# mandyxmq/NeuralBTF-tiny-cuda-nn

Measured on AMD Instinct MI355X. Metric: training steps/sec at batch=2^18, config_hash.json (HashGrid+64-wide MLP), higher is better.
Workload: dtype fp16 storage / fp32 MFMA accumulate; 1 GPU; HashGrid L16 F2 log2T15 s1.5 base16 + FullyFusedMLP W64 H2 ReLU, RelativeL2, Adam, B=2^18; global_batch=262144, per_gpu_batch=262144, parallelism=dp1

## Files before the change

### neuralbtf-tiny-cuda-nn_amd/csrc/capi.cpp

```cpp
#include "../../include/tcnn_mi355x.h"
#include "debug_api.h"

#include <algorithm>
#include <cstring>
#include <mutex>

#include "runtime.h"

using namespace tcnn_amd;

namespace {
thread_local std::string g_last_error;
thread_local std::string g_str;

std::mutex g_log_mutex;
tcnn_log_callback_t g_log_cb = nullptr;
void* g_log_user = nullptr;

template <typename F>
int guard(F&& f) {
	try {
		f();
		return 0;
	} catch (const std::exception& e) {
		g_last_error = e.what();
	} catch (...) {
		g_last_error = "unknown C++ exception";
	}
	return 1;
}

template <typename T, typename F>
T* guard_ptr(F&& f) {
	try {
		return f();
	} catch (const std::exception& e) {
		g_last_error = e.what();
	} catch (...) {
		g_last_error = "unknown C++ exception";
	}
	return nullptr;
}

json parse_json(const char* s) {
	if (!s || !*s) return json::object();
	return json::parse(std::string(s));
}

struct KeepPool {
	std::mutex mu;
	std::vector<std::unique_ptr<DevBuf>> free;
	std::unique_ptr<DevBuf> get() {
		std::lock_guard<std::mutex> lk(mu);
		if (free.empty()) return std::make_unique<DevBuf>();
// ... 643 lines not shown
}
const char* tcnn_trainer_engine(const tcnn_trainer* t) { return t->t->model->engine(); }
const char* tcnn_trainer_inference_engine(const tcnn_trainer* t) { return t->t->model->inference_engine(); }
const char* tcnn_module_engine(const tcnn_module* m) { return m->m->engine(); }
const char* tcnn_module_inference_engine(const tcnn_module* m) { return m->m->inference_engine(); }
int tcnn_trainer_set_max_level(tcnn_trainer* t, float max_level) {
	return guard([&] {
		TCNN_CHECK(t->t->model->grid != nullptr, "trainer model has no grid encoding");
		t->t->model->grid->max_level = max_level;
	});
}

int tcnn_trainer_profile_begin(tcnn_trainer* t) { return tcnn_trainer_profile_begin_sampled(t, 1); }
int tcnn_trainer_profile_begin_sampled(tcnn_trainer* t, uint32_t every) {
	return guard([&] {
		t->t->timer.reset();
		t->t->timer.every = every ? every : 1;
		t->t->timer.counter = 0;
		t->t->timer.enabled = true;
	});
}
int tcnn_trainer_profile_end(tcnn_trainer* t, double* ms, uint32_t n_phases, uint32_t* n_steps) {
	return guard([&] { t->t->profile_end(ms, n_phases, n_steps); });
}

int tcnn_debug_fused_phase_cycles(tcnn_trainer* t, void* stream, uint32_t n, const float* input, const float* target,
                                  uint64_t* host_cycles8) {
	return guard([&] {
		auto& tr = *t->t;
		auto& m = *tr.model;
		TCNN_CHECK(m.mlp.width == 64 && m.mlp.n_input == 32 && m.mlp.n_hidden_layers == 2 && m.grid->desc.n_pos_dims == 2,
		           "phase profile: config_hash shape only");
		hipStream_t st = (hipStream_t)stream;
		tr.training_step(st, n, input, target, false);
		const uint32_t nb = fused_train_n_blocks(64, 32, 2, 2, tr.n_output_dims, false, n);
		const size_t WV = fused_train_waves();
		DevBuf prof;
		prof.reserve((size_t)nb * WV * 16 * 8);
		TCNN_HIP_CHECK(hipMemsetAsync(prof.p, 0, (size_t)nb * WV * 16 * 8, st));
		launch_fused_train_profile(st, n, tr.n_output_dims, tr.w16.p, (const uint8_t*)tr.w16.p + tr.n_mlp * 2, input, target,
		                           tr.ws.dLdenc.p, tr.ws.wgrad_partial.as<float>(), tr.ws.loss_partial.as<float>(),
		                           m.grid->dev_levels(), nb, tr.ws.wimage.p, prof.as<unsigned long long>());
		std::vector<unsigned long long> h((size_t)nb * WV * 16);
		TCNN_HIP_CHECK(hipMemcpyAsync(h.data(), prof.p, h.size() * 8, hipMemcpyDeviceToHost, st));
		TCNN_HIP_CHECK(hipStreamSynchronize(st));
		for (int k = 0; k < 16; ++k) {
			unsigned long long sum = 0;
			for (size_t w = 0; w < (size_t)nb * WV; ++w) sum += h[w * 16 + k];
			host_cycles8[k] = sum;
		}
	});
}

int tcnn_debug_hfma(void* stream, const void* a, const void* b, const void* c, void* out, uint32_t n_pairs) {
	return guard([&] { launch_probe_hfma((hipStream_t)stream, a, b, c, out, n_pairs); });
}

int tcnn_debug_probe(void* stream, float* mfma_out, int16_t* tr_out) {
	return guard([&] { launch_probe((hipStream_t)stream, mfma_out, tr_out); });
}

}

namespace tcnn_amd {
void log_msg(LogSeverity s, const std::string& msg) {
	std::lock_guard<std::mutex> lk(g_log_mutex);
	if (g_log_cb) g_log_cb((int)s, msg.c_str(), g_log_user);
}
}
```

### neuralbtf-tiny-cuda-nn_amd/csrc/dp.cpp

```cpp
#include <dlfcn.h>

#include <rccl/rccl.h>

#include <cstring>
#include <mutex>

#include "runtime.h"

namespace tcnn_amd {

namespace {
struct RcclApi {
	decltype(&ncclGetUniqueId) get_unique_id = nullptr;
	decltype(&ncclCommInitRank) comm_init_rank = nullptr;
	decltype(&ncclCommDestroy) comm_destroy = nullptr;
	decltype(&ncclAllReduce) all_reduce = nullptr;
	decltype(&ncclReduceScatter) reduce_scatter = nullptr;
	decltype(&ncclAllGather) all_gather = nullptr;
	decltype(&ncclGetErrorString) error_string = nullptr;
};

const RcclApi& rccl() {
	static std::once_flag once;
	static RcclApi api;
// ... 56 lines not shown
	if (n) check(rccl().all_reduce(buf, buf, n, ncclFloat32, ncclSum, (ncclComm_t)comm, st), "ncclAllReduce");
}

void DpComm::reduce_scatter_f32(float* buf, size_t per, hipStream_t st) {
	check(rccl().reduce_scatter(buf, buf + (size_t)rank * per, per, ncclFloat32, ncclSum, (ncclComm_t)comm, st), "ncclReduceScatter");
}

void DpComm::all_gather(void* buf, size_t per_elems, int elem_bytes, hipStream_t st) {
	const ncclDataType_t t = elem_bytes == 2 ? ncclFloat16 : ncclUint32;
	check(rccl().all_gather((const uint8_t*)buf + (size_t)rank * per_elems * elem_bytes, buf, per_elems, t, (ncclComm_t)comm, st),
	      "ncclAllGather");
}

static void grow_preserve(DevBuf& b, size_t bytes, size_t valid) {
	if (b.bytes >= bytes) return;
	DevBuf n;
	n.reserve(bytes);
	TCNN_HIP_CHECK(hipMemset(n.p, 0, bytes));
	if (b.p && valid) TCNN_HIP_CHECK(hipMemcpy(n.p, b.p, valid, hipMemcpyDeviceToDevice));
	std::swap(b.p, n.p);
	std::swap(b.bytes, n.bytes);
}

void TrainerHost::set_dp(DpComm* c, bool sharded) {
	TCNN_CHECK(!peer_attached, "set_dp: the trainer is attached to a peer exchange (detach it first)");
	if (dp && dp_sharded && dp_state_partial) dp_gather_state(nullptr);
	TCNN_HIP_CHECK(hipDeviceSynchronize());
	dp = c;
	dp_sharded = c && sharded;
	dp_state_partial = false;
	grad_scale = grad_scale_user / (float)dp_nranks();
	if (graph) set_graph(use_graph);
	if (!dp_sharded) return;
	const uint64_t N = (uint64_t)c->nranks;
	dp_per = (n_params + N - 1) / N;
	const size_t pad = (size_t)(dp_per * N);
	grow_preserve(w32, pad * 4, n_params * 4);
	grow_preserve(w16, pad * 2, n_params * 2);
	grow_preserve(g16, pad * 2, n_params * 2);
	grow_preserve(g32, pad * 4, n_params * 4);
	grow_preserve(m1, pad * 4, n_params * 4);
	grow_preserve(m2, pad * 4, n_params * 4);
	grow_preserve(steps, pad * 4, n_params * 4);
	ws.wimage_valid = false;
}

void TrainerHost::training_step_dp(hipStream_t st, uint32_t B, const float* input, const float* target) {
	DpComm& c = *dp;
	NetworkHost& m = *model;
	const size_t nm = (size_t)n_mlp;
	float* g = g32.as<float>();
	mark(st, 0);
	if (overlapped_ok()) {
		m.fused_kernel(st, ws, B, input, target, n_output_dims, loss_scale, w16.p, false);
		launch_column_sums(st, ws.wgrad_partial.as<float>(), ws.n_fused_blocks, (uint32_t)n_mlp, g);
		launch_sum(st, ws.loss_partial.as<float>(), ws.n_loss_partials, d_loss.as<float>());
		if (!dp_sharded) {
			TCNN_HIP_CHECK(hipEventRecord(c.ev[0], st));
			TCNN_HIP_CHECK(hipStreamWaitEvent(c.cs, c.ev[0], 0));
			c.all_reduce_f32(g, nm, c.cs);
		}
		mark(st, 1);
		m.grid_backward(st, ws, B, input);
		m.grid->backward_acc(st, ws.gbw, B, ws.dLdenc.p, 0, 0, g + nm);
		m.grid->reduce_items(st, ws.gbw, g + nm);
	} else {
		m.fwd_bwd(st, ws, B, input, target, n_output_dims, loss_scale, w16.p, nullptr, nullptr, g);
		launch_sum(st, ws.loss_partial.as<float>(), ws.n_loss_partials, d_loss.as<float>());
		mark(st, 1);
	}
	mark(st, 2);
	TCNN_HIP_CHECK(hipEventRecord(c.ev[1], st));
	TCNN_HIP_CHECK(hipStreamWaitEvent(c.cs, c.ev[1], 0));
	if (dp_sharded) c.reduce_scatter_f32(g, (size_t)dp_per, c.cs);
	else if (overlapped_ok()) c.all_reduce_f32(g + nm, (size_t)(n_params - nm), c.cs);
	else c.all_reduce_f32(g, (size_t)n_params, c.cs);
	TCNN_HIP_CHECK(hipEventRecord(c.ev[2], c.cs));
	TCNN_HIP_CHECK(hipStreamWaitEvent(st, c.ev[2], 0));
	last_B = B;
	if (dp_sharded) {
		const uint64_t lo = std::min<uint64_t>(n_params, (uint64_t)c.rank * dp_per), hi = std::min<uint64_t>(n_params, lo + dp_per);
		optimizer_step_range(st, lo, hi);
		c.all_gather(w16.p, (size_t)dp_per, 2, st);
		dp_state_partial = true;
	} else {
		optimizer_step(st);
	}
	mark(st, 3);
}

void TrainerHost::dp_gather_state(hipStream_t st) {
	if (peer_attached) {
		if (dp_state_partial) dp_peer_gather_state(st);
		return;
	}
	if (!dp || !dp_sharded || !dp_state_partial) return;
	for (DevBuf* b : {&w32, &m1, &m2, &steps}) dp->all_gather(b->p, (size_t)dp_per, 4, st);
	TCNN_HIP_CHECK(hipStreamSynchronize(st));
	dp_state_partial = false;
}

}
```

### neuralbtf-tiny-cuda-nn_amd/csrc/fused.hip

```cpp
#include "kernels.h"

#include <cstdlib>

#include "grid_device.h"
#include "mlp_fused.h"

namespace tcnn_amd {

#define TCNN_FUSED_SHAPES(X) \
	X(64, 32, 2)             \
	X(64, 32, 1)             \
	X(32, 32, 2)             \
	X(32, 32, 1)

bool fused_train_supported(uint32_t W, uint32_t IN, uint32_t NH, uint32_t D, uint32_t F, uint32_t OUTP, int act, HashType h) {
	if (F != 2 || OUTP != 16 || (D != 2 && D != 3) || (act != 0 && act != 1)) return false;
#define X(w, in, nh) if (W == w && IN == in && NH == nh) return true;
	TCNN_FUSED_SHAPES(X)
#undef X
	return false;
}

size_t fused_weight_image_bytes(uint32_t W, uint32_t IN, uint32_t NH) {
#define X(w, in, nh) if (W == w && IN == in && NH == nh) return (size_t)FusedLayout<w, in, nh>::oStage * 2;
// ... 40 lines not shown
}

uint32_t fused_train_waves() { return FUSED_WAVES; }

uint32_t fused_train_n_blocks(uint32_t W, uint32_t IN, uint32_t NH, uint32_t D, uint32_t dims, bool ext_dout, uint32_t B) {
	const uint32_t n_cu = device_cu_count();
	const uint32_t nb = div_round_up(B, 32u * FUSED_WAVES);
	const uint32_t cap = (8u / FUSED_WAVES) * n_cu;
	return nb < cap ? nb : cap;
}

template <int W, int IN, int NH, uint32_t D, HashType H, Act A, bool EXT, bool ENC = false>
static void launch_fused_e(hipStream_t st, const FusedTrainArgs& args, uint32_t n_blocks) {
	constexpr size_t bytes = RegKernelLayout<W, IN, NH>::BYTES;
	static uint64_t done = 0;
	set_dyn_lds((const void*)k_fused_train_grid<W, IN, NH, D, H, A, EXT, ENC>, (int)bytes, done);
	hipLaunchKernelGGL((k_fused_train_grid<W, IN, NH, D, H, A, EXT, ENC>), dim3(n_blocks), dim3(64 * FUSED_WAVES), bytes, st, args);
	TCNN_HIP_CHECK(hipGetLastError());
}

template <int W, int IN, int NH, uint32_t D, HashType H, Act A>
static void launch_fused_t(hipStream_t st, const FusedTrainArgs& args, uint32_t n_blocks) {
	if (args.enc) {
		if (args.dout) launch_fused_e<W, IN, NH, 2, HashType::CoherentPrime, A, true, true>(st, args, n_blocks);
		else launch_fused_e<W, IN, NH, 2, HashType::CoherentPrime, A, false, true>(st, args, n_blocks);
	} else if (args.dout) {
		launch_fused_e<W, IN, NH, D, H, A, true>(st, args, n_blocks);
	} else {
		launch_fused_e<W, IN, NH, D, H, A, false>(st, args, n_blocks);
	}
}

template <int W, int IN, int NH>
static void launch_fused_shape(hipStream_t st, uint32_t D, HashType h, int act, const FusedTrainArgs& a, uint32_t nb) {
#define DISPATCH_H(DD, AA)                                                                                   \
	switch (h) {                                                                                          \
		case HashType::Prime: launch_fused_t<W, IN, NH, DD, HashType::Prime, AA>(st, a, nb); break;       \
		case HashType::ReversedPrime: launch_fused_t<W, IN, NH, DD, HashType::ReversedPrime, AA>(st, a, nb); break; \
		default: launch_fused_t<W, IN, NH, DD, HashType::CoherentPrime, AA>(st, a, nb); break;            \
	}
	if (D == 2) {
		if (act == 1) { DISPATCH_H(2, Act::ReLU) } else { DISPATCH_H(2, Act::None) }
	} else {
		if (act == 1) { DISPATCH_H(3, Act::ReLU) } else { DISPATCH_H(3, Act::None) }
	}
#undef DISPATCH_H
}

void launch_fused_train(hipStream_t st, uint32_t W, uint32_t IN, uint32_t NH, uint32_t D, HashType h, int act,
                        uint32_t B, uint32_t dims, float loss_scale, const void* params16, const void* table16,
                        const float* pos, const float* target, void* out16, void* dLdenc_pairs,
                        float* wgrad_partial, float* loss_partial, const LevelInfo* levels, bool hash_grid,
                        Interp interp, uint32_t n_blocks, const void* dout16, const void* wimage, uint32_t loss_l2,
                        bool inrange_index, const void* enc16, float dout_scale) {
	TCNN_CHECK(B % 32 == 0, "fused train: batch must be a multiple of 32");
	TCNN_CHECK(wimage || ((uintptr_t)params16 & 15) == 0, "fused train: parameters must be 16-byte aligned");
	FusedTrainArgs a;
	a.enc = (const _Float16*)enc16;
	a.loss_l2 = loss_l2;
	a.inrange_index = inrange_index ? 1u : 0u;
	a.wimage = (const _Float16*)wimage;
	a.dout = (const _Float16*)dout16;
	a.dout_scale = dout_scale;
	a.B = B;
	a.dims = dims;
	a.loss_scale = loss_scale;
	a.n_total = (float)(B * dims);
	a.params = (const _Float16*)params16;
	a.table = (const uint32_t*)table16;
	a.pos = pos;
	a.target = target;
	a.out = (_Float16*)out16;
	a.dLdenc = (uint32_t*)dLdenc_pairs;
	a.wgrad_partial = wgrad_partial;
	a.loss_partial = loss_partial;
	a.levels = levels;
	a.hash_grid = hash_grid ? 1u : 0u;
	a.interp = (uint32_t)interp;
	a.prof = nullptr;
#define X(w, in, nh) if (W == w && IN == in && NH == nh) { launch_fused_shape<w, in, nh>(st, D, h, act, a, n_blocks); return; }
	TCNN_FUSED_SHAPES(X)
#undef X
	throw std::runtime_error("fused train: unsupported shape");
}

template <int W, int IN, int NH, Act A, bool SOA>
static void launch_infer_t(hipStream_t st, uint32_t B, const void* wimage, const void* in, void* out) {
	constexpr size_t bytes = (size_t)FusedLayout<W, IN, NH>::oStage * 2;
	static uint64_t done = 0;
	set_dyn_lds((const void*)k_mlp_infer<W, IN, NH, A, SOA>, (int)bytes, done);
	uint32_t nb = div_round_up(B, 64);
	if (nb > 1024) nb = 1024;
	hipLaunchKernelGGL((k_mlp_infer<W, IN, NH, A, SOA>), dim3(nb), dim3(256), bytes, st, B, (const _Float16*)wimage,
	                   (const _Float16*)in, (_Float16*)out);
	TCNN_HIP_CHECK(hipGetLastError());
}

bool mlp_infer_supported(uint32_t W, uint32_t IN, uint32_t NH, uint32_t OUTP, int act) {
	if (OUTP != 16 || (act != 0 && act != 1)) return false;
#define X(w, in, nh) if (W == w && IN == in && NH == nh) return true;
	TCNN_FUSED_SHAPES(X)
#undef X
	return false;
}

void launch_mlp_infer(hipStream_t st, uint32_t W, uint32_t IN, uint32_t NH, int act, bool soa, uint32_t B,
                      const void* wimage, const void* in16, void* out16) {
	TCNN_CHECK(B % 16 == 0, "mlp inference: batch must be a multiple of 16");
	if (B == 0) return;
#define X(w, in, nh)                                                                                      \
	if (W == w && IN == in && NH == nh) {                                                                 \
		if (act == 1) { if (soa) launch_infer_t<w, in, nh, Act::ReLU, true>(st, B, wimage, in16, out16);   \
		                else launch_infer_t<w, in, nh, Act::ReLU, false>(st, B, wimage, in16, out16); }    \
		else { if (soa) launch_infer_t<w, in, nh, Act::None, true>(st, B, wimage, in16, out16);            \
		       else launch_infer_t<w, in, nh, Act::None, false>(st, B, wimage, in16, out16); }             \
		return;                                                                                           \
	}
	TCNN_FUSED_SHAPES(X)
#undef X
	throw std::runtime_error("mlp inference: unsupported shape");
}

template <int W, int IN, int NH, uint32_t D, HashType H, Act A>
static void launch_fused_fwd_t(hipStream_t st, const FusedFwdArgs& a) {
	constexpr size_t bytes = FwdLayout<W, IN, NH>::BYTES;
	static uint64_t done = 0;
	set_dyn_lds((const void*)k_fused_fwd_grid<W, IN, NH, D, H, A>, (int)bytes, done);
	uint32_t nb = div_round_up(a.B, 16u * FWD_WAVES);
	const uint32_t cap = 3 * device_cu_count();
	if (nb > cap) nb = cap;
	hipLaunchKernelGGL((k_fused_fwd_grid<W, IN, NH, D, H, A>), dim3(nb), dim3(64 * FWD_WAVES), bytes, st, a);
	TCNN_HIP_CHECK(hipGetLastError());
// ... 77 lines not shown
```

### neuralbtf-tiny-cuda-nn_amd/csrc/grid.hip

```cpp
#include "kernels.h"

#include <algorithm>
#include <cstdio>
#include <cstdlib>
#include <vector>

#include "adam_device.h"
#include "grid_bwd_lds.h"
#include "grid_device.h"

namespace tcnn_amd {

template <uint32_t D, uint32_t F, HashType H>
__global__ __launch_bounds__(256) void k_grid_fwd(uint32_t B, const float* __restrict__ pos, uint32_t pstride,
                                                  const _Float16* __restrict__ table, _Float16* __restrict__ out,
                                                  uint32_t soa, uint32_t out_stride, const LevelInfo* __restrict__ levels,
                                                  uint32_t hash_grid, uint32_t interp_u, const GridOpts o, uint32_t L) {
	uint32_t i, level;
	if (soa) {
		i = blockIdx.x * blockDim.x + threadIdx.x;
		level = blockIdx.y;
	} else {
		const uint32_t t = blockIdx.x * blockDim.x + threadIdx.x;
		i = t / L;
// ... 515 lines not shown
template <uint32_t D, typename T>
static void grid_bwd_bwd_f(hipStream_t st, uint32_t F, HashType h, dim3 g, uint32_t B, uint32_t L, const float* pos, uint32_t ps,
                           const T* t, const float* gx, const T* dy, uint32_t dys, float* grad, T* ddy,
                           uint32_t ddys, float* dx, const LevelInfo* lv, uint32_t hg, uint32_t in, const GridOpts& go) {
	switch (F) {
		case 1: grid_bwd_bwd_h<D, 1, T>(st, h, g, B, L, pos, ps, t, gx, dy, dys, grad, ddy, ddys, dx, lv, hg, in, go); break;
		case 2: grid_bwd_bwd_h<D, 2, T>(st, h, g, B, L, pos, ps, t, gx, dy, dys, grad, ddy, ddys, dx, lv, hg, in, go); break;
		case 4: grid_bwd_bwd_h<D, 4, T>(st, h, g, B, L, pos, ps, t, gx, dy, dys, grad, ddy, ddys, dx, lv, hg, in, go); break;
		case 8: grid_bwd_bwd_h<D, 8, T>(st, h, g, B, L, pos, ps, t, gx, dy, dys, grad, ddy, ddys, dx, lv, hg, in, go); break;
		default: throw std::runtime_error("GridEncoding: n_features_per_level must be 1, 2, 4 or 8");
	}
}

template <typename T>
static void grid_bwd_bwd_t(hipStream_t st, uint32_t D, uint32_t F, HashType h, uint32_t B, uint32_t L, const float* pos, uint32_t pos_stride,
                           const T* t, const float* dL_ddLdx, const T* dy, uint32_t dy_stride, float* grad32, T* ddy, uint32_t ddy_stride,
                           float* dx, const LevelInfo* levels, bool hash_grid, Interp interp, const GridOpts& go) {
	if (B == 0) return;
	const dim3 g(div_round_up(B, 256));
	const uint32_t hg = hash_grid ? 1u : 0u, in = (uint32_t)interp;
	switch (D) {
		case 2: grid_bwd_bwd_f<2, T>(st, F, h, g, B, L, pos, pos_stride, t, dL_ddLdx, dy, dy_stride, grad32, ddy, ddy_stride, dx, levels, hg, in, go); break;
		case 3: grid_bwd_bwd_f<3, T>(st, F, h, g, B, L, pos, pos_stride, t, dL_ddLdx, dy, dy_stride, grad32, ddy, ddy_stride, dx, levels, hg, in, go); break;
		case 4: grid_bwd_bwd_f<4, T>(st, F, h, g, B, L, pos, pos_stride, t, dL_ddLdx, dy, dy_stride, grad32, ddy, ddy_stride, dx, levels, hg, in, go); break;
		default: throw std::runtime_error("GridEncoding: number of input dims must be 2, 3 or 4");
	}
	TCNN_HIP_CHECK(hipGetLastError());
}

void launch_grid_bwd_bwd(hipStream_t st, uint32_t D, uint32_t F, HashType h, uint32_t B, uint32_t L, const float* pos,
                         uint32_t pos_stride, const void* table16, const float* dL_ddLdx, const void* dLdy16, uint32_t dy_stride,
                         float* grad32, void* dLddLdy16, uint32_t ddy_stride, float* dx, const LevelInfo* levels, bool hash_grid,
                         Interp interp, const GridOpts& go) {
	grid_bwd_bwd_t<_Float16>(st, D, F, h, B, L, pos, pos_stride, (const _Float16*)table16, dL_ddLdx, (const _Float16*)dLdy16, dy_stride, grad32,
	                         (_Float16*)dLddLdy16, ddy_stride, dx, levels, hash_grid, interp, go);
}

void launch_grid_bwd_bwd_f32(hipStream_t st, uint32_t D, uint32_t F, HashType h, uint32_t B, uint32_t L, const float* pos,
                             uint32_t pos_stride, const float* table32, const float* dL_ddLdx, const float* dLdy32, uint32_t dy_stride,
                             float* grad32, float* dLddLdy32, uint32_t ddy_stride, float* dx, const LevelInfo* levels, bool hash_grid,
                             Interp interp, const GridOpts& go) {
	grid_bwd_bwd_t<float>(st, D, F, h, B, L, pos, pos_stride, table32, dL_ddLdx, dLdy32, dy_stride, grad32, dLddLdy32, ddy_stride, dx, levels,
	                      hash_grid, interp, go);
}

static DevBufLite g_dbg_times;
static bool dbg_grid_times() {
	static const bool on = std::getenv("TCNN_DEBUG_GRID_TIMES") != nullptr;
	return on;
}

uint32_t grid_bwd_slot_budget() { return GRID_BWD_SLOTS; }

extern template void grid_bwd_f<2>(hipStream_t, uint32_t, HashType, int, uint32_t, dim3, size_t, uint32_t, const float*, uint32_t,
                                   const _Float16*, const GridSlice*, float*, uint32_t, const LevelInfo*, uint32_t, uint32_t, uint32_t,
                                   const GridBwdLaunch&);
extern template void grid_bwd_f<3>(hipStream_t, uint32_t, HashType, int, uint32_t, dim3, size_t, uint32_t, const float*, uint32_t,
                                   const _Float16*, const GridSlice*, float*, uint32_t, const LevelInfo*, uint32_t, uint32_t, uint32_t,
                                   const GridBwdLaunch&);
extern template void grid_bwd_f<4>(hipStream_t, uint32_t, HashType, int, uint32_t, dim3, size_t, uint32_t, const float*, uint32_t,
                                   const _Float16*, const GridSlice*, float*, uint32_t, const LevelInfo*, uint32_t, uint32_t, uint32_t,
                                   const GridBwdLaunch&);

void launch_grid_bwd(hipStream_t st, uint32_t D, uint32_t F, HashType h, uint32_t B, const float* pos,
                     uint32_t pos_stride, const void* dLdy16, int dy_layout, uint32_t dy_stride, const GridSlice* slices,
                     uint32_t n_slices, uint32_t n_chunks, float* partial, uint32_t partial_stride,
                     const LevelInfo* levels, bool hash_grid, Interp interp, const GridBwdEpilogue* ep, const GridOpts& go,
                     const GridSlice* host_slices, const LevelInfo* host_levels, uint32_t n_levels) {
	const uint32_t n_tail = (ep && ep->enabled) ? ep->n_mlp_groups : 0u;
	if (n_tail == 0 && (n_slices == 0 || B == 0)) return;
	if (B == 0) n_slices = 0;
	const uint32_t ppc = div_round_up(std::max(B, 1u), n_chunks);
	GridBwdLaunch gl{};
	gl.n_items = n_slices;
	gl.n_chunks = n_chunks;
	if (ep) gl.ep = *ep;
	else gl.ep.enabled = 0;
	gl.dbg_times = nullptr;
	gl.opts = go;
	gl.tb.n_items = gl.tb.n_levels = 0;
	if (host_slices && host_levels && n_slices <= GRID_BWD_ARG_ITEMS && n_levels <= GRID_BWD_ARG_LEVELS) {
		gl.tb.n_items = n_slices;
		gl.tb.n_levels = n_levels;
		std::copy(host_slices, host_slices + n_slices, gl.tb.items);
		std::copy(host_levels, host_levels + n_levels, gl.tb.levels);
	}
	dim3 g(n_slices * n_chunks + n_tail);
	if (dbg_grid_times()) gl.dbg_times = (unsigned long long*)g_dbg_times.get((size_t)g.x * 64);
	const size_t lds = GRID_BWD_LDS_BYTES;
	const _Float16* dy = (const _Float16*)dLdy16;
	switch (D) {
		case 2: grid_bwd_f<2>(st, F, h, dy_layout, dy_stride, g, lds, B, pos, pos_stride, dy, slices, partial, partial_stride, levels, hash_grid, (uint32_t)interp, ppc, gl); break;
		case 3: grid_bwd_f<3>(st, F, h, dy_layout, dy_stride, g, lds, B, pos, pos_stride, dy, slices, partial, partial_stride, levels, hash_grid, (uint32_t)interp, ppc, gl); break;
		case 4: grid_bwd_f<4>(st, F, h, dy_layout, dy_stride, g, lds, B, pos, pos_stride, dy, slices, partial, partial_stride, levels, hash_grid, (uint32_t)interp, ppc, gl); break;
		default: throw std::runtime_error("GridEncoding: number of input dims must be 2, 3 or 4");
	}
	TCNN_HIP_CHECK(hipGetLastError());
	if (gl.dbg_times) {
		std::vector<unsigned long long> t((size_t)g.x * 8);
		TCNN_HIP_CHECK(hipStreamSynchronize(st));
		TCNN_HIP_CHECK(hipMemcpy(t.data(), gl.dbg_times, t.size() * 8, hipMemcpyDeviceToHost));
		unsigned long long t0 = ~0ull, t1 = 0;
		for (uint32_t b = 0; b < g.x; ++b) { t0 = std::min(t0, t[8 * b]); t1 = std::max(t1, t[8 * b + 4]); }
		fprintf(stderr, "grid_bwd: %u items x %u chunks + %u tail, span %.1f us\n", n_slices, n_chunks, n_tail, (t1 - t0) / 100.0);
		for (uint32_t it = 0; it < n_slices; ++it) {
			double sum = 0, mx = 0, st0 = 1e30, ph[4] = {0, 0, 0, 0}, ld = 0, zr = 0;
			for (uint32_t c = 0; c < n_chunks; ++c) {
				const uint32_t b = it * n_chunks + c;
				const double d = (t[8 * b + 4] - t[8 * b]) / 100.0;
				sum += d; mx = std::max(mx, d); st0 = std::min(st0, (t[8 * b] - t0) / 100.0);
				for (int k = 0; k < 4; ++k) ph[k] += (t[8 * b + k + 1] - t[8 * b + k]) / 100.0 / n_chunks;
					ld += ((double)t[8 * b + 5] - (double)t[8 * b]) / 100.0 / n_chunks;
					zr += ((double)t[8 * b + 6] - (double)t[8 * b]) / 100.0 / n_chunks;
			}
			fprintf(stderr, "  item %2u: mean %.1f max %.1f us, first start +%.1f | prepass %.1f (zero %.1f, +loads %.1f) accumulate %.1f merge %.1f write %.1f\n", it,
			        sum / n_chunks, mx, st0, ph[0], zr, ld, ph[1], ph[2], ph[3]);
		}
		for (uint32_t b = n_slices * n_chunks; b < g.x; ++b)
			fprintf(stderr, "  tail wg %u: %.1f us start +%.1f\n", b - n_slices * n_chunks, (t[8 * b + 4] - t[8 * b]) / 100.0, (t[8 * b] - t0) / 100.0);
	}
}

}
```

### neuralbtf-tiny-cuda-nn_amd/csrc/grid_bwd_lds.h

```cpp
#pragma once

#include "kernels.h"

#include <algorithm>
#include <cstdio>
#include <cstdlib>
#include <vector>

#include "adam_device.h"
#include "grid_device.h"

namespace tcnn_amd {

constexpr uint32_t GRID_BWD_THREADS = 1024;
constexpr uint32_t GRID_BWD_LDS_BYTES = 128 * 1024;
constexpr uint32_t GRID_BWD_SLOTS = GRID_BWD_LDS_BYTES / 4;



__device__ __forceinline__ void lds_add_i32(int* acc, float v) {
	__hip_atomic_fetch_add(acc, __float2int_rn(v), __ATOMIC_RELAXED, __HIP_MEMORY_SCOPE_WORKGROUP);
}

enum : int { IDX_HASH_POW2 = 0, IDX_DENSE = 1, IDX_GENERIC = 2, IDX_HASH_RANGE = 3 };

template <uint32_t D, HashType H, int KIND>
__device__ __forceinline__ uint32_t level_index(bool hash_grid, uint32_t size, uint32_t res, const uint32_t* g) {
	if constexpr (KIND == IDX_HASH_POW2 || KIND == IDX_HASH_RANGE) {
		uint32_t h = 0;
#pragma unroll
		for (uint32_t d = 0; d < D; ++d) h ^= g[d] * hash_prime<H>(d);
		return h & (size - 1);
	} else if constexpr (KIND == IDX_DENSE) {
		uint32_t idx = 0, stride = 1;
#pragma unroll
		for (uint32_t d = 0; d < D; ++d) {
			idx += g[d] * stride;
			stride *= res;
		}
		if (idx >= size) {
			idx -= size;
			if (idx >= size) idx %= size;
		}
		return idx;
	} else {
		return grid_index<D, H>(hash_grid, size, res, g);
	}
}

template <uint32_t D, uint32_t F, HashType H, int KIND, int MODE, bool OPTS>
__device__ __forceinline__ void accum_point(const float (&x)[D], const float (&dy)[F], uint32_t i, uint32_t level, uint32_t B,
                                            const LevelInfo& li, bool hash_grid, Interp interp, uint32_t begin, uint32_t len,
                                            uint32_t f0, uint32_t nf, int* acc, const GridOpts& o) {
	float p[D];
	uint32_t pg[D];
#pragma unroll
	for (uint32_t d = 0; d < D; ++d) pos_fract(x[d], li.scale, interp, p[d], pg[d]);
	const bool nearest = interp == Interp::Nearest;
	const bool single = nearest || (OPTS && o.stochastic);
	uint32_t cbits = 0;
	if (single && !nearest) {
		const float smp = random_val_1337(i + level * B);
// ... 49 lines not shown
		t[1][1] = t[1][0] + hash_prime<H>(1);
	} else {
		t[0][0] = g[0];
		t[0][1] = g[0] + 1u;
		t[1][0] = g[1] * li.res;
		t[1][1] = t[1][0] + li.res;
	}
#pragma unroll
	for (uint32_t c = 0; c < 4; ++c) {
		const uint32_t bx = c & 1u, by = c >> 1;
		const float w = (bx ? p[0] : 1.0f - p[0]) * (by ? p[1] : 1.0f - p[1]);
		const float wh = (float)f16_rn(w);
		uint32_t rel;
		if constexpr (KIND == IDX_HASH_POW2) {
			rel = (t[0][bx] ^ t[1][by]) & (li.size - 1u);
		} else if constexpr (KIND == IDX_HASH_RANGE) {
			rel = ((t[0][bx] ^ t[1][by]) & (li.size - 1u)) - begin;
			if (rel >= len) continue;
		} else {
			const uint32_t d = t[0][bx] + t[1][by];
			rel = __builtin_elementwise_min(d, d - li.size);
		}
		if constexpr (MODE == 0) {
			const int a = __float2int_rn(wh * dy[0]);
			const int b = __float2int_rn(wh * dy[1]);
			const unsigned long long pk = (unsigned long long)(((long long)b << 32) + (long long)a);
			__hip_atomic_fetch_add((unsigned long long*)acc + rel, pk, __ATOMIC_RELAXED, __HIP_MEMORY_SCOPE_WORKGROUP);
		} else {
#pragma unroll
			for (uint32_t f = 0; f < F; ++f) {
				if constexpr (MODE == 1) {
					if (f - f0 < nf) lds_add_i32(&acc[rel * nf + (f - f0)], wh * dy[f]);
				} else {
					lds_add_i32(&acc[rel * F + f], wh * dy[f]);
				}
			}
		}
	}
}

constexpr uint32_t GRID_BWD_PR = 32, GRID_BWD_PU = 8;
static_assert(GRID_BWD_THREADS * GRID_BWD_PR == GRID_BWD_REG_POINTS, "kernels.h GRID_BWD_REG_POINTS");
template <uint32_t D>
__device__ __forceinline__ void load_pos_batch(const float* __restrict__ pos, uint32_t pstride, uint32_t i0, uint32_t i1, uint32_t k,
                                               float (&dst)[GRID_BWD_PU][D]) {
#pragma unroll
	for (uint32_t u = 0; u < GRID_BWD_PU; ++u) {
		const uint32_t i = i0 + threadIdx.x + (k * GRID_BWD_PU + u) * blockDim.x;
#pragma unroll
		for (uint32_t d = 0; d < D; ++d) dst[u][d] = i < i1 ? pos[(size_t)i * pstride + d] : 0.0f;
	}
}

template <uint32_t D, uint32_t F, HashType H, int KIND, int MODE>
__device__ __forceinline__ void grid_bwd_points_regs(const uint32_t (&dyb)[GRID_BWD_PR], const float (&xs0)[GRID_BWD_PU][D],
                                                     uint32_t B, const float* __restrict__ pos,
                                                     uint32_t pstride, uint32_t level, const LevelInfo& li, bool hash_grid,
                                                     Interp interp, uint32_t begin, uint32_t len, uint32_t f0, uint32_t nf,
                                                     uint32_t i0, uint32_t i1, float scale, int* acc, const GridOpts& o) {
	constexpr uint32_t U = GRID_BWD_PU, NB = GRID_BWD_PR / U;
	constexpr bool FAST_KIND = D == 2 && (KIND == IDX_HASH_POW2 || KIND == IDX_DENSE || KIND == IDX_HASH_RANGE);
	const bool fast = FAST_KIND && interp == Interp::Linear && (begin == 0 || KIND == IDX_HASH_RANGE);
	float xs[2][U][D];
#pragma unroll
	for (uint32_t u = 0; u < U; ++u)
#pragma unroll
		for (uint32_t d = 0; d < D; ++d) xs[0][u][d] = xs0[u][d];
#pragma unroll
	for (uint32_t k = 0; k < NB; ++k) {
		if (i0 + threadIdx.x + k * U * blockDim.x >= i1) break;
		if (k + 1 < NB) load_pos_batch<D>(pos, pstride, i0, i1, k + 1, xs[(k + 1) & 1]);
		bool fast_b = fast;
		if constexpr (FAST_KIND && KIND == IDX_DENSE) {
			bool inr = true;
#pragma unroll
			for (uint32_t u = 0; u < U; ++u)
#pragma unroll
				for (uint32_t d = 0; d < D; ++d) inr = inr && xs[k & 1][u][d] >= 0.0f && xs[k & 1][u][d] <= 1.0f;
			fast_b = fast_b && __builtin_amdgcn_ballot_w64(!inr) == 0;
		}
		if (fast_b) {
			if constexpr (FAST_KIND) {
				if (i0 + threadIdx.x + (k * U + U - 1) * blockDim.x < i1) {
#pragma unroll
					for (uint32_t u = 0; u < U; ++u) {
						const uint32_t p = k * U + u;
						float dy[F];
#pragma unroll
						for (uint32_t f = 0; f < F; ++f) dy[f] = dy_bits_feature(dyb[p], f) * scale;
						accum_point_2d_fast<F, H, KIND, MODE>(*(const float(*)[2]) & xs[k & 1][u][0], dy, li, f0, nf, acc, begin, len);
					}
				} else {
#pragma unroll
					for (uint32_t u = 0; u < U; ++u) {
						const uint32_t p = k * U + u;
						if (i0 + threadIdx.x + p * blockDim.x >= i1) break;
						float dy[F];
#pragma unroll
						for (uint32_t f = 0; f < F; ++f) dy[f] = dy_bits_feature(dyb[p], f) * scale;
						accum_point_2d_fast<F, H, KIND, MODE>(*(const float(*)[2]) & xs[k & 1][u][0], dy, li, f0, nf, acc, begin, len);
					}
				}
			}
			continue;
		}
#pragma unroll
		for (uint32_t u = 0; u < U; ++u) {
			const uint32_t p = k * U + u;
			const uint32_t i = i0 + threadIdx.x + p * blockDim.x;
			if (i >= i1) break;
			float dy[F];
#pragma unroll
			for (uint32_t f = 0; f < F; ++f) dy[f] = dy_bits_feature(dyb[p], f) * scale;
			accum_point<D, F, H, KIND, MODE, false>(xs[k & 1][u], dy, i, level, B, li, hash_grid, interp, begin, len, f0, nf, acc, o);
		}
	}
}

template <uint32_t D, uint32_t F, HashType H, int KIND, int MODE, bool OPTS>
__device__ __forceinline__ void grid_bwd_points(int layout, uint32_t B, const float* __restrict__ pos, uint32_t pstride,
                                                const _Float16* __restrict__ dLdy, uint32_t dy_stride, uint32_t level,
                                                const LevelInfo& li, bool hash_grid, Interp interp, uint32_t begin,
                                                uint32_t len, uint32_t f0, uint32_t nf, uint32_t i0, uint32_t i1, float scale,
                                                int* acc, const GridOpts& o) {
	constexpr uint32_t NF = F;
	constexpr uint32_t U = 8;
	constexpr bool FAST_KIND = D == 2 && !OPTS && (KIND == IDX_HASH_POW2 || KIND == IDX_DENSE || KIND == IDX_HASH_RANGE);
	const bool fast = FAST_KIND && interp == Interp::Linear && (begin == 0 || KIND == IDX_HASH_RANGE);
	for (uint32_t base = i0 + threadIdx.x; base < i1; base += U * blockDim.x) {
		float xs[U][D], dy[U][NF];
#pragma unroll
		for (uint32_t u = 0; u < U; ++u) {
			const uint32_t i = base + u * blockDim.x;
			float v[F];
			if (i < i1) {
#pragma unroll
				for (uint32_t d = 0; d < D; ++d) xs[u][d] = pos[(size_t)i * pstride + d];
				load_dy<F>(layout, dLdy, dy_stride, level, B, i, v);
			} else {
#pragma unroll
				for (uint32_t d = 0; d < D; ++d) xs[u][d] = 0.0f;
#pragma unroll
				for (uint32_t f = 0; f < F; ++f) v[f] = 0.0f;
			}
			if (OPTS && i < i1 && (float)level > grid_max_level(o, i, F) + 1e-3f) {
#pragma unroll
				for (uint32_t f = 0; f < F; ++f) v[f] = 0.0f;
			}
#pragma unroll
			for (uint32_t f = 0; f < F; ++f) dy[u][f] = v[f] * scale;
		}
		if constexpr (FAST_KIND) {
			bool fast_b = fast;
			if constexpr (KIND == IDX_DENSE) {
				bool inr = true;
#pragma unroll
				for (uint32_t u = 0; u < U; ++u)
#pragma unroll
					for (uint32_t d = 0; d < D; ++d) inr = inr && xs[u][d] >= 0.0f && xs[u][d] <= 1.0f;
				fast_b = fast_b && __builtin_amdgcn_ballot_w64(!inr) == 0;
			}
			if (fast_b && base + (U - 1) * blockDim.x < i1) {
#pragma unroll
				for (uint32_t u = 0; u < U; ++u)
					accum_point_2d_fast<F, H, KIND, MODE>(*(const float(*)[2]) & xs[u][0], dy[u], li, f0, nf, acc, begin, len);
				continue;
			}
		}
#pragma unroll
		for (uint32_t u = 0; u < U; ++u) {
			if (base + u * blockDim.x >= i1) break;
			accum_point<D, F, H, KIND, MODE, OPTS>(xs[u], dy[u], base + u * blockDim.x, level, B, li, hash_grid, interp, begin, len, f0,
			                                       nf, acc, o);
		}
	}
}

template <uint32_t D, uint32_t F, HashType H, int KIND, bool OPTS>
__device__ __forceinline__ void grid_bwd_mode(int mode, int layout, uint32_t B, const float* pos, uint32_t pstride,
                                              const _Float16* dLdy, uint32_t dy_stride, uint32_t level, const LevelInfo& li,
                                              bool hash_grid, Interp interp, uint32_t begin, uint32_t len, uint32_t f0,
                                              uint32_t nf, uint32_t i0, uint32_t i1, float scale, int* acc, const GridOpts& o) {
	if constexpr (F == 2) {
		if (mode == 0) { grid_bwd_points<D, F, H, KIND, 0, OPTS>(layout, B, pos, pstride, dLdy, dy_stride, level, li, hash_grid, interp, begin, len, f0, nf, i0, i1, scale, acc, o); return; }
	} else if constexpr (F > 2) {
		if (mode == 2) { grid_bwd_points<D, F, H, KIND, 2, OPTS>(layout, B, pos, pstride, dLdy, dy_stride, level, li, hash_grid, interp, begin, len, f0, nf, i0, i1, scale, acc, o); return; }
	}
	grid_bwd_points<D, F, H, KIND, 1, OPTS>(layout, B, pos, pstride, dLdy, dy_stride, level, li, hash_grid, interp, begin, len, f0, nf, i0, i1, scale, acc, o);
}

template <uint32_t D, uint32_t F, HashType H, int KIND>
__device__ __forceinline__ void grid_bwd_mode_regs(int mode, const uint32_t (&dyb)[GRID_BWD_PR], const float (&xs0)[GRID_BWD_PU][D],
                                                   uint32_t B, const float* pos,
                                                   uint32_t pstride, uint32_t level, const LevelInfo& li, bool hash_grid, Interp interp,
                                                   uint32_t begin, uint32_t len, uint32_t f0, uint32_t nf, uint32_t i0, uint32_t i1,
                                                   float scale, int* acc, const GridOpts& o) {
	if constexpr (F == 2) {
		if (mode == 0) { grid_bwd_points_regs<D, F, H, KIND, 0>(dyb, xs0, B, pos, pstride, level, li, hash_grid, interp, begin, len, f0, nf, i0, i1, scale, acc, o); return; }
	}
	grid_bwd_points_regs<D, F, H, KIND, 1>(dyb, xs0, B, pos, pstride, level, li, hash_grid, interp, begin, len, f0, nf, i0, i1, scale, acc, o);
}

__device__ __forceinline__ void grid_bwd_mlp_tail(const GridBwdEpilogue& ep, uint32_t g, float* lds) {
	const uint32_t N = ep.n_mlp;
	const uint32_t cb = column_block(N, ep.n_mlp_groups);
	const uint32_t c0 = g * cb;
	if (c0 < N) {
		const uint32_t ncol = min(cb, N - c0);
		float* out = lds;
		float* tmp = lds + cb;
		block_column_sums(ep.wpart, ep.n_wparts, N, c0, ncol, tmp, out);
		const uint32_t nW0 = ep.W * ep.IN, nWh = (ep.NH - 1) * ep.W * ep.W;
		for (uint32_t t = threadIdx.x; t < ncol; t += blockDim.x) {
			const uint32_t i = c0 + t;
			const float s = out[t];
			if (ep.fin.out) {
				grad_finalize_store(s, ep.fin.s, ep.fin.out, i, ep.fin.out_f32);
				continue;
			}
			ep.buf.g32[i] = s;
			if (!ep.apply_adam) continue;
			const _Float16 h = adam_update(ep.adam_mlp, ep.buf, i, s);
			uint32_t o;
			if (i < nW0) {
				o = (i / ep.IN) * ep.RSI + i % ep.IN;
			} else if (i < nW0 + nWh) {
				const uint32_t k = i - nW0;
				o = ep.oWh + (k / ep.W) * ep.RSW + k % ep.W;
			} else {
				const uint32_t k = i - nW0 - nWh;
				o = ep.oWo + (4 * ((k / ep.W) & 3) + (k / ep.W) / 4) * ep.RSW + k % ep.W;
			}
			ep.wimage[o] = h;
		}
	}
	if (g == 0) {
		__syncthreads();
		const float l = block_sum_fixed(ep.lpart, ep.n_wparts, lds);
		if (threadIdx.x == 0) *ep.d_loss = l;
	}
}

constexpr uint32_t GRID_BWD_ARG_ITEMS = 32, GRID_BWD_ARG_LEVELS = 24;
struct GridBwdTables {
	uint32_t n_items, n_levels;
	GridSlice items[GRID_BWD_ARG_ITEMS];
	LevelInfo levels[GRID_BWD_ARG_LEVELS];
};

template <uint32_t D, uint32_t F, HashType H, bool OPTS>
__global__ __launch_bounds__(GRID_BWD_THREADS) void k_grid_bwd_lds(
	int layout, uint32_t B, const float* __restrict__ pos, uint32_t pstride, const _Float16* __restrict__ dLdy, uint32_t dy_stride,
	const GridSlice* __restrict__ items, float* __restrict__ partial, uint32_t partial_stride,
	const LevelInfo* __restrict__ levels, uint32_t hash_grid, uint32_t interp_u, uint32_t pts_per_chunk, uint32_t n_items,
	uint32_t n_chunks, const GridBwdEpilogue ep, unsigned long long* dbg_times, const GridOpts o, const GridBwdTables tb) {
	extern __shared__ __attribute__((aligned(16))) int acc[];
	const unsigned long long t_start = dbg_times ? wall_clock64() : 0ull;
	__shared__ float red[GRID_BWD_THREADS / 64];
	if (blockIdx.x >= n_items * n_chunks) {
		grid_bwd_mlp_tail(ep, blockIdx.x - n_items * n_chunks, (float*)acc);
		if (dbg_times && threadIdx.x == 0) {
			dbg_times[8 * blockIdx.x] = t_start;
			for (int k = 1; k < 5; ++k) dbg_times[8 * blockIdx.x + k] = wall_clock64();
		}
		return;
	}
	const uint32_t item = blockIdx.x / n_chunks, chunk = blockIdx.x % n_chunks;
	GridSlice it;
	if (item < tb.n_items) {
		it.level = tb.items[item].level;
		it.begin = tb.items[item].begin;
		it.end = tb.items[item].end;
		it.f0 = tb.items[item].f0;
		it.nf = tb.items[item].nf;
	} else {
		it = items[item];
	}
	const uint32_t len = it.end - it.begin;
	const uint32_t nf = it.nf, f0 = it.f0;
	const Interp interp = (Interp)interp_u;
	const uint32_t i0 = chunk * pts_per_chunk;
	const uint32_t i1 = min(B, i0 + pts_per_chunk);

	float m = 0.0f;
	constexpr bool REGS_OK = D == 2 && F <= 2 && !OPTS;
	const uint32_t n_pts = i1 > i0 ? i1 - i0 : 0u;
	const bool use_regs = REGS_OK && n_pts <= GRID_BWD_THREADS * GRID_BWD_PR;
	uint32_t dyb[GRID_BWD_PR];
	float xs0[GRID_BWD_PU][D];
	if constexpr (REGS_OK) {
		if (use_regs) {
#pragma unroll
			for (uint32_t p = 0; p < GRID_BWD_PR; ++p) {
				const uint32_t i = i0 + threadIdx.x + p * blockDim.x;
				dyb[p] = i < i1 ? load_dy_bits<F>(layout, dLdy, dy_stride, it.level, B, i) : 0u;
			}
			load_pos_batch<D>(pos, pstride, i0, i1, 0, xs0);
		}
	}
	LevelInfo li;
	if (it.level < tb.n_levels) {
		li.scale = tb.levels[it.level].scale;
		li.res = tb.levels[it.level].res;
		li.offset = tb.levels[it.level].offset;
		li.size = tb.levels[it.level].size;
	} else {
		li = levels[it.level];
	}
	const uint32_t slots = len * nf;
	const uint32_t R = max(1u, min(16u, GRID_BWD_SLOTS / max(slots, 1u)));
	const uint32_t nz = R * slots;
	for (uint32_t j = 4 * threadIdx.x; j + 4 <= nz; j += 4 * blockDim.x) *(int4*)(acc + j) = int4{0, 0, 0, 0};
	for (uint32_t j = nz / 4 * 4 + threadIdx.x; j < nz; j += blockDim.x) acc[j] = 0;
	if (dbg_times && threadIdx.x == 0) dbg_times[8 * blockIdx.x + 6] = wall_clock64();
	int* acc_w = acc + ((threadIdx.x >> 6) % R) * slots;
	if constexpr (REGS_OK) {
		if (use_regs) {
#pragma unroll
			for (uint32_t p = 0; p < GRID_BWD_PR; ++p) {
				float s = 0.0f;
#pragma unroll
				for (uint32_t f = 0; f < F; ++f) {
					const float v = dy_bits_feature(dyb[p], f);
					if (f - f0 < nf) s = __builtin_isfinite(v) ? fmaxf(s, fabsf(v)) : __builtin_inff();
				}
				m += s;
			}
		}
	}
	if (!use_regs) {
		for (uint32_t ib = i0 + threadIdx.x; ib < i1; ib += 8 * blockDim.x) {
			float dy[8][F];
#pragma unroll
			for (uint32_t u = 0; u < 8; ++u) {
				const uint32_t i = ib + u * blockDim.x;
				if (i < i1) load_dy<F>(layout, dLdy, dy_stride, it.level, B, i, dy[u]);
				else {
#pragma unroll
					for (uint32_t f = 0; f < F; ++f) dy[u][f] = 0.0f;
				}
			}
#pragma unroll
			for (uint32_t u = 0; u < 8; ++u) {
				float s = 0.0f;
#pragma unroll
				for (uint32_t f = 0; f < F; ++f)
					if (f - f0 < nf) s = __builtin_isfinite(dy[u][f]) ? fmaxf(s, fabsf(dy[u][f])) : __builtin_inff();
				m += s;
			}
		}
	}
	if (dbg_times && threadIdx.x == 0) dbg_times[8 * blockIdx.x + 5] = wall_clock64() + (m != m ? 1 : 0);
#pragma unroll
	for (int o = 32; o > 0; o >>= 1) m += __shfl_xor(m, o);
	if ((threadIdx.x & 63) == 0) red[threadIdx.x >> 6] = m;
	__syncthreads();
	m = red[0];
#pragma unroll
	for (uint32_t w = 1; w < GRID_BWD_THREADS / 64; ++w) m += red[w];
	const float P = (float)(i1 > i0 ? i1 - i0 : 1u);
	const bool finite = __builtin_isfinite(m);
	int e = 0;
	if (m > 0.0f && finite) {
		const float lim = (2147483647.0f - (float)(1u << D) * P) / (m * 1.01f);
		e = ilogbf(lim);
		e = max(-126, min(e, 100));
	}
	const float scale = ldexpf(1.0f, e);
	if (dbg_times && threadIdx.x == 0) dbg_times[8 * blockIdx.x + 1] = wall_clock64();

	uint64_t full = 1;
	for (uint32_t d = 0; d < D; ++d) full = full * li.res > 0xffffffffull ? 0x100000000ull : full * li.res;
	const bool whole = it.begin == 0 && len == li.size;
	int kind = IDX_GENERIC;
	if (whole && full <= li.size) kind = IDX_DENSE;
	else if (whole && hash_grid && (li.size & (li.size - 1)) == 0) kind = IDX_HASH_POW2;
	else if (!whole && hash_grid && (li.size & (li.size - 1)) == 0 && full > li.size) kind = IDX_HASH_RANGE;
	const int mode = nf < F ? 1 : (F == 2 ? 0 : 2);
	if constexpr (REGS_OK) {
		if (use_regs) {
			if (kind == IDX_HASH_POW2)
				grid_bwd_mode_regs<D, F, H, IDX_HASH_POW2>(mode, dyb, xs0, B, pos, pstride, it.level, li, hash_grid != 0, interp, it.begin, len, f0, nf, i0, i1, scale, acc_w, o);
			else if (kind == IDX_HASH_RANGE)
				grid_bwd_mode_regs<D, F, H, IDX_HASH_RANGE>(mode, dyb, xs0, B, pos, pstride, it.level, li, hash_grid != 0, interp, it.begin, len, f0, nf, i0, i1, scale, acc_w, o);
			else if (kind == IDX_DENSE)
				grid_bwd_mode_regs<D, F, H, IDX_DENSE>(mode, dyb, xs0, B, pos, pstride, it.level, li, hash_grid != 0, interp, it.begin, len, f0, nf, i0, i1, scale, acc_w, o);
			else
				grid_bwd_mode_regs<D, F, H, IDX_GENERIC>(mode, dyb, xs0, B, pos, pstride, it.level, li, hash_grid != 0, interp, it.begin, len, f0, nf, i0, i1, scale, acc_w, o);
		}
	}
	if (!use_regs) {
	if (kind == IDX_HASH_POW2)
		grid_bwd_mode<D, F, H, IDX_HASH_POW2, OPTS>(mode, layout, B, pos, pstride, dLdy, dy_stride, it.level, li, hash_grid != 0, interp, it.begin, len, f0, nf, i0, i1, scale, acc_w, o);
	else if (kind == IDX_HASH_RANGE)
		grid_bwd_mode<D, F, H, IDX_HASH_RANGE, OPTS>(mode, layout, B, pos, pstride, dLdy, dy_stride, it.level, li, hash_grid != 0, interp, it.begin, len, f0, nf, i0, i1, scale, acc_w, o);
	else if (kind == IDX_DENSE)
		grid_bwd_mode<D, F, H, IDX_DENSE, OPTS>(mode, layout, B, pos, pstride, dLdy, dy_stride, it.level, li, hash_grid != 0, interp, it.begin, len, f0, nf, i0, i1, scale, acc_w, o);
	else
		grid_bwd_mode<D, F, H, IDX_GENERIC, OPTS>(mode, layout, B, pos, pstride, dLdy, dy_stride, it.level, li, hash_grid != 0, interp, it.begin, len, f0, nf, i0, i1, scale, acc_w, o);
	}
	__syncthreads();
	if (dbg_times && threadIdx.x == 0) dbg_times[8 * blockIdx.x + 2] = wall_clock64();
	if (R > 1) {
		if (mode == 0) {
			long long* a64 = (long long*)acc;
			for (uint32_t j = threadIdx.x; j < len; j += blockDim.x) {
				long long t = a64[j];
				for (uint32_t r = 1; r < R; ++r) t += a64[(size_t)r * len + j];
				a64[j] = t;
			}
		} else {
			for (uint32_t j = threadIdx.x; j < slots; j += blockDim.x) {
				int t = acc[j];
				for (uint32_t r = 1; r < R; ++r) t += acc[(size_t)r * slots + j];
				acc[j] = t;
			}
		}
		__syncthreads();
	}
	if (dbg_times && threadIdx.x == 0) dbg_times[8 * blockIdx.x + 3] = wall_clock64();
	const float inv = finite ? ldexpf(1.0f, -e) : __builtin_nanf("");
	float* dst = partial + (size_t)chunk * partial_stride + (size_t)li.offset * F + (size_t)f0 * li.size + (size_t)it.begin * nf;
	if (mode == 0) {
		const long long* a64 = (const long long*)acc;
		auto dec = [&](long long t) {
			const int lo = (int)(uint32_t)(unsigned long long)t;
			const int hi = (int)((t - (long long)lo) >> 32);
			return make_float2((float)lo * inv, (float)hi * inv);
		};
		const bool al = (((uintptr_t)dst) & 15) == 0;
		for (uint32_t j = 2 * threadIdx.x; j < len; j += 2 * blockDim.x) {
			const float2 a = dec(a64[j]);
			if (al && j + 1 < len) {
				const float2 b = dec(a64[j + 1]);
				*(f4*)(dst + 2 * j) = f4{a.x, a.y, b.x, b.y};
			} else {
				*(float2*)(dst + 2 * j) = a;
				if (j + 1 < len) *(float2*)(dst + 2 * j + 2) = dec(a64[j + 1]);
			}
		}
	} else {
		const uint32_t n = len * nf;
		const bool al = (((uintptr_t)dst) & 15) == 0;
		for (uint32_t j = 4 * threadIdx.x; j < n; j += 4 * blockDim.x) {
			if (al && j + 4 <= n) {
				const int4 v = *(const int4*)(acc + j);
				*(f4*)(dst + j) = f4{(float)v.x * inv, (float)v.y * inv, (float)v.z * inv, (float)v.w * inv};
			} else {
				for (uint32_t k = j; k < n && k < j + 4; ++k) dst[k] = (float)acc[k] * inv;
			}
		}
	}
	if (dbg_times && threadIdx.x == 0) {
		dbg_times[8 * blockIdx.x] = t_start;
		dbg_times[8 * blockIdx.x + 4] = wall_clock64();
	}
}

struct GridBwdLaunch {
	uint32_t n_items, n_chunks;
	GridBwdEpilogue ep;
	unsigned long long* dbg_times;
	GridOpts opts;
	GridBwdTables tb;
};

template <uint32_t D, uint32_t F, HashType H>
static void grid_bwd_t(hipStream_t st, int layout, uint32_t dys, dim3 g, size_t lds, uint32_t B, const float* pos, uint32_t ps,
                       const _Float16* dy, const GridSlice* sl, float* part, uint32_t pstr, const LevelInfo* lv,
                       uint32_t hg, uint32_t in, uint32_t ppc, const GridBwdLaunch& gl) {
	static uint64_t done0 = 0, done1 = 0;
	set_dyn_lds((const void*)k_grid_bwd_lds<D, F, H, false>, (int)GRID_BWD_LDS_BYTES, done0);
	set_dyn_lds((const void*)k_grid_bwd_lds<D, F, H, true>, (int)GRID_BWD_LDS_BYTES, done1);
	if (gl.opts.active)
		hipLaunchKernelGGL((k_grid_bwd_lds<D, F, H, true>), g, dim3(GRID_BWD_THREADS), lds, st, layout, B, pos, ps, dy, dys, sl, part, pstr, lv, hg, in,
		                   ppc, gl.n_items, gl.n_chunks, gl.ep, gl.dbg_times, gl.opts, gl.tb);
	else
		hipLaunchKernelGGL((k_grid_bwd_lds<D, F, H, false>), g, dim3(GRID_BWD_THREADS), lds, st, layout, B, pos, ps, dy, dys, sl, part, pstr, lv, hg, in,
		                   ppc, gl.n_items, gl.n_chunks, gl.ep, gl.dbg_times, gl.opts, gl.tb);
}

template <uint32_t D, uint32_t F>
static void grid_bwd_h(hipStream_t st, HashType h, int pairs, uint32_t dys, dim3 g, size_t lds, uint32_t B, const float* pos, uint32_t ps,
                       const _Float16* dy, const GridSlice* sl, float* part, uint32_t pstr, const LevelInfo* lv,
                       uint32_t hg, uint32_t in, uint32_t ppc, const GridBwdLaunch& gl) {
	switch (h) {
		case HashType::Prime: grid_bwd_t<D, F, HashType::Prime>(st, pairs, dys, g, lds, B, pos, ps, dy, sl, part, pstr, lv, hg, in, ppc, gl); break;
		case HashType::ReversedPrime: grid_bwd_t<D, F, HashType::ReversedPrime>(st, pairs, dys, g, lds, B, pos, ps, dy, sl, part, pstr, lv, hg, in, ppc, gl); break;
		default: grid_bwd_t<D, F, HashType::CoherentPrime>(st, pairs, dys, g, lds, B, pos, ps, dy, sl, part, pstr, lv, hg, in, ppc, gl); break;
	}
}

template <uint32_t D>
void grid_bwd_f(hipStream_t st, uint32_t F, HashType h, int pairs, uint32_t dys, dim3 g, size_t lds, uint32_t B, const float* pos,
                       uint32_t ps, const _Float16* dy, const GridSlice* sl, float* part, uint32_t pstr, const LevelInfo* lv,
                       uint32_t hg, uint32_t in, uint32_t ppc, const GridBwdLaunch& gl) {
	switch (F) {
		case 1: grid_bwd_h<D, 1>(st, h, pairs, dys, g, lds, B, pos, ps, dy, sl, part, pstr, lv, hg, in, ppc, gl); break;
		case 2: grid_bwd_h<D, 2>(st, h, pairs, dys, g, lds, B, pos, ps, dy, sl, part, pstr, lv, hg, in, ppc, gl); break;
		case 4: grid_bwd_h<D, 4>(st, h, pairs, dys, g, lds, B, pos, ps, dy, sl, part, pstr, lv, hg, in, ppc, gl); break;
		case 8: grid_bwd_h<D, 8>(st, h, pairs, dys, g, lds, B, pos, ps, dy, sl, part, pstr, lv, hg, in, ppc, gl); break;
		default: throw std::runtime_error("GridEncoding: n_features_per_level must be 1, 2, 4 or 8");
	}
}

}
```

### neuralbtf-tiny-cuda-nn_amd/csrc/kernels.h

```cpp
#pragma once

#include "common.h"

namespace tcnn_amd {

struct LevelInfo;

struct GridSlice {
	uint32_t level;
	uint32_t begin;
	uint32_t end;
	uint32_t f0;
	uint32_t nf;
};

struct GridBinLevel {
	uint32_t level;
	uint32_t slice_log2;
	uint32_t n_slices;
	uint32_t bucket_base;
};

struct GridBinArgs {
	const GridBinLevel* lv;
// ... 37 lines not shown
	float loss_scale, grad_scale;
	float lr, beta1, beta2, eps, l2_reg, rel_decay, abs_decay, clip, nonmat_lr_factor;
	float lower_lr_bound, upper_lr_bound;
	int opt_matrix, opt_nonmatrix;
	float inv_loss_scale;
	uint32_t begin;
	const float* part;
	uint32_t n_parts, part_stride;
	const float* factor_table;
	uint32_t factor_n;
	const GridSlabMap* part_map;
};

struct AdamBuffers {
	float* w32;
	_Float16* w16;
	float* g32;
	_Float16* g16;
	float* m1;
	float* m2;
	uint32_t* steps;
};

struct GradFinalize {
	void* out = nullptr;
	float s = 1.0f;
	int out_f32 = 0;
};

struct GridBwdEpilogue {
	int enabled;
	int apply_adam;
	AdamArgs adam_mlp;
	AdamBuffers buf;
	uint32_t n_mlp_groups;
	const float* wpart;
	uint32_t n_wparts, n_mlp;
	const float* lpart;
	float* d_loss;
	_Float16* wimage;
	uint32_t W, IN, NH, RSI, RSW, oWh, oWo;
	GradFinalize fin;
};

bool fused_train_supported(uint32_t W, uint32_t IN, uint32_t NH, uint32_t D, uint32_t F, uint32_t OUTP, int act, HashType h);
uint32_t fused_train_waves();
uint32_t fused_train_n_blocks(uint32_t W, uint32_t IN, uint32_t NH, uint32_t D, uint32_t dims, bool ext_dout, uint32_t B);
void launch_fused_train(hipStream_t st, uint32_t W, uint32_t IN, uint32_t NH, uint32_t D, HashType h, int act,
                        uint32_t B, uint32_t dims, float loss_scale, const void* params16, const void* table16,
                        const float* pos, const float* target, void* out16, void* dLdenc_pairs,
                        float* wgrad_partial, float* loss_partial, const LevelInfo* levels, bool hash_grid,
                        Interp interp, uint32_t n_blocks, const void* dout16, const void* wimage, uint32_t loss_l2 = 0, bool inrange_index = false,
                        const void* enc16 = nullptr,
                        float dout_scale = 1.0f);
size_t fused_weight_image_bytes(uint32_t W, uint32_t IN, uint32_t NH);
void launch_pack_weights(hipStream_t st, uint32_t W, uint32_t IN, uint32_t NH, const void* params16, void* image);

bool mlp_infer_supported(uint32_t W, uint32_t IN, uint32_t NH, uint32_t OUTP, int act);
void launch_fused_fwd(hipStream_t st, uint32_t W, uint32_t IN, uint32_t NH, uint32_t D, HashType h, int act, uint32_t B,
                      const void* wimage, const void* params16, const void* table16, const float* pos, const LevelInfo* levels, bool hash_grid,
                      Interp interp, bool inrange_index, void* enc16, void* out16);
void launch_mlp_infer(hipStream_t st, uint32_t W, uint32_t IN, uint32_t NH, int act, bool soa, uint32_t B,
                      const void* wimage, const void* in16, void* out16);
void launch_trim_cast(hipStream_t st, uint32_t B, uint32_t in_stride, uint32_t n_out, const void* in16, float* out);

void launch_grid_fwd(hipStream_t st, uint32_t D, uint32_t F, HashType h, uint32_t B, uint32_t L,
                     const float* pos, uint32_t pos_stride, const void* table16, void* out16, bool soa,
                     uint32_t out_stride, const LevelInfo* levels, bool hash_grid, Interp interp, const GridOpts& opts = GridOpts{},
                     uint32_t aos_row_cols = 0);

uint32_t grid_bwd_slot_budget();
void launch_grid_bwd(hipStream_t st, uint32_t D, uint32_t F, HashType h, uint32_t B, const float* pos,
                     uint32_t pos_stride, const void* dLdy16, int dy_layout, uint32_t dy_stride, const GridSlice* slices,
                     uint32_t n_slices, uint32_t n_chunks, float* partial, uint32_t partial_stride,
                     const LevelInfo* levels, bool hash_grid, Interp interp, const GridBwdEpilogue* ep = nullptr,
                     const GridOpts& opts = GridOpts{}, const GridSlice* host_slices = nullptr, const LevelInfo* host_levels = nullptr,
                     uint32_t n_levels = 0);
void launch_grid_bin(hipStream_t st, uint32_t D, uint32_t F, HashType h, uint32_t B, const float* pos, uint32_t pos_stride,
                     const void* dLdy16, int dy_layout, uint32_t dy_stride, const LevelInfo* levels, bool hash_grid, Interp interp,
                     const GridBinArgs& a, const GridOpts& opts = GridOpts{});
struct GridAccAdam {
	AdamArgs a;
	AdamBuffers buf;
	uint32_t param_base;
	int write_grad32;
};
void launch_grid_acc(hipStream_t st, uint32_t D, uint32_t F, uint32_t B, const void* dLdy16, int dy_layout, uint32_t dy_stride,
                     const LevelInfo* levels, const GridBinArgs& a, float* grad32, const GridAccAdam* adam);

void launch_grid_bwd_input(hipStream_t st, uint32_t D, uint32_t F, HashType h, uint32_t B, uint32_t L, const float* pos,
                           uint32_t pos_stride, const void* table16, const void* dLdy16, int dy_layout, uint32_t dy_stride, float* dx,
                           uint32_t dx_stride, const LevelInfo* levels, bool hash_grid, Interp interp, const GridOpts& opts = GridOpts{});
void launch_grid_bwd_bwd(hipStream_t st, uint32_t D, uint32_t F, HashType h, uint32_t B, uint32_t L, const float* pos,
                         uint32_t pos_stride, const void* table16, const float* dL_ddLdx, const void* dLdy16, uint32_t dy_stride,
                         float* grad32, void* dLddLdy16, uint32_t ddy_stride, float* dx, const LevelInfo* levels, bool hash_grid,
                         Interp interp, const GridOpts& opts = GridOpts{});
void fused_image_layout(uint32_t W, uint32_t IN, uint32_t NH, uint32_t* RSI, uint32_t* RSW, uint32_t* oWh, uint32_t* oWo);

void launch_column_sums(hipStream_t st, const float* in, uint32_t n_parts, uint32_t N, float* out);
uint32_t mlp_tail_groups();
void launch_grid_slab_reduce(hipStream_t st, const float* in, uint32_t n_parts, uint32_t stride, uint32_t n, float* out,
                             const GridSlabMap* map, GradFinalize fin = {});
size_t reduce_partials_tmp_floats(uint32_t n_parts, uint32_t n);
void launch_reduce_partials(hipStream_t st, const float* in, uint32_t n_parts, uint32_t stride, uint32_t n,
                            float* out, float* tmp);

uint32_t tile_train_lds_bytes(uint32_t W, uint32_t IN, uint32_t NH);
bool tile_train_supported(uint32_t W, uint32_t IN, uint32_t NH, uint32_t outp, int act);
uint32_t tile_train_blocks(uint32_t B, uint32_t W, uint32_t IN, uint32_t NH);
uint32_t tile_train_n_streamed(uint32_t W, uint32_t IN, uint32_t NH);
uint32_t tile_train_wT_bytes(uint32_t W, uint32_t IN, uint32_t NH);
struct TileGridEnc {
	const float* pos;
	const void* table16;
	const LevelInfo* levels;
	HashType hash;
	uint32_t hash_grid, inrange;
};
bool tile_train_genc_ok(uint32_t W, uint32_t IN, uint32_t NH, int act, uint32_t B, HashType h);
void launch_mlp_tile_train(hipStream_t st, uint32_t W, uint32_t IN, uint32_t NH, int act, int out_act, uint32_t B, uint32_t dims,
                           float loss_scale, uint32_t loss_l2, const void* params16, const void* enc16, const float* target,
                           const void* dout16, void* out16, void* dldenc, int dldenc_pairs, float* wgrad_partial, float* loss_partial,
                           void* wT, const TileGridEnc* genc = nullptr);
bool tile_infer_supported(uint32_t W, uint32_t IN, uint32_t NH, uint32_t outp, int act);
uint32_t tile_infer_blocks(uint32_t B, uint32_t W, uint32_t IN, uint32_t NH);
void launch_mlp_tile_infer(hipStream_t st, uint32_t W, uint32_t IN, uint32_t NH, int act, int out_act, uint32_t B, const void* params16,
                           const void* enc16, void* out16);

void launch_generate_uniform(hipStream_t st, uint64_t n, uint64_t state, uint64_t inc, float* out, float lo, float hi);
void launch_generate_logistic(hipStream_t st, uint64_t n, uint64_t state, uint64_t inc, float* out, float mean, float stddev);
// ... 96 lines not shown
```

### neuralbtf-tiny-cuda-nn_amd/csrc/mlp_fused.h

```cpp
#pragma once

#include "common.h"
#include "grid_device.h"
#include "lds_dma.h"
#include "kernels.h"

namespace tcnn_amd {

enum class Act : int { None = 0, ReLU = 1 };

__device__ __forceinline__ f4 mfma16(h8 a, h8 b, f4 c) { return __builtin_amdgcn_mfma_f32_16x16x32_f16(a, b, c, 0, 0, 0); }

__device__ __forceinline__ h8 cat8(h4 lo, h4 hi) { return __builtin_shufflevector(lo, hi, 0, 1, 2, 3, 4, 5, 6, 7); }

typedef uint32_t u32x2 __attribute__((ext_vector_type(2)));

__device__ __forceinline__ h4 zero4() { return h4{(_Float16)0.0f, (_Float16)0.0f, (_Float16)0.0f, (_Float16)0.0f}; }

__device__ __forceinline__ uint32_t relu_pk_f16(uint32_t x) {
	const h2 m = __builtin_elementwise_max(__builtin_bit_cast(h2, x), (h2){(_Float16)0.0f, (_Float16)0.0f});
	return __builtin_bit_cast(uint32_t, m) & 0x7fff7fffu;
}
template <Act A>
__device__ __forceinline__ h4 act_fwd(f4 v) {
// ... 183 lines not shown
	constexpr int N0 = W * IN, NHW = L::NHM * W * W;
	const uint4* p = (const uint4*)params;
	for (int v = tid; v < L::N_MLP / 8; v += nthreads) {
		const int idx = 8 * v;
		int o;
		if (idx < N0) {
			o = L::oW0 + (idx / IN) * L::RSI + idx % IN;
		} else if (idx < N0 + NHW) {
			const int k = idx - N0;
			o = L::oWh + (k / W) * L::RSW + k % W;
		} else {
			const int k = idx - N0 - NHW;
			o = L::oWo + out_row(k / W) * L::RSW + k % W;
		}
		*(uint4*)(smem + o) = p[v];
	}
}

template <int W, int IN, int NH>
__global__ void k_pack_weights(const _Float16* __restrict__ params, _Float16* __restrict__ image) {
	load_weights_lds<W, IN, NH>(image, params, blockIdx.x * blockDim.x + threadIdx.x, gridDim.x * blockDim.x);
}

__device__ __forceinline__ void copy_image_to_lds(_Float16* smem, const _Float16* __restrict__ image, int n_halves, int tid, int nthreads) {
	const uint4* src = (const uint4*)image;
	uint4* dst = (uint4*)smem;
	const int n16 = n_halves / 8;
	for (int k = tid; k < n16; k += nthreads) dst[k] = src[k];
}

struct FusedTrainArgs {
	const _Float16* wimage;
	uint32_t B;
	uint32_t dims;
	float loss_scale;
	float n_total;
	uint32_t loss_l2;
	uint32_t inrange_index;
	const _Float16* params;
	const uint32_t* table;
	const float* pos;
	const float* target;
	_Float16* out;
	uint32_t* dLdenc;
	float* wgrad_partial;
	float* loss_partial;
	const LevelInfo* levels;
	uint32_t hash_grid;
	uint32_t interp;
	const _Float16* dout;
	float dout_scale;
	const _Float16* enc;
	unsigned long long* prof;
};

__device__ __forceinline__ unsigned long long stamp() {
	unsigned long long t;
	__builtin_amdgcn_sched_barrier(0);
	asm volatile("s_memtime %0\n\ts_waitcnt lgkmcnt(0)" : "=s"(t)::"memory");
	__builtin_amdgcn_sched_barrier(0);
	return t;
}

template <int W, int IN, int NH>
struct WgradAcc {
	using L = FusedLayout<W, IN, NH>;
	f4 Wo[L::NT];
	f4 H[L::NHM > 0 ? L::NHM : 1][L::NT][L::NT];
	f4 W0[L::NT][L::NTI];
	float loss;
	__device__ __forceinline__ void zero() {
		const f4 fz = {0.0f, 0.0f, 0.0f, 0.0f};
#pragma unroll
		for (int t = 0; t < L::NT; ++t) {
			Wo[t] = fz;
#pragma unroll
			for (int u = 0; u < L::NTI; ++u) W0[t][u] = fz;
#pragma unroll
			for (int j = 0; j < (L::NHM > 0 ? L::NHM : 1); ++j)
#pragma unroll
				for (int u = 0; u < L::NT; ++u) H[j][t][u] = fz;
		}
		loss = 0.0f;
	}
};

template <int W, int IN, int NH, Act ACT, bool EXT_DOUT, bool PROF, class TargetFn>
__device__ __forceinline__ void slice_fwd_loss(const FusedTrainArgs& a, uint32_t base, int c, int q, const h4 (&xt)[2][IN / 16],
                                               TargetFn target, const h4 (&Gext)[2], const _Float16* sW0, const _Float16* sWh,
                                               const _Float16* sWo, h4 (&act)[NH][2][W / 16], h4 (&G)[2], float& loss,
                                               unsigned long long (&ph)[8], unsigned long long& t0) {
	using L = FusedLayout<W, IN, NH>;
	constexpr int NT = L::NT, KW = L::KW, KI = L::KI;
	const f4 fz = {0.0f, 0.0f, 0.0f, 0.0f};
	unsigned long long t1;
	{
		f4 ac[2][NT];
#pragma unroll
		for (int t = 0; t < NT; ++t) {
			ac[0][t] = fz; ac[1][t] = fz;
#pragma unroll
			for (int s = 0; s < KI; ++s) {
				const h8 af = lds_afrag(sW0, L::RSI, 16 * t + c, 32 * s + 4 * q);
				ac[0][t] = mfma16(af, cat8(xt[0][2 * s], xt[0][2 * s + 1]), ac[0][t]);
				ac[1][t] = mfma16(af, cat8(xt[1][2 * s], xt[1][2 * s + 1]), ac[1][t]);
			}
		}
// ... 10 lines not shown
#pragma unroll
			for (int s = 0; s < KW; ++s) {
				const h8 af = lds_afrag(Wm, L::RSW, 16 * t + c, 32 * s + 4 * q);
				ac[0][t] = mfma16(af, cat8(act[j - 1][0][2 * s], act[j - 1][0][2 * s + 1]), ac[0][t]);
				ac[1][t] = mfma16(af, cat8(act[j - 1][1][2 * s], act[j - 1][1][2 * s + 1]), ac[1][t]);
			}
		}
#pragma unroll
		for (int t = 0; t < NT; ++t) { act[j][0][t] = act_fwd<ACT>(ac[0][t]); act[j][1][t] = act_fwd<ACT>(ac[1][t]); }
	}
	if constexpr (PROF) { t1 = stamp(); ph[1] += t1 - t0; t0 = t1; }
	{
		f4 yacc[2] = {fz, fz};
#pragma unroll
		for (int s = 0; s < KW; ++s) {
			const h8 af = lds_afrag(sWo, L::RSW, c, 32 * s + 4 * q);
			yacc[0] = mfma16(af, cat8(act[NH - 1][0][2 * s], act[NH - 1][0][2 * s + 1]), yacc[0]);
			yacc[1] = mfma16(af, cat8(act[NH - 1][1][2 * s], act[NH - 1][1][2 * s + 1]), yacc[1]);
		}
#pragma unroll
		for (int tau = 0; tau < 2; ++tau) {
			const uint32_t i = base + 16 * tau + c;
			if constexpr (EXT_DOUT) {
				(void)Gext;
				const _Float16* dp = a.dout + (size_t)i * 16 + q;
				const float ds = a.dout_scale;
				G[tau] = h4{f16_rn((float)dp[0] * ds), f16_rn((float)dp[4] * ds), f16_rn((float)dp[8] * ds), f16_rn((float)dp[12] * ds)};
				continue;
			}
			const h4 y = __builtin_convertvector(yacc[tau], h4);
			if (a.out) {
#pragma unroll
				for (int r = 0; r < 4; ++r) a.out[(size_t)i * 16 + 4 * r + q] = y[r];
			}
			h4 g = zero4();
#pragma unroll
			for (int r = 0; r < 4; ++r) {
				if (4u * r >= a.dims) break;
				const uint32_t o = 4 * r + q;
				if (o < a.dims) {
					const float p = (float)y[r];
					const float pse = a.loss_l2 ? 1.0f : __builtin_fmaf(p, p, 0.01f);
					const float d = p - target(tau, r, o);
					loss += d * d / pse / a.n_total;
					const float gr = 2.0f * d / pse;
					g[r] = f16_rn(a.loss_scale * gr / a.n_total);
				}
			}
			G[tau] = g;
		}
	}
}

template <int W, int IN, int NH, Act ACT, bool EXT_DOUT, bool PROF, class TargetFn, class AfterLossFn>
__device__ __forceinline__ void fused_slice(const FusedTrainArgs& a, uint32_t base, int c, int q, const h4 (&xt)[2][IN / 16],
                                            TargetFn target, AfterLossFn after_loss, const h4 (&Gext)[2], const _Float16* sW0,
                                            const _Float16* sWh, const _Float16* sWo, _Float16* bufA, _Float16* bufD,
                                            WgradAcc<W, IN, NH>& acc, unsigned long long (&ph)[8], unsigned long long& t0) {
	using L = FusedLayout<W, IN, NH>;
	constexpr int NT = L::NT, KW = L::KW, NTI = L::NTI;
	const f4 fz = {0.0f, 0.0f, 0.0f, 0.0f};
	unsigned long long t1;
	h4 act[NH][2][NT];
	h4 G[2];
	slice_fwd_loss<W, IN, NH, ACT, EXT_DOUT, PROF>(a, base, c, q, xt, target, Gext, sW0, sWh, sWo, act, G, acc.loss, ph, t0);
	after_loss();
	if constexpr (PROF) { t1 = stamp(); ph[2] += t1 - t0; t0 = t1; }
#pragma unroll
	for (int tau = 0; tau < 2; ++tau) {
		stg_put(bufD, 16 * tau + c, 4 * q, G[tau]);
#pragma unroll
		for (int t = 0; t < NT; ++t) stg_put(bufA, 16 * tau + c, 16 * t + 4 * q, act[NH - 1][tau][t]);
	}
	lds_fence();
	{
		const h8 ga = stg_trfrag(bufD, q, c, 0);
#pragma unroll
		for (int nt = 0; nt < NT; ++nt) acc.Wo[nt] = mfma16(ga, stg_trfrag(bufA, q, c, nt), acc.Wo[nt]);
	}
	h4 dl[2][NT];
#pragma unroll
	for (int t = 0; t < NT; ++t) {
		const h8 af = lds_wtfrag16(sWo, L::RSW, 16 * t, q, c);
		dl[0][t] = act_bwd<ACT>(act[NH - 1][0][t], mfma16(af, cat8(G[0], zero4()), fz));
		dl[1][t] = act_bwd<ACT>(act[NH - 1][1][t], mfma16(af, cat8(G[1], zero4()), fz));
	}
#pragma unroll
	for (int j = NH - 1; j >= 1; --j) {
		lds_fence();
#pragma unroll
		for (int tau = 0; tau < 2; ++tau) {
#pragma unroll
			for (int t = 0; t < NT; ++t) {
				stg_put(bufD, 16 * tau + c, 16 * t + 4 * q, dl[tau][t]);
				stg_put(bufA, 16 * tau + c, 16 * t + 4 * q, act[j - 1][tau][t]);
			}
		}
		lds_fence();
		{
			h8 bf[NT];
#pragma unroll
			for (int nt = 0; nt < NT; ++nt) bf[nt] = stg_trfrag(bufA, q, c, nt);
#pragma unroll
			for (int mt = 0; mt < NT; ++mt) {
				const h8 ad = stg_trfrag(bufD, q, c, mt);
#pragma unroll
				for (int nt = 0; nt < NT; ++nt) acc.H[j - 1][mt][nt] = mfma16(ad, bf[nt], acc.H[j - 1][mt][nt]);
			}
		}
		const _Float16* Wm = sWh + (j - 1) * W * L::RSW;
#pragma unroll
		for (int t = 0; t < NT; ++t) {
			f4 acc0 = fz, acc1 = fz;
#pragma unroll
			for (int s = 0; s < KW; ++s) {
				const h8 af = lds_wtfrag(Wm, L::RSW, 32 * s, 16 * t, q, c);
				acc0 = mfma16(af, stg_afrag(bufD, c, 32 * s + 4 * q), acc0);
				acc1 = mfma16(af, stg_afrag(bufD, 16 + c, 32 * s + 4 * q), acc1);
			}
			dl[0][t] = act_bwd<ACT>(act[j - 1][0][t], acc0);
			dl[1][t] = act_bwd<ACT>(act[j - 1][1][t], acc1);
		}
	}
	if constexpr (PROF) { t1 = stamp(); ph[3] += t1 - t0; t0 = t1; }
	lds_fence();
#pragma unroll
	for (int tau = 0; tau < 2; ++tau) {
#pragma unroll
		for (int t = 0; t < NT; ++t) stg_put(bufD, 16 * tau + c, 16 * t + 4 * q, dl[tau][t]);
#pragma unroll
		for (int u = 0; u < NTI; ++u) stg_put(bufA, 16 * tau + c, 16 * u + 4 * q, xt[tau][u]);
	}
	lds_fence();
	{
		h8 bf[NTI];
#pragma unroll
		for (int u = 0; u < NTI; ++u) bf[u] = stg_trfrag(bufA, q, c, u);
#pragma unroll
		for (int mt = 0; mt < NT; ++mt) {
			const h8 ad = stg_trfrag(bufD, q, c, mt);
#pragma unroll
			for (int u = 0; u < NTI; ++u) acc.W0[mt][u] = mfma16(ad, bf[u], acc.W0[mt][u]);
		}
	}
	if constexpr (PROF) { t1 = stamp(); ph[4] += t1 - t0; t0 = t1; }
#pragma unroll
	for (int u = 0; u < NTI; ++u) {
		f4 acc0 = fz, acc1 = fz;
#pragma unroll
		for (int s = 0; s < KW; ++s) {
			const h8 af = lds_wtfrag(sW0, L::RSI, 32 * s, 16 * u, q, c);
			acc0 = mfma16(af, stg_afrag(bufD, c, 32 * s + 4 * q), acc0);
			acc1 = mfma16(af, stg_afrag(bufD, 16 + c, 32 * s + 4 * q), acc1);
		}
		const h4 d0 = __builtin_convertvector(acc0, h4);
		const h4 d1 = __builtin_convertvector(acc1, h4);
		const uint32_t lv = 8 * u + 2 * q;
		const uint32_t i0 = base + c, i1 = base + 16 + c;
		a.dLdenc[(size_t)lv * a.B + i0] = __builtin_bit_cast(uint32_t, h2{d0[0], d0[1]});
		a.dLdenc[(size_t)(lv + 1) * a.B + i0] = __builtin_bit_cast(uint32_t, h2{d0[2], d0[3]});
		a.dLdenc[(size_t)lv * a.B + i1] = __builtin_bit_cast(uint32_t, h2{d1[0], d1[1]});
		a.dLdenc[(size_t)(lv + 1) * a.B + i1] = __builtin_bit_cast(uint32_t, h2{d1[2], d1[3]});
	}
	if constexpr (PROF) { t1 = stamp(); ph[5] += t1 - t0; t0 = t1; }
}

template <int W, int IN, int NH>
__device__ __forceinline__ uint32_t wgrad_frag_to_param(uint32_t f) {
	using L = FusedLayout<W, IN, NH>;
	constexpr uint32_t NT = L::NT, NTI = L::NTI, NHM = L::NHM;
	constexpr uint32_t oH = W * IN, oO = W * IN + NHM * W * W;
	const uint32_t j = f / 256, rem = f % 256, lane = rem / 4, r = rem % 4, q = lane >> 4, c = lane & 15;
	if (j < NT * NTI) {
		const uint32_t mt = j / NTI, u = j % NTI, n = 16 * mt + 4 * q + r;
		return n * IN + 16 * u + c;
	}
	if (j < NT * NTI + NHM * NT * NT) {
		const uint32_t k = j - NT * NTI, jj = k / (NT * NT), mt = (k / NT) % NT, nt = k % NT, n = 16 * mt + 4 * q + r;
		return oH + jj * W * W + n * W + 16 * nt + c;
	}
	const uint32_t nt = j - NT * NTI - NHM * NT * NT;
	return oO + (4 * r + q) * W + 16 * nt + c;
}

template <int W, int IN, int NH, int WAVES, bool PROF = false>
__device__ __forceinline__ void block_reduce_wgrad(WgradAcc<W, IN, NH>& acc, float* slab, const FusedTrainArgs& a,
                                                   int tid, int wave, int lane, unsigned long long* pst = nullptr) {
	int np = 0;
	auto pstamp = [&] {
		if constexpr (PROF) {
			const unsigned long long t = stamp();
			if (lane == 0 && np < 6) pst[np] = t;
			++np;
		}
	};
	using L = FusedLayout<W, IN, NH>;
	constexpr int NT = L::NT, NTI = L::NTI, NHM = L::NHM, N = L::N_MLP;
	static_assert(N % 256 == 0, "whole f4 per lane");
#pragma unroll
	for (int off = 32; off > 0; off >>= 1) acc.loss += __shfl_xor(acc.loss, off);
	float* lsum = slab + 2 * N;
	if (lane == 0) lsum[wave] = acc.loss;
	auto visit = [&](float* S, bool add) {
		int j = 0;
		auto io = [&](f4& v) {
			f4* p = (f4*)(S + 256 * j + 4 * lane);
			if (add) v += *p; else *p = v;
			++j;
		};
#pragma unroll
		for (int mt = 0; mt < NT; ++mt)
#pragma unroll
			for (int u = 0; u < NTI; ++u) io(acc.W0[mt][u]);
#pragma unroll
		for (int jj = 0; jj < NHM; ++jj)
// ... 166 lines not shown
				for (int s = 0; s < KI; ++s)
#pragma unroll
					for (int pp = 0; pp < 4; ++pp) {
						const float sc = sLvl[16 * s + 8 * (pp >> 1) + 2 * q + (pp & 1)].scale;
#pragma unroll
						for (int tau = 0; tau < 2; ++tau) {
							const h2 e = encode_level_f2_pair_combine<D>(g[s][pp][tau], sc, xA[tau], xB[tau], par);
							xt[tau][2 * s + (pp >> 1)][2 * (pp & 1) + 0] = e[0];
							xt[tau][2 * s + (pp >> 1)][2 * (pp & 1) + 1] = e[1];
						}
					}
			} else
#endif
			{
#pragma unroll
			for (int s = 0; s < KI; ++s)
#pragma unroll
				for (int pp = 0; pp < 4; ++pp) {
					const int level = 16 * s + 8 * (pp >> 1) + 2 * q + (pp & 1);
					const LevelConsts<D> lc = level_consts<D>(sLvl[level], hash_grid);
#pragma unroll
					for (int tau = 0; tau < 2; ++tau) {
#if TCNN_PAIR_GATHER
						const h2 e = encode_level_f2_pair<D, H>(a.table, lc, xA[tau], xB[tau], par);
#else
						const h2 e = encode_level_f2_inrange<D, H>(a.table, lc, xs[tau]);
#endif
						xt[tau][2 * s + (pp >> 1)][2 * (pp & 1) + 0] = e[0];
						xt[tau][2 * s + (pp >> 1)][2 * (pp & 1) + 1] = e[1];
					}
				}
			}
		} else {
#pragma unroll
			for (int tau = 0; tau < 2; ++tau)
#pragma unroll
				for (int s = 0; s < KI; ++s)
#pragma unroll
					for (int pp = 0; pp < 4; ++pp) {
						const int level = 16 * s + 8 * (pp >> 1) + 2 * q + (pp & 1);
						const h2 e = encode_level_f2<D, H>(a.table, sLvl[level], hash_grid, interp, xs[tau]);
						xt[tau][2 * s + (pp >> 1)][2 * (pp & 1) + 0] = e[0];
						xt[tau][2 * s + (pp >> 1)][2 * (pp & 1) + 1] = e[1];
					}
		}
		if (image_pending) {
			asm volatile("s_waitcnt vmcnt(0)" ::: "memory");
			__syncthreads();
			image_pending = false;
		}
		if constexpr (PROF) { t1 = stamp(); ph[0] += t1 - t0; t0 = t1; }
		auto target = [&](int tau, int r, uint32_t o) { return r == 0 ? tg[tau] : a.target[(size_t)(base + 16 * tau + c) * a.dims + o]; };
		auto after_loss = [] {};
		fused_slice<W, IN, NH, ACT, EXT_DOUT, PROF>(a, base, c, q, xt, target, after_loss, Gext, smem + L::oW0,
		                                            smem + L::oWh, smem + L::oWo, bufA, bufD, acc, ph, t0);
	}
	if (image_pending) {
		asm volatile("s_waitcnt vmcnt(0)" ::: "memory");
		__syncthreads();
	}
	if constexpr (PROF) {
		if (lane == 0) {
			unsigned long long* o = a.prof + (size_t)(blockIdx.x * FUSED_WAVES + wave) * 16;
			for (int k = 0; k < 7; ++k) o[k] = ph[k];
		}
		t0 = stamp();
	}
	__syncthreads();
	unsigned long long ts = 0;
	unsigned long long pst[6] = {0, 0, 0, 0, 0, 0};
	if constexpr (PROF) ts = stamp();
	block_reduce_wgrad<W, IN, NH, FUSED_WAVES, PROF>(acc, (float*)smem, a, tid, wave, lane, pst);
	if constexpr (PROF) {
		t1 = stamp();
		if (lane == 0) {
			unsigned long long* o = a.prof + (size_t)(blockIdx.x * FUSED_WAVES + wave) * 16;
			o[7] = t1 - ts;
			o[8] = ts - t0;
			unsigned long long prev = ts;
			for (int k = 0; k < 6; ++k) {
				if (pst[k] == 0) break;
				o[9 + k] = pst[k] - prev;
				prev = pst[k];
			}
		}
	}
}


template <int W, int IN, int NH, Act ACT, bool SOA>
__global__ __launch_bounds__(256, 2) void k_mlp_infer(uint32_t B, const _Float16* __restrict__ wimage,
                                                      const _Float16* __restrict__ in, _Float16* __restrict__ out) {
	using L = FusedLayout<W, IN, NH>;
	constexpr int NT = L::NT, KW = L::KW, NTI = L::NTI, KI = L::KI;
	extern __shared__ __attribute__((aligned(16))) _Float16 smem[];
	const int tid = threadIdx.x, lane = tid & 63, wave = tid >> 6;
	const int c = lane & 15, q = lane >> 4;
	copy_image_to_lds(smem, wimage, L::oStage, tid, 256);
	__syncthreads();
	const _Float16* sW0 = smem + L::oW0;
	const _Float16* sWh = smem + L::oWh;
	const _Float16* sWo = smem + L::oWo;
	const f4 fz = {0.0f, 0.0f, 0.0f, 0.0f};
	const uint32_t n_chunks = B / 16;
	for (uint32_t chunk = blockIdx.x * 4 + wave; chunk < n_chunks; chunk += gridDim.x * 4) {
		const uint32_t i = chunk * 16 + c;
		h4 xt[NTI];
// ... 180 lines not shown
```

### neuralbtf-tiny-cuda-nn_amd/csrc/runtime.cpp

```cpp
#include "runtime.h"

#include <algorithm>
#include <cctype>
#include <cmath>
#include <cstring>
#include <limits>
#include <random>

namespace tcnn_amd {

static constexpr uint64_t PCG32_MULT = 0x5851f42d4c957f2dULL;

void Pcg32::seed(uint64_t initstate, uint64_t initseq) {
	state = 0u;
	inc = (initseq << 1u) | 1u;
	next_uint();
	state += initstate;
	next_uint();
}

uint32_t Pcg32::next_uint() {
	uint64_t old = state;
	state = old * PCG32_MULT + inc;
	uint32_t xorshifted = (uint32_t)(((old >> 18u) ^ old) >> 27u);
// ... 23 lines not shown
	state = acc_mult * state + acc_plus;
}

static void strided_uniform(Pcg32& rng, size_t n, float* out, float lo, float hi) {
	const size_t n_gen = 4;
	const size_t n_thr = (n + n_gen - 1) / n_gen;
	const size_t n_threads = (n_thr + 127) / 128 * 128;
	const float range = hi - lo;
	for (size_t i = 0; i < n_threads; ++i) {
		Pcg32 r = rng;
		r.advance((int64_t)(i * n_gen));
		for (size_t j = 0; j < n_gen; ++j) {
			size_t idx = i + n_threads * j;
			if (idx >= n) break;
			out[idx] = std::fma(r.next_float(), range, lo);
		}
	}
	rng.advance((int64_t)n);
}

DevBuf::~DevBuf() { release(); }

void DevBuf::release() {
	if (p) (void)hipFree(p);
	p = nullptr;
	bytes = 0;
}

void DevBuf::reserve(size_t n) {
	if (n <= bytes && p) return;
	release();
	if (n == 0) n = 16;
	TCNN_HIP_CHECK(hipMalloc(&p, n));
	bytes = n;
	static const bool poison = std::getenv("TCNN_DEBUG_POISON") != nullptr;
	if (poison) TCNN_HIP_CHECK(hipMemset(p, 0xff, n));
}

EngineSwitches EngineSwitches::from_env() {
	EngineSwitches s;
	auto on = [](const char* n) { return std::getenv(n) != nullptr; };
	s.no_fused_grid = on("TCNN_NO_FUSED_GRID");
	s.no_tile_engine = on("TCNN_NO_TILE_ENGINE");
	s.no_inrange_index = on("TCNN_NO_INRANGE_INDEX");
	s.split_encode = on("TCNN_SPLIT_ENCODE");
	s.no_forward_keep = on("TCNN_NO_FORWARD_KEEP");
	s.split_forward = on("TCNN_SPLIT_FORWARD");
	const char* bin = std::getenv("TCNN_GRID_BIN");
	s.grid_bin_all = bin && std::string(bin) == "all";
	if (const char* e = std::getenv("TCNN_GRID_BWD_CHUNKS"))
		if (std::atoi(e) > 0) s.grid_bwd_chunks = (uint32_t)std::atoi(e);
	if (const char* e = std::getenv("TCNN_GRID_BWD_RANGES"))
		if (std::atoi(e) > 0) s.grid_bwd_ranges = (uint32_t)std::atoi(e);
	if (const char* e = std::getenv("TCNN_GRID_BWD_PLAN")) s.grid_bwd_plan = std::string(e) == "feature" ? 1 : (std::string(e) == "range" ? 0 : -1);
	return s;
}

bool ieq(const std::string& a, const std::string& b) {
	if (a.size() != b.size()) return false;
	for (size_t i = 0; i < a.size(); ++i)
		if (std::tolower((unsigned char)a[i]) != std::tolower((unsigned char)b[i])) return false;
	return true;
}

template <typename T>
static T jval(const json& j, const char* key, T dflt) {
	auto it = j.find(key);
	if (it == j.end() || it->is_null()) return dflt;
	return it->get<T>();
}

static bool jhas(const json& j, const char* key) { return j.is_object() && j.find(key) != j.end(); }

static uint32_t powi_u32(uint32_t base, uint32_t exp) {
	uint32_t r = 1;
	for (uint32_t i = 0; i < exp; ++i) r *= base;
	return r;
}

GridEncodingHost::GridEncodingHost(uint32_t n_dims, const json& enc) {
	const std::string otype = jval<std::string>(enc, "otype", "Grid");
	const std::string default_type = ieq(otype, "TiledGrid") ? "Tiled" : (ieq(otype, "DenseGrid") ? "Dense" : "Hash");
	const uint32_t F = jval<uint32_t>(enc, "n_features_per_level", 2u);
	TCNN_CHECK(F == 1 || F == 2 || F == 4 || F == 8, "GridEncoding: n_features_per_level must be 1, 2, 4, or 8.");
	uint32_t n_feat;
	if (jhas(enc, "n_features") || jhas(enc, "n_grid_features")) {
		n_feat = jhas(enc, "n_features") ? enc["n_features"].get<uint32_t>() : enc["n_grid_features"].get<uint32_t>();
		TCNN_CHECK(!jhas(enc, "n_levels"), "GridEncoding: may not specify n_features and n_levels simultaneously (one determines the other)");
	} else {
		n_feat = F * jval<uint32_t>(enc, "n_levels", 16u);
	}
	TCNN_CHECK(n_feat % F == 0, "GridEncoding: n_features must be a multiple of n_features_per_level");
	const uint32_t L = n_feat / F;
	TCNN_CHECK(L >= 1 && L <= MAX_LEVELS, "GridEncoding: too many levels");
	const std::string type = jval<std::string>(enc, "type", default_type);
	GridType gt;
	if (ieq(type, "Hash")) gt = GridType::Hash;
	else if (ieq(type, "Dense")) gt = GridType::Dense;
	else if (ieq(type, "Tiled")) gt = GridType::Tiled;
	else throw std::runtime_error("GridEncoding: invalid grid type " + type);
	const uint32_t base = jval<uint32_t>(enc, "base_resolution", 16u);
	const float default_scale = gt == GridType::Dense ? std::exp(std::log(256.0f / (float)base) / (float)(L - 1)) : 2.0f;
	const std::string interp = jval<std::string>(enc, "interpolation", "Linear");
	const std::string hash = jval<std::string>(enc, "hash", "CoherentPrime");
	TCNN_CHECK(n_dims >= 2 && n_dims <= 4, "GridEncoding: number of input dims must be 2, 3 or 4.");

// ... 95 lines not shown
		GridBinLevel b{l, s, div_round_up(size, 1u << s), n_buckets};
		n_buckets += b.n_slices;
		acc_lds_bytes = std::max(acc_lds_bytes, (1u << s) * F * 4);
		bin_levels.push_back(b);
	}
	if (!bin_levels.empty()) {
		d_bin_levels.reserve(bin_levels.size() * sizeof(GridBinLevel));
		TCNN_HIP_CHECK(hipMemcpy(d_bin_levels.p, bin_levels.data(), bin_levels.size() * sizeof(GridBinLevel), hipMemcpyHostToDevice));
	}

	inrange_index_ok = true;
	for (const LevelInfo& li : levels) {
		uint32_t stride = 1;
		for (uint32_t d = 0; d < desc.n_pos_dims; ++d)
			if (stride <= li.size) stride *= li.res;
		uint64_t full = 1;
		for (uint32_t d = 0; d < desc.n_pos_dims; ++d) full = std::min<uint64_t>(full * li.res, 1ull << 40);
		const bool hashed = hash_grid() && li.size < stride;
		if (hashed ? (li.size & (li.size - 1)) != 0 : full > li.size) inrange_index_ok = false;
		if (li.res < 2) inrange_index_ok = false;
	}
	d_levels.reserve(levels.size() * sizeof(LevelInfo));
	TCNN_HIP_CHECK(hipMemcpy(d_levels.p, levels.data(), levels.size() * sizeof(LevelInfo), hipMemcpyHostToDevice));
	for (GridPlan& pl : plans) {
		pl.d_slices.reserve(pl.slices.size() * sizeof(GridSlice));
		TCNN_HIP_CHECK(hipMemcpy(pl.d_slices.p, pl.slices.data(), pl.slices.size() * sizeof(GridSlice), hipMemcpyHostToDevice));
	}
}

void GridEncodingHost::initialize_params(Pcg32& rng, float* out, float scale) const {
	strided_uniform(rng, n_params, out, -1e-4f * scale, 1e-4f * scale);
}

GridBinArgs GridEncodingHost::bin_args(GridBwdBufs& w, uint32_t B) const {
	GridBinArgs a{};
	a.lv = d_bin_levels.as<GridBinLevel>();
	a.n_slots = (uint32_t)bin_levels.size();
	a.n_buckets = n_buckets;
	a.pts_per_chunk = GRID_BIN_RECS >> desc.n_pos_dims;
	a.n_chunks = div_round_up(std::max(B, 1u), a.pts_per_chunk);
	a.acc_lds_bytes = acc_lds_bytes;
	if (a.n_slots) {
		w.recs.reserve((size_t)a.n_slots * a.n_chunks * GRID_BIN_RECS * sizeof(uint2));
		w.dir.reserve((size_t)a.n_buckets * a.n_chunks * sizeof(uint2));
		w.dysum.reserve((size_t)a.n_slots * a.n_chunks * desc.n_features_per_level * sizeof(float));
	}
	a.recs = w.recs.as<uint2>();
	a.dir = w.dir.as<uint2>();
	a.dysum = w.dysum.as<float>();
	return a;
}

void GridEncodingHost::backward_items(hipStream_t st, GridBwdBufs& w, uint32_t B, const float* pos, uint32_t pstride, const void* dy,
                                      int layout, uint32_t dy_stride, const GridBwdEpilogue* ep, uint32_t reserved) const {
	const uint32_t n_chunks = bwd_chunks(B, reserved);
	w.n_chunks = n_chunks;
	w.plan = plan_for(B, reserved);
	const GridPlan& pl = plans[w.plan];
	if (!pl.slices.empty()) w.partial.reserve((size_t)n_chunks * n_lds_params * 4);
	launch_grid_bwd(st, desc.n_pos_dims, desc.n_features_per_level, desc.hash_type, B, pos, pstride, dy, layout, dy_stride,
	                pl.d_slices.as<GridSlice>(), (uint32_t)pl.slices.size(), n_chunks, w.partial.as<float>(), n_lds_params, dev_levels(),
	                hash_grid(), desc.interp, ep, opts(), pl.slices.data(), levels.data(), (uint32_t)levels.size());
}

void GridEncodingHost::backward_bin(hipStream_t st, GridBwdBufs& w, uint32_t B, const float* pos, uint32_t pstride, const void* dy,
                                    int layout, uint32_t dy_stride) const {
	if (bin_levels.empty() || B == 0) return;
	const GridBinArgs a = bin_args(w, B);
	launch_grid_bin(st, desc.n_pos_dims, desc.n_features_per_level, desc.hash_type, B, pos, pstride, dy, layout, dy_stride, dev_levels(),
	                hash_grid(), desc.interp, a, opts());
}

void GridEncodingHost::backward_acc(hipStream_t st, GridBwdBufs& w, uint32_t B, const void* dy, int layout, uint32_t dy_stride,
                                    float* grad32, const GridAccAdam* adam) const {
	if (bin_levels.empty()) return;
	if (B == 0) {
		if (!adam) TCNN_HIP_CHECK(hipMemsetAsync(grad32 + n_lds_params, 0, (size_t)(n_params - n_lds_params) * 4, st));
		return;
	}
	const GridBinArgs a = bin_args(w, B);
	launch_grid_acc(st, desc.n_pos_dims, desc.n_features_per_level, B, dy, layout, dy_stride, dev_levels(), a, grad32, adam);
}

void GridEncodingHost::reduce_items(hipStream_t st, GridBwdBufs& w, float* grad32, GradFinalize fin) const {
	if (plans[0].slices.empty()) return;
	launch_grid_slab_reduce(st, w.partial.as<float>(), w.n_chunks, n_lds_params, n_lds_params, grad32, slab_map(w.plan), fin);
}

void GridEncodingHost::backward(hipStream_t st, GridBwdBufs& w, uint32_t B, const float* pos, uint32_t pstride, const void* dy,
                                int layout, uint32_t dy_stride, float* grad32) const {
	backward_items(st, w, B, pos, pstride, dy, layout, dy_stride);
	backward_bin(st, w, B, pos, pstride, dy, layout, dy_stride);
	backward_acc(st, w, B, dy, layout, dy_stride, grad32);
	reduce_items(st, w, grad32);
}

void GridEncodingHost::forward(hipStream_t st, uint32_t B, const float* pos, uint32_t pos_stride, const void* table16, void* out16,
                               bool soa, uint32_t out_stride, uint32_t aos_row_cols) const {
	launch_grid_fwd(st, desc.n_pos_dims, desc.n_features_per_level, desc.hash_type, B, desc.n_levels, pos, pos_stride, table16, out16, soa,
	                out_stride, dev_levels(), hash_grid(), desc.interp, opts(), aos_row_cols);
}

void GridEncodingHost::backward_input(hipStream_t st, uint32_t B, const float* pos, uint32_t pos_stride, const void* table16,
                                      const void* dy16, int dy_layout, uint32_t dy_stride, float* dx, uint32_t dx_stride) const {
	launch_grid_bwd_input(st, desc.n_pos_dims, desc.n_features_per_level, desc.hash_type, B, desc.n_levels, pos, pos_stride, table16, dy16,
	                      dy_layout, dy_stride, dx, dx_stride, dev_levels(), hash_grid(), desc.interp, opts());
}

void GridEncodingHost::backward_backward_input(hipStream_t st, uint32_t B, const float* pos, uint32_t pos_stride, const void* table16,
                                               const float* dL_ddLdx, const void* dy16, uint32_t dy_stride, float* grad32,
                                               void* dLddLdy16, uint32_t ddy_stride, float* dx) const {
	launch_grid_bwd_bwd(st, desc.n_pos_dims, desc.n_features_per_level, desc.hash_type, B, desc.n_levels, pos, pos_stride, table16,
	                    dL_ddLdx, dy16, dy_stride, grad32, dLddLdy16, ddy_stride, dx, dev_levels(), hash_grid(), desc.interp, opts());
}

// ... 529 lines not shown
		ws.wimage_valid = false;
		use_image = true;
	}
	launch_fused_fwd(st, mlp.width, IN, mlp.n_hidden_layers, grid->desc.n_pos_dims, grid->desc.hash_type, mlp.activation, B,
	                 use_image ? ws.wimage.p : nullptr, params16, eparams, pos, grid->dev_levels(), grid->hash_grid(), grid->desc.interp,
	                 grid->inrange_index_ok && grid->desc.interp == Interp::Linear && !sw.no_inrange_index, enc_soa, out16);
}

int NetworkHost::backward_engine_keep(bool with_dinput) const {
	if (fused_ok() && !with_dinput) return KEEP_FUSED_SOA;
	if (tile_shape_ok()) return KEEP_TILE_AOS;
	return KEEP_NONE;
}

int NetworkHost::forward_keep(hipStream_t st, StepWorkspace& ws, uint32_t B, const float* pos, const void* params16, void* out16,
                              bool with_dinput, DevBuf& keep) {
	const int layout = backward_engine_keep(with_dinput);
	const uint32_t IN = mlp.n_input;
	const void* eparams = enc_params(params16);
	if (layout == KEEP_FUSED_SOA && mlp_infer_supported(mlp.width, IN, mlp.n_hidden_layers, mlp.padded_output, mlp.activation)) {
		keep.reserve((size_t)IN * B * 2);
		fused_forward(st, ws, B, pos, params16, false, keep.p, out16);
		return KEEP_FUSED_SOA;
	}
	if (layout == KEEP_TILE_AOS && tile_infer_ok()) {
		keep.reserve((size_t)IN * B * 2);
		enc->forward_aos(st, B, pos, eparams, keep.p);
		launch_mlp_tile_infer(st, mlp.width, IN, mlp.n_hidden_layers, mlp.activation, mlp.output_activation, B, params16, keep.p, out16);
		return KEEP_TILE_AOS;
	}
	inference(st, ws, B, pos, params16, out16);
	return KEEP_NONE;
}

void NetworkHost::fwd_bwd(hipStream_t st, StepWorkspace& ws, uint32_t B, const float* pos, const float* target, uint32_t dims,
                          float loss_scale, const void* params16, const void* dout16, void* out16, float* grad32,
                          const std::function<void(int)>& mark, float* dL_dinput, const void* kept, int kept_layout) {
	if (fused_ok() && !dL_dinput)
		fwd_bwd_fused(st, ws, B, pos, target, dims, loss_scale, params16, dout16, out16, grad32, mark,
		              kept_layout == KEEP_FUSED_SOA ? kept : nullptr);
	else if (tile_shape_ok())
		fwd_bwd_tile(st, ws, B, pos, target, dims, loss_scale, params16, dout16, out16, grad32, mark, dL_dinput,
		             kept_layout == KEEP_TILE_AOS ? kept : nullptr);
	else fwd_bwd_layered(st, ws, B, pos, target, dims, loss_scale, params16, dout16, out16, grad32, mark, dL_dinput);
}

void NetworkHost::pack_weights(hipStream_t st, StepWorkspace& ws, const void* params16) {
	ws.wimage.reserve(fused_weight_image_bytes(mlp.width, mlp.n_input, mlp.n_hidden_layers));
	launch_pack_weights(st, mlp.width, mlp.n_input, mlp.n_hidden_layers, params16, ws.wimage.p);
	ws.wimage_valid = true;
}

void NetworkHost::fused_kernel(hipStream_t st, StepWorkspace& ws, uint32_t B, const float* pos, const float* target, uint32_t dims,
                               float loss_scale, const void* params16, bool pack, const void* dout16, void* out16, const void* enc_soa) {
	TCNN_CHECK(B % 32 == 0, "training: batch must be a multiple of 32");
	const uint32_t n_mlp = mlp.n_params();
	const uint32_t L = grid->desc.n_levels, F = grid->desc.n_features_per_level;
	const uint32_t nb = fused_train_n_blocks(mlp.width, mlp.n_input, mlp.n_hidden_layers, grid->desc.n_pos_dims, dims,
	                                         dout16 != nullptr, B);
	ws.n_fused_blocks = nb;
	ws.n_loss_partials = nb;
	ws.dLdenc.reserve((size_t)L * F * B * 2);
	ws.wgrad_partial.reserve((size_t)nb * n_mlp * 4);
	ws.loss_partial.reserve((size_t)nb * 4);
	ws.wimage.reserve(fused_weight_image_bytes(mlp.width, mlp.n_input, mlp.n_hidden_layers));
	bool use_image = !pack && ws.wimage_valid;
	if (!use_image && ((uintptr_t)params16 & 15)) {
		launch_pack_weights(st, mlp.width, mlp.n_input, mlp.n_hidden_layers, params16, ws.wimage.p);
		ws.wimage_valid = false;
		use_image = true;
	}
	launch_fused_train(st, mlp.width, mlp.n_input, mlp.n_hidden_layers, grid->desc.n_pos_dims, grid->desc.hash_type,
	                   mlp.activation, B, dims, loss_scale, params16, enc_params(params16), pos, target, out16, ws.dLdenc.p,
	                   ws.wgrad_partial.as<float>(), ws.loss_partial.as<float>(), grid->dev_levels(), grid->hash_grid(),
	                   grid->desc.interp, nb, dout16, use_image ? ws.wimage.p : nullptr, loss_l2,
	                   grid->inrange_index_ok && grid->desc.interp == Interp::Linear && !sw.no_inrange_index, enc_soa,
	                   dout16 ? ext_dout_scale : 1.0f);
}

void NetworkHost::grid_backward(hipStream_t st, StepWorkspace& ws, uint32_t B, const float* pos, GridBwdEpilogue* ep) {
	if (ep) {
		ep->wimage = ws.wimage.as<_Float16>();
		ep->W = mlp.width;
		ep->IN = mlp.n_input;
		ep->NH = mlp.n_hidden_layers;
		fused_image_layout(mlp.width, mlp.n_input, mlp.n_hidden_layers, &ep->RSI, &ep->RSW, &ep->oWh, &ep->oWo);
		ep->wpart = ws.wgrad_partial.as<float>();
		ep->n_wparts = ws.n_fused_blocks;
		ep->lpart = ws.loss_partial.as<float>();
	}
	grid->backward_items(st, ws.gbw, B, pos, grid->desc.n_pos_dims, ws.dLdenc.p, 0, 0, ep, ep ? ep->n_mlp_groups : 0u);
	grid->backward_bin(st, ws.gbw, B, pos, grid->desc.n_pos_dims, ws.dLdenc.p, 0, 0);
	if (ep && ep->apply_adam) ws.wimage_valid = true;
}

void NetworkHost::fwd_bwd_fused(hipStream_t st, StepWorkspace& ws, uint32_t B, const float* pos, const float* target,
                                uint32_t dims, float loss_scale, const void* params16, const void* dout16, void* out16, float* grad32,
                                const std::function<void(int)>& mark, const void* enc_soa) {
	const uint32_t n_mlp = mlp.n_params();
	fused_kernel(st, ws, B, pos, target, dims, loss_scale, params16, true, dout16, out16, enc_soa);
	if (mark) mark(1);
	GridBwdEpilogue ep{};
	ep.enabled = 1;
	ep.apply_adam = 0;
	ep.buf.g32 = grad32;
	ep.n_mlp_groups = mlp_tail_groups();
	ep.n_mlp = n_mlp;
	ws.loss_sum.reserve(16);
	ep.d_loss = ws.loss_sum.as<float>();
	TCNN_CHECK(n_mlp % 4 == 0, "network parameter count must be a multiple of 4");
	const bool fin = grad_fin.out && grid->bin_levels.empty();
	GradFinalize fin_grid{};
	if (fin) {
		ep.fin = grad_fin;
		fin_grid = grad_fin;
		fin_grid.out = (char*)grad_fin.out + (size_t)n_mlp * (grad_fin.out_f32 ? 4 : 2);
	}
	grad_fin_done = fin;
	grid_backward(st, ws, B, pos, &ep);
	grid->backward_acc(st, ws.gbw, B, ws.dLdenc.p, 0, 0, grad32 + n_mlp);
	if (mark) mark(2);
	grid->reduce_items(st, ws.gbw, grad32 + n_mlp, fin_grid);
	if (mark) mark(3);
}

void NetworkHost::fwd_bwd_tile(hipStream_t st, StepWorkspace& ws, uint32_t B, const float* pos, const float* target, uint32_t dims,
                               float loss_scale, const void* params16, const void* dout16, void* out16, float* grad32,
                               const std::function<void(int)>& mark, float* dL_dinput, const void* enc_aos) {
	TCNN_CHECK(B % 32 == 0, "training: batch must be a multiple of 32");
	const uint32_t W = mlp.width, IN = mlp.n_input, NH = mlp.n_hidden_layers;
	const uint32_t n_mlp = mlp.n_params();
	const void* eparams = enc_params(params16);
	TileGridEnc genc{};
	const bool in_kernel = !enc_aos && grid && grid->desc.n_pos_dims == 2 && grid->desc.n_features_per_level == 2 &&
	                       grid->n_to_pad == 0 && grid->desc.interp == Interp::Linear && !grid->opts().active &&
	                       tile_train_genc_ok(W, IN, NH, mlp.activation, B, grid->desc.hash_type);
	if (in_kernel) {
		genc.pos = pos;
		genc.table16 = eparams;
		genc.levels = grid->dev_levels();
		genc.hash = grid->desc.hash_type;
		genc.hash_grid = grid->hash_grid() ? 1u : 0u;
		genc.inrange = grid->opts().inrange_index;
	} else if (!enc_aos) {
// ... 154 lines not shown
	launch_cast_f32_f16(nullptr, w32.as<float>(), w16.p, n_params);
	ws.wimage_valid = false;
	TCNN_HIP_CHECK(hipDeviceSynchronize());
}

void TrainerHost::training_step(hipStream_t st, uint32_t B, const float* input, const float* target, bool run_optimizer) {
	TCNN_CHECK(B % BATCH_GRANULARITY == 0, "training_step: batch size must be a multiple of 256");
	if (timer.enabled) {
		timer.sampling = (timer.counter++ % timer.every) == 0;
		if (timer.sampling) timer.marks.push_back({-1, -1, -1, -1, -1});
	}
	if (run_optimizer && use_graph && !(timer.enabled && timer.sampling) && !adam.adabound && training_step_graph(st, B, input, target))
		return;
	if (run_optimizer) {
		step_eager(st, B, input, target);
		return;
	}
	if (overlapped_ok()) {
		training_step_overlapped(st, B, input, target, false);
		return;
	}
	training_step_sequential(st, B, input, target, false);
}

void TrainerHost::step_eager(hipStream_t st, uint32_t B, const float* input, const float* target) {
	if (dp) training_step_dp(st, B, input, target);
	else if (peer_attached) training_step_peer(st, B, input, target);
	else if (overlapped_ok()) training_step_overlapped(st, B, input, target, true);
	else training_step_sequential(st, B, input, target, true);
}

void TrainerHost::training_step_sequential(hipStream_t st, uint32_t B, const float* input, const float* target, bool run_optimizer) {
	mark(st, 0);
	model->fwd_bwd(st, ws, B, input, target, n_output_dims, loss_scale, w16.p, nullptr, nullptr, g32.as<float>(),
	               [&](int ph) { mark(st, ph); });
	launch_sum(st, ws.loss_partial.as<float>(), ws.n_loss_partials, d_loss.as<float>());
	mark(st, 4);
	last_B = B;
	if (run_optimizer) optimizer_step(st);
}


void TrainerHost::training_step_overlapped(hipStream_t st, uint32_t B, const float* input, const float* target, bool run_optimizer,
                                           float* grad_out, bool skip_reduce) {
	NetworkHost& m = *model;
	float* const gsum = (grad_out && !run_optimizer) ? grad_out : g32.as<float>();
	mark(st, 0);
	const void* enc_soa = nullptr;
	if (m.sw.split_encode) {
		ws.enc16.reserve((size_t)m.mlp.n_input * B * 2);
		m.grid->forward(st, B, input, m.grid->desc.n_pos_dims, m.enc_params(w16.p), ws.enc16.p, true, 0);
		enc_soa = ws.enc16.p;
	}
	m.fused_kernel(st, ws, B, input, target, n_output_dims, loss_scale, w16.p, false, nullptr, nullptr, enc_soa);
	mark(st, 1);
	if (run_optimizer) ++adam_step;
	GridBwdEpilogue ep{};
	ep.enabled = 1;
	ep.apply_adam = run_optimizer ? 1 : 0;
	ep.adam_mlp = run_optimizer ? adam_args_table(st, adam_step) : adam_args();
	ep.adam_mlp.n = (uint32_t)n_mlp;
	ep.buf = AdamBuffers{w32.as<float>(), w16.as<_Float16>(), gsum, g16.as<_Float16>(), m1.as<float>(), m2.as<float>(),
	                     steps.as<uint32_t>()};
	ep.n_mlp_groups = mlp_tail_groups();
	ep.n_mlp = (uint32_t)n_mlp;
	ep.d_loss = d_loss.as<float>();
	TCNN_CHECK(n_mlp % 4 == 0, "network parameter count must be a multiple of 4");
	m.grid_backward(st, ws, B, input, &ep);
	GridEncodingHost& g = *m.grid;
	if (run_optimizer) {
		GridAccAdam ga{};
		ga.a = adam_args_table(st, adam_step);
		ga.buf = ep.buf;
		ga.param_base = (uint32_t)n_mlp;
		ga.write_grad32 = 0;
		g.backward_acc(st, ws.gbw, B, ws.dLdenc.p, 0, 0, g32.as<float>() + n_mlp, &ga);
		mark(st, 2);
		AdamArgs ag = adam_args_table(st, adam_step);
		ag.n = (uint32_t)n_mlp + g.n_lds_params;
		ag.begin = (uint32_t)n_mlp;
		ag.part = ws.gbw.partial.as<float>();
		ag.n_parts = ws.gbw.n_chunks;
		ag.part_stride = g.n_lds_params;
		ag.part_map = g.slab_map(ws.gbw.plan);
		if (!g.plans[0].slices.empty())
			launch_adam(st, ag, w32.as<float>(), w16.p, g32.as<float>(), g16.p, m1.as<float>(), m2.as<float>(), steps.as<uint32_t>());
	} else {
		g.backward_acc(st, ws.gbw, B, ws.dLdenc.p, 0, 0, gsum + n_mlp);
		mark(st, 2);
		if (!skip_reduce) g.reduce_items(st, ws.gbw, gsum + n_mlp);
	}
	mark(st, 3);
	last_B = B;
}

struct TrainerHost::StepGraph {
	static constexpr size_t MAX_GRAPHS = 8;
	hipStream_t cs = nullptr;
	hipEvent_t e0 = nullptr, e1 = nullptr;
	std::vector<std::pair<std::vector<uint64_t>, hipGraphExec_t>> execs;
	StepGraph() {
		TCNN_HIP_CHECK(hipStreamCreateWithFlags(&cs, hipStreamNonBlocking));
		TCNN_HIP_CHECK(hipEventCreateWithFlags(&e0, hipEventDisableTiming));
		TCNN_HIP_CHECK(hipEventCreateWithFlags(&e1, hipEventDisableTiming));
	}
	~StepGraph() {
		for (auto& e : execs) (void)hipGraphExecDestroy(e.second);
		(void)hipEventDestroy(e0);
		(void)hipEventDestroy(e1);
		(void)hipStreamDestroy(cs);
	}
	hipGraphExec_t find(const std::vector<uint64_t>& key) {
		for (size_t i = 0; i < execs.size(); ++i)
			if (execs[i].first == key) {
				auto e = execs[i];
				execs.erase(execs.begin() + i);
				execs.push_back(e);
				return e.second;
			}
		return nullptr;
	}
};

TrainerHost::~TrainerHost() {
	if (graph) (void)hipDeviceSynchronize();
}

void TrainerHost::set_graph(bool on) {
	if (!on && graph) {
		TCNN_HIP_CHECK(hipDeviceSynchronize());
		graph.reset();
	}
	use_graph = on;
}

std::vector<uint64_t> TrainerHost::graph_key(uint32_t B, const float* input, const float* target) const {
	std::vector<uint64_t> k = {B, (uint64_t)(uintptr_t)input, (uint64_t)(uintptr_t)target, (uint64_t)ftable_valid,
	                           (uint64_t)(uintptr_t)w32.p, (uint64_t)(uintptr_t)w16.p, (uint64_t)(uintptr_t)g16.p,
	                           (uint64_t)(uintptr_t)g32.p, (uint64_t)(uintptr_t)m1.p, (uint64_t)(uintptr_t)m2.p,
	                           (uint64_t)(uintptr_t)steps.p, (uint64_t)(uintptr_t)d_loss.p, (uint64_t)(uintptr_t)d_ftable.p,
	                           (uint64_t)(uintptr_t)ws.dLdenc.p, (uint64_t)(uintptr_t)ws.wgrad_partial.p,
	                           (uint64_t)(uintptr_t)ws.loss_partial.p, (uint64_t)(uintptr_t)ws.wimage.p,
	                           (uint64_t)(uintptr_t)ws.gbw.partial.p, (uint64_t)(uintptr_t)ws.gbw.recs.p,
	                           (uint64_t)(uintptr_t)ws.gbw.dir.p, (uint64_t)(uintptr_t)ws.gbw.dysum.p, ws.n_fused_blocks,
	                           ws.gbw.n_chunks, (uint64_t)overlapped_ok(), (uint64_t)(uintptr_t)dp, (uint64_t)dp_sharded, dp_per,
	                           (uint64_t)(uintptr_t)ws.enc16.p, (uint64_t)(uintptr_t)ws.acts.p, (uint64_t)(uintptr_t)ws.delta0.p,
	                           (uint64_t)(uintptr_t)ws.delta1.p, (uint64_t)(uintptr_t)ws.dout16.p, (uint64_t)(uintptr_t)ws.out16.p,
	                           (uint64_t)(uintptr_t)ws.red_tmp.p, (uint64_t)(uintptr_t)ws.tile_wT.p, (uint64_t)(uintptr_t)ws.loss_sum.p,
	                           ws.n_loss_partials, (uint64_t)(uintptr_t)peer.get(), (uint64_t)peer_attached};
	const AdamArgs a = adam_args();
	const size_t n = sizeof(AdamArgs) / 8 + 1;
	std::vector<uint64_t> ab(n, 0);
	std::memcpy(ab.data(), &a, sizeof(AdamArgs));
	k.insert(k.end(), ab.begin(), ab.end());
	const GridOpts o = model->grid ? model->grid->opts() : GridOpts{};
	uint32_t ml = 0;
	std::memcpy(&ml, &o.max_level, 4);
	k.insert(k.end(), {(uint64_t)ml, (uint64_t)(uintptr_t)o.max_level_gpu, o.stochastic, o.n_features, o.active, o.inrange_index});
	uint32_t ls = 0, gs = 0;
	std::memcpy(&ls, &loss_scale, 4);
	std::memcpy(&gs, &grad_scale, 4);
	k.insert(k.end(), {(uint64_t)ls, (uint64_t)gs});
	return k;
}

bool TrainerHost::training_step_graph(hipStream_t st, uint32_t B, const float* input, const float* target) {
	const bool image_step = overlapped_ok() && !dp && !peer_attached;
	if (adam_step + 1 >= GRAPH_STEPS || (image_step && !ws.wimage_valid)) return false;
	if (peer_attached) peer_check();
	if (ftable_valid < GRAPH_STEPS || ftable_b1 != adam.beta1 || ftable_b2 != adam.beta2)
		(void)adam_args_table(st, GRAPH_STEPS, GRAPH_STEPS);
	if (!graph) graph = std::make_unique<StepGraph>();
	std::vector<uint64_t> key = graph_key(B, input, target);
	hipGraphExec_t exec = graph->find(key);
	if (!exec) {
		step_eager(st, B, input, target);
		key = graph_key(B, input, target);
		TCNN_HIP_CHECK(hipStreamSynchronize(st));
		TCNN_HIP_CHECK(hipStreamSynchronize(graph->cs));
		if (graph->execs.size() >= StepGraph::MAX_GRAPHS) {
			(void)hipGraphExecDestroy(graph->execs.front().second);
			graph->execs.erase(graph->execs.begin());
		}
		const uint32_t step0 = adam_step, ftv0 = ftable_valid, lb0 = last_B;
		const bool wv0 = ws.wimage_valid, dps0 = dp_state_partial;
		hipGraph_t g = nullptr;
		const bool tim = timer.enabled;
		timer.enabled = false;
		TCNN_HIP_CHECK(hipStreamBeginCapture(graph->cs, hipStreamCaptureModeThreadLocal));
		step_eager(graph->cs, B, input, target);
		TCNN_HIP_CHECK(hipStreamEndCapture(graph->cs, &g));
		timer.enabled = tim;
		adam_step = step0;
		ftable_valid = ftv0;
// ... 45 lines not shown
	for (auto& m : timer.marks) {
		for (uint32_t p = 0; p < P; ++p) {
			if (m[p] < 0 || m[p + 1] < 0) continue;
			float t = 0.0f;
			TCNN_HIP_CHECK(hipEventElapsedTime(&t, timer.pool[m[p]], timer.pool[m[p + 1]]));
			ms[p] += t;
			++cnt[p];
		}
	}
	for (uint32_t p = 0; p < P; ++p)
		if (cnt[p]) ms[p] /= cnt[p];
	if (n_steps) *n_steps = P ? cnt[0] : 0;
	timer.enabled = false;
	timer.reset();
}

AdamArgs TrainerHost::adam_args() const {
	AdamArgs a{};
	a.n = (uint32_t)n_params;
	a.n_matrix = (uint32_t)n_mlp;
	a.loss_scale = loss_scale;
	a.grad_scale = grad_scale;
	a.lr = adam.learning_rate;
	a.beta1 = adam.beta1;
	a.beta2 = adam.beta2;
	a.eps = adam.epsilon;
	a.l2_reg = adam.l2_reg;
	a.rel_decay = adam.relative_decay;
	a.abs_decay = adam.absolute_decay;
	a.clip = adam.clipping_magnitude;
	a.nonmat_lr_factor = adam.non_matrix_learning_rate_factor;
	a.lower_lr_bound = 0.0f;
	a.upper_lr_bound = std::numeric_limits<float>::max();
	if (adam.adabound) {
		a.lower_lr_bound = 0.1f - 0.1f / ((1 - adam.beta2) * (float)adam_step + 1);
		a.upper_lr_bound = 0.1f + 0.1f / ((1 - adam.beta2) * (float)adam_step);
	}
	a.opt_matrix = adam.optimize_matrix_params;
	a.opt_nonmatrix = adam.optimize_non_matrix_params;
	int e = 0;
	a.inv_loss_scale = (std::frexp(loss_scale, &e) == 0.5f) ? 1.0f / loss_scale : 0.0f;
	return a;
}

void TrainerHost::training_step_part(hipStream_t st, uint32_t B, const float* input, const float* target, int part) {
	TCNN_CHECK(B % BATCH_GRANULARITY == 0, "training_step: batch size must be a multiple of 256");
	TCNN_CHECK(part == 0 || part == 1, "training_step_part: part must be 0 or 1");
	NetworkHost& m = *model;
	if (!overlapped_ok()) {
		if (part == 0) training_step(st, B, input, target, false);
		return;
	}
	if (part == 0) {
		m.fused_kernel(st, ws, B, input, target, n_output_dims, loss_scale, w16.p, false);
		launch_column_sums(st, ws.wgrad_partial.as<float>(), ws.n_fused_blocks, (uint32_t)n_mlp, g32.as<float>());
		launch_sum(st, ws.loss_partial.as<float>(), ws.n_loss_partials, d_loss.as<float>());
		last_B = B;
		return;
	}
	TCNN_CHECK(last_B == B, "training_step_part: part 1 must follow part 0 of the same batch");
	m.grid_backward(st, ws, B, input);
	m.grid->backward_acc(st, ws.gbw, B, ws.dLdenc.p, 0, 0, g32.as<float>() + n_mlp);
	m.grid->reduce_items(st, ws.gbw, g32.as<float>() + n_mlp);
}

AdamArgs TrainerHost::adam_args_table(hipStream_t st, uint32_t upto, uint32_t reserve) {
	AdamArgs a = adam_args();
	if (ftable_b1 != adam.beta1 || ftable_b2 != adam.beta2) {
		ftable_valid = 0;
		ftable_b1 = adam.beta1;
		ftable_b2 = adam.beta2;
	}
	if (std::max(upto, reserve) > ftable_cap) {
		ftable_cap = std::max((std::max(upto, reserve) + 1023u) / 1024u * 1024u, std::max(1024u, 2 * ftable_cap));
		TCNN_HIP_CHECK(hipStreamSynchronize(st));
		d_ftable.reserve((size_t)ftable_cap * 4);
		ftable_valid = 0;
	}
	if (std::max(upto, reserve) > ftable_valid) {
		const uint32_t ahead = std::min(ftable_cap, (std::max(upto, reserve) + 1023u) / 1024u * 1024u);
		h_ftable.resize(ahead);
		for (uint32_t t = ftable_valid + 1; t <= ahead; ++t)
			h_ftable[t - 1] = std::sqrt(1.0f - std::pow(adam.beta2, (float)t)) / (1.0f - std::pow(adam.beta1, (float)t));
		TCNN_HIP_CHECK(hipMemcpyAsync(d_ftable.as<float>() + ftable_valid, h_ftable.data() + ftable_valid, (size_t)(ahead - ftable_valid) * 4,
		                              hipMemcpyHostToDevice, st));
		TCNN_HIP_CHECK(hipStreamSynchronize(st));
		ftable_valid = ahead;
	}
	a.factor_table = d_ftable.as<float>();
	a.factor_n = ftable_valid;
	return a;
}

void TrainerHost::optimizer_step(hipStream_t st) {
	++adam_step;
	const AdamArgs a = adam_args_table(st, adam_step);
	launch_adam(st, a, w32.as<float>(), w16.p, g32.as<float>(), g16.p, m1.as<float>(), m2.as<float>(), steps.as<uint32_t>());
	ws.wimage_valid = false;
}

std::unique_ptr<TrainerFwdCtx> TrainerHost::forward(hipStream_t st, uint32_t B, const float* input, const float* target, const float* pdf,
                                                    const void* ext_dLdy16, bool prep_dinput, const float* perturbation) {
	TCNN_CHECK(B % BATCH_GRANULARITY == 0, "forward: batch size must be a multiple of 256");
	TCNN_CHECK(ext_dLdy16 || target, "forward: a target (or an external dL/dy) is required");
	NetworkHost& m = *model;
	const uint32_t OUTP = m.mlp.padded_output;
	auto c = std::make_unique<TrainerFwdCtx>();
// ... 68 lines not shown
```

### neuralbtf-tiny-cuda-nn_amd/csrc/runtime.h

```cpp
#pragma once

#include <json.hpp>

#include <array>
#include <cstdlib>
#include <functional>
#include <memory>
#include <string>
#include <vector>

#include "common.h"
#include "grid_device.h"
#include "kernels.h"

namespace tcnn_amd {

using json = nlohmann::json;

struct Pcg32 {
	uint64_t state = 0x853c49e6748fea9bULL, inc = 0xda3e39cb94b95bdbULL;
	Pcg32() = default;
	explicit Pcg32(uint64_t initstate, uint64_t initseq = 1u) { seed(initstate, initseq); }
	void seed(uint64_t initstate, uint64_t initseq = 1u);
	uint32_t next_uint();
	float next_float();
	void advance(int64_t delta);
};

struct DevBuf {
	void* p = nullptr;
	size_t bytes = 0;
	DevBuf() = default;
	DevBuf(const DevBuf&) = delete;
	DevBuf& operator=(const DevBuf&) = delete;
	~DevBuf();
	void reserve(size_t n);
	void release();
	template <typename T> T* as() const { return (T*)p; }
};

bool ieq(const std::string& a, const std::string& b);

struct GridBwdBufs {
	DevBuf partial, recs, dir, dysum;
	uint32_t n_chunks = 0;
	int plan = 0;
};
struct GridPlan {
	std::vector<GridSlice> slices;
	DevBuf d_slices;
	bool identity = true;
	GridPlan() = default;
	GridPlan& operator=(const GridPlan& o) {
		slices = o.slices;
		identity = o.identity;
		return *this;
	}
};
enum : int { PLAN_RANGE = 0, PLAN_FEATURE = 1 };

struct EngineSwitches {
	bool no_fused_grid = false;
	bool no_tile_engine = false;
	bool no_inrange_index = false;
	bool split_encode = false;
	bool no_forward_keep = false;
	bool split_forward = false;
	bool grid_bin_all = false;
	uint32_t grid_bwd_chunks = 0;
	uint32_t grid_bwd_ranges = 0;
	int grid_bwd_plan = -1;
	static EngineSwitches from_env();
};

struct GridEncodingHost {
	EngineSwitches sw = EngineSwitches::from_env();
	GridDesc desc{};
	uint32_t n_features = 0;
	uint32_t n_to_pad = 0;
	uint32_t n_params = 0;
	bool stochastic = false;
	float max_level = 1000.0f;
	const float* max_level_gpu = nullptr;
	std::vector<LevelInfo> levels;
	GridPlan plans[2];
	uint32_t first_binned = 0;
	bool inrange_index_ok = false;
	uint32_t n_lds_params = 0;
	std::vector<GridBinLevel> bin_levels;
	uint32_t n_buckets = 0, acc_lds_bytes = 0;
	DevBuf d_levels, d_slab_map, d_bin_levels;

	GridEncodingHost(uint32_t n_dims_to_encode, const json& enc);
	uint32_t padded_output_width() const { return n_features + n_to_pad; }
	void set_alignment(uint32_t a) { n_to_pad = (n_features + a - 1) / a * a - n_features; }
	bool hash_grid() const { return desc.grid_type == GridType::Hash; }
	void initialize_params(Pcg32& rng, float* host_out, float scale = 1.0f) const;
	json hyperparams() const;
	const LevelInfo* dev_levels() const { return d_levels.as<LevelInfo>(); }
	GridOpts opts() const {
		GridOpts o;
		o.max_level = max_level;
		o.max_level_gpu = max_level_gpu;
		o.stochastic = stochastic ? 1u : 0u;
		o.n_features = n_features;
		const float t = (max_level * (float)n_features) / (float)desc.n_features_per_level + 1e-3f;
		o.active = (stochastic || max_level_gpu || (float)(desc.n_levels - 1) >= t) ? 1u : 0u;
		o.inrange_index = (inrange_index_ok && desc.interp == Interp::Linear && !sw.no_inrange_index) ? 1u : 0u;
		return o;
	}
	const GridSlabMap* slab_map(int plan) const { return plans[plan].identity ? nullptr : d_slab_map.as<GridSlabMap>(); }
	int plan_for(uint32_t B, uint32_t reserved = 0) const {
		if (sw.grid_bwd_plan >= 0) return sw.grid_bwd_plan;
		const uint32_t n_items = (uint32_t)plans[PLAN_RANGE].slices.size();
		return (uint64_t)bwd_chunks(B, reserved) * n_items + reserved <= 256 ? PLAN_RANGE : PLAN_FEATURE;
	}
	uint32_t bwd_chunks(uint32_t B, uint32_t reserved = 0) const {
		const std::vector<GridSlice>& slices = plans[PLAN_RANGE].slices;
		if (slices.empty()) return 1;
		const uint32_t n_cu = 256;
		const uint32_t fit = (n_cu > reserved ? n_cu - reserved : 1u) / (uint32_t)slices.size();
		uint32_t c = std::max(1u, fit > 2 ? fit - 1 : fit);
		c = std::max(c, (B + GRID_BWD_REG_POINTS - 1) / GRID_BWD_REG_POINTS);
		if (sw.grid_bwd_chunks) return std::max(1u, std::min(std::min(sw.grid_bwd_chunks, 32u), B / 1024));
		return std::max(1u, std::min(std::min(c, 32u), B / 8192));
	}
	GridBinArgs bin_args(GridBwdBufs& w, uint32_t B) const;
	void backward_items(hipStream_t st, GridBwdBufs& w, uint32_t B, const float* pos, uint32_t pstride, const void* dy, int layout,
	                    uint32_t dy_stride, const GridBwdEpilogue* ep = nullptr, uint32_t reserved = 0) const;
	void backward_bin(hipStream_t st, GridBwdBufs& w, uint32_t B, const float* pos, uint32_t pstride, const void* dy, int layout,
	                  uint32_t dy_stride) const;
	void backward_acc(hipStream_t st, GridBwdBufs& w, uint32_t B, const void* dy, int layout, uint32_t dy_stride, float* grad32,
	                  const GridAccAdam* adam = nullptr) const;
	void reduce_items(hipStream_t st, GridBwdBufs& w, float* grad32, GradFinalize fin = {}) const;
	void backward(hipStream_t st, GridBwdBufs& w, uint32_t B, const float* pos, uint32_t pstride, const void* dy, int layout,
	              uint32_t dy_stride, float* grad32) const;
	void forward(hipStream_t st, uint32_t B, const float* pos, uint32_t pos_stride, const void* table16, void* out16, bool soa,
	             uint32_t out_stride, uint32_t aos_row_cols = 0) const;
	void backward_input(hipStream_t st, uint32_t B, const float* pos, uint32_t pos_stride, const void* table16, const void* dy16,
	                    int dy_layout, uint32_t dy_stride, float* dx, uint32_t dx_stride) const;
	void backward_backward_input(hipStream_t st, uint32_t B, const float* pos, uint32_t pos_stride, const void* table16,
	                             const float* dL_ddLdx, const void* dy16, uint32_t dy_stride, float* grad32, void* dLddLdy16,
	                             uint32_t ddy_stride, float* dx) const;

	GridPlan plan_f32;
	void build_plan_f32();
	uint32_t bwd_chunks_f32(uint32_t B) const {
		const uint32_t n_items = std::max<uint32_t>(1u, (uint32_t)plan_f32.slices.size());
		return std::max(1u, std::min(std::min(std::max(256u / n_items, 1u), 32u), B / 8192));
	}
	void forward_f32(hipStream_t st, uint32_t B, const float* pos, uint32_t pos_stride, const float* table32, float* out32,
	                 uint32_t out_stride) const;
	void backward_f32(hipStream_t st, GridBwdBufs& w, uint32_t B, const float* pos, uint32_t pstride, const float* dy32, uint32_t dy_stride,
	                  float* grad32) const;
	void backward_input_f32(hipStream_t st, uint32_t B, const float* pos, uint32_t pos_stride, const float* table32, const float* dy32,
	                        uint32_t dy_stride, float* dx, uint32_t dx_stride) const;
	void backward_backward_input_f32(hipStream_t st, uint32_t B, const float* pos, uint32_t pos_stride, const float* table32,
	                                 const float* dL_ddLdx, const float* dy32, uint32_t dy_stride, float* grad32, float* dLddLdy32,
	                                 uint32_t ddy_stride, float* dx) const;
};

struct MlpHost {
	uint32_t width = 64, n_input = 32, n_hidden_layers = 2, n_output = 16, padded_output = 16;
	int activation = 1, output_activation = 0;
	std::string otype = "FullyFusedMLP";
	MlpHost() = default;
	MlpHost(uint32_t n_input_dims, uint32_t n_output_dims, const json& net);
	uint32_t n_params() const {
		return n_hidden_layers == 0 ? padded_output * n_input
		                            : width * n_input + (n_hidden_layers - 1) * width * width + padded_output * width;
	}
	void initialize_params(Pcg32& rng, float* host_out, float scale = 1.0f) const;
	json hyperparams() const;
};

struct AdamHost {
	float learning_rate = 1e-3f, beta1 = 0.9f, beta2 = 0.999f, epsilon = 1e-8f, l2_reg = 1e-8f;
	float relative_decay = 0.0f, absolute_decay = 0.0f, clipping_magnitude = 0.0f, non_matrix_learning_rate_factor = 1.0f;
	bool adabound = false, optimize_matrix_params = true, optimize_non_matrix_params = true;
	void update(const json& p);
	json hyperparams() const;
};
// ... 3 lines not shown
	bool f32 = false;

	struct Part {
		uint32_t kind = 0;
		uint32_t in_col = 0, n_in = 0, out_col = 0, width = 0, n_values = 0;
		uint32_t p0 = 0;
		float f0 = 1.0f, f1 = 0.0f;
		uint32_t param_offset = 0;
		std::unique_ptr<GridEncodingHost> grid;
		std::unique_ptr<GridBwdBufs> bufs;
		bool f32 = false;
		uint32_t required_alignment() const { return grid ? grid->desc.n_features_per_level : 1u; }
		bool own_kernel() const { return kind == COMP_GRID || kind == COMP_ONEBLOB || kind == COMP_IDENTITY; }
		json hyperparams() const;
		void forward(hipStream_t st, uint32_t B, const float* x, uint32_t x_stride, const void* params16, void* out16, uint32_t stride,
		             bool alone) const;
		void backward_input(hipStream_t st, uint32_t B, const float* x, uint32_t x_stride, const void* params16, const void* dy16,
		                    int dy_layout, uint32_t stride, float* dx) const;
	};
	std::vector<Part> parts;
	std::string otype;
	CompTable table{};
	uint32_t n_grid_params = 0;

	EncodingHost(uint32_t n_dims_to_encode, const json& enc, bool fp32 = false);
	static bool known(const std::string& otype);
	static bool is_grid_otype(const std::string& otype);
	const Part* lone_part() const { return otype != "Composite" && parts[0].own_kernel() ? &parts[0] : nullptr; }
	GridEncodingHost* lone_grid() const { return lone_part() ? parts[0].grid.get() : nullptr; }
	uint32_t padded_output_width() const { return parts.empty() ? 0u : parts.back().out_col + parts.back().width; }
	void set_alignment(uint32_t a) { layout(a); }
	uint32_t n_params() const { return n_grid_params; }
	void initialize_params(Pcg32& rng, float* host_out, float scale = 1.0f) const;
	json hyperparams() const;
	std::string name() const { return otype + "Encoding"; }
	void forward_aos(hipStream_t st, uint32_t B, const float* x, const void* params16, void* out16) const;
	int dy_layout() const {
		const GridEncodingHost* g = lone_grid();
		return !f32 && g && g->desc.n_features_per_level == 2 && g->n_to_pad == 0 ? 0 : 2;
	}
	void backward_input(hipStream_t st, uint32_t B, const float* x, const void* dy16, float* dx, const void* params16 = nullptr,
	                    int dy_layout = 2) const;
	void backward_params(hipStream_t st, uint32_t B, const float* x, const void* dy16, int dy_layout, float* grad32) const;

private:
	void parse_composite(const json& enc);
	void add_part(uint32_t n_in, uint32_t in_col, const json& enc);
	void layout(uint32_t alignment);
	void build_table();
};

struct StepWorkspace {
	DevBuf dLdenc, wgrad_partial, loss_partial, grad32_tmp, out16, enc16, wimage;
	GridBwdBufs gbw;
	DevBuf acts, delta0, delta1, dout16, red_tmp;
	DevBuf tile_wT;
	DevBuf loss_sum;
	uint32_t n_fused_blocks = 0, n_loss_partials = 0;
	bool wimage_valid = false;
};

struct NetworkHost {
	EngineSwitches sw = EngineSwitches::from_env();
	float ext_dout_scale = 1.0f;
	GradFinalize grad_fin{};
	bool grad_fin_done = false;
	std::unique_ptr<EncodingHost> enc;
	GridEncodingHost* grid = nullptr;
	MlpHost mlp;
	uint32_t n_input_dims = 0, n_output_dims = 0;
	uint32_t loss_l2 = 0;
	NetworkHost(uint32_t n_in, uint32_t n_out, const json& enc, const json& net);
	uint64_t n_params() const { return (uint64_t)mlp.n_params() + enc->n_params(); }
	const void* enc_params(const void* params16) const { return (const uint8_t*)params16 + (size_t)mlp.n_params() * 2; }
	bool fused_ok() const;
	bool tile_shape_ok() const;
	bool tile_ok() const;
	bool tile_infer_ok() const;
	bool layered_ok() const;
	const char* engine() const { return (fused_ok() || tile_ok()) ? "fused" : layered_ok() ? "layered" : "unsupported"; }
	const char* inference_engine() const;
	void initialize_params(Pcg32& rng, float* host_out, float scale = 1.0f) const;

	void inference(hipStream_t st, StepWorkspace& ws, uint32_t B, const float* pos, const void* params16, void* out16,
	               bool trust_image = false);
	enum : int { KEEP_NONE = 0, KEEP_FUSED_SOA = 1, KEEP_TILE_AOS = 2 };
	int backward_engine_keep(bool with_dinput) const;
	void fused_forward(hipStream_t st, StepWorkspace& ws, uint32_t B, const float* pos, const void* params16, bool use_image, void* enc_soa,
	                   void* out16);
	int forward_keep(hipStream_t st, StepWorkspace& ws, uint32_t B, const float* pos, const void* params16, void* out16, bool with_dinput,
	                 DevBuf& keep);
	void fwd_bwd(hipStream_t st, StepWorkspace& ws, uint32_t B, const float* pos, const float* target, uint32_t dims,
	             float loss_scale, const void* params16, const void* dout16, void* out16, float* grad32,
	             const std::function<void(int)>& mark = nullptr, float* dL_dinput = nullptr, const void* kept = nullptr,
	             int kept_layout = KEEP_NONE);
	json hyperparams() const;

	void fused_kernel(hipStream_t st, StepWorkspace& ws, uint32_t B, const float* pos, const float* target, uint32_t dims,
	                  float loss_scale, const void* params16, bool pack, const void* dout16 = nullptr, void* out16 = nullptr,
	                  const void* enc_soa = nullptr);
	void grid_backward(hipStream_t st, StepWorkspace& ws, uint32_t B, const float* pos, GridBwdEpilogue* ep = nullptr);
	void pack_weights(hipStream_t st, StepWorkspace& ws, const void* params16);

private:
	void fwd_bwd_fused(hipStream_t st, StepWorkspace& ws, uint32_t B, const float* pos, const float* target, uint32_t dims,
	                   float loss_scale, const void* params16, const void* dout16, void* out16, float* grad32,
	                   const std::function<void(int)>& mark, const void* enc_soa);
	void fwd_bwd_tile(hipStream_t st, StepWorkspace& ws, uint32_t B, const float* pos, const float* target, uint32_t dims,
	                  float loss_scale, const void* params16, const void* dout16, void* out16, float* grad32,
	                  const std::function<void(int)>& mark, float* dL_dinput, const void* enc_aos);
	void fwd_bwd_layered(hipStream_t st, StepWorkspace& ws, uint32_t B, const float* pos, const float* target, uint32_t dims,
	                     float loss_scale, const void* params16, const void* dout16, void* out16, float* grad32,
	                     const std::function<void(int)>& mark, float* dL_dinput);
	void forward_layers(hipStream_t st, StepWorkspace& ws, uint32_t B, const void* params16, void* out16, bool keep);
};

struct PhaseTimer {
	static constexpr int N_PHASES = 4;
	bool enabled = false;
	uint32_t every = 1, counter = 0;
	bool sampling = false;
	std::vector<hipEvent_t> pool;
	std::vector<std::array<int, N_PHASES + 1>> marks;
	size_t next = 0;
	hipEvent_t get();
	void reset() { next = 0; marks.clear(); }
	~PhaseTimer();
};

struct DpComm {
	void* comm = nullptr;
	int nranks = 1, rank = 0;
	hipStream_t cs = nullptr;
	hipEvent_t ev[3] = {nullptr, nullptr, nullptr};
	DpComm(const void* unique_id, int nranks, int rank);
	~DpComm();
	DpComm(const DpComm&) = delete;
	DpComm& operator=(const DpComm&) = delete;
	void all_reduce_f32(float* buf, size_t n, hipStream_t st);
	void reduce_scatter_f32(float* buf, size_t per, hipStream_t st);
	void all_gather(void* buf, size_t per_elems, int elem_bytes, hipStream_t st);
};
void dp_unique_id(void* id128);

struct TrainerFwdCtx {
	uint32_t B = 0;
	DevBuf keep;
	int layout = 0;
	DevBuf out16, dLdy16, lpart;
	DevBuf pert16;
	const void* ext = nullptr;
	uint32_t n_lpart = 0;
	const void* dLdy() const { return ext ? ext : dLdy16.p; }
// ... 94 lines not shown
```

Before: 11700 training steps/s (2^18-sample batches, whole job).

## Emit per-slice dy bounds from fused kernel to stream grid backward dy loads

```diff
diff --git a/neuralbtf-tiny-cuda-nn_amd/csrc/capi.cpp b/neuralbtf-tiny-cuda-nn_amd/csrc/capi.cpp
--- a/neuralbtf-tiny-cuda-nn_amd/csrc/capi.cpp
+++ b/neuralbtf-tiny-cuda-nn_amd/csrc/capi.cpp
@@ -1,5 +1,6 @@
 #include "../../include/tcnn_mi355x.h"
 #include "debug_api.h"
+#include "debug_grid_bwd.h"
 
 #include <algorithm>
 #include <cstring>
@@ -749,6 +750,46 @@
 	});
 }
 
+int tcnn_debug_grid_bwd_count_fallbacks(int on) {
+	return guard([&] { grid_bwd_debug_count_fallbacks(on != 0); });
+}
+int tcnn_debug_grid_bwd_fallbacks(uint32_t* count) {
+	return guard([&] { *count = grid_bwd_debug_fallbacks(); });
+}
+int tcnn_debug_step_dldenc(tcnn_trainer* t, void* host_dldenc, size_t dldenc_bytes, float* host_bound, size_t bound_bytes,
+                           int* bound_live) {
+	return guard([&] {
+		auto& ws = t->t->ws;
+		TCNN_HIP_CHECK(hipDeviceSynchronize());
+		TCNN_CHECK(dldenc_bytes <= ws.dLdenc.bytes, "debug: dL/d(encoding) read past the workspace");
+		TCNN_HIP_CHECK(hipMemcpy(host_dldenc, ws.dLdenc.p, dldenc_bytes, hipMemcpyDeviceToHost));
+		*bound_live = ws.dy_bound_live ? 1 : 0;
+		if (ws.dy_bound_live) {
+			TCNN_CHECK(bound_bytes <= ws.dy_bound.bytes, "debug: slice sums read past the workspace");
+			TCNN_HIP_CHECK(hipMemcpy(host_bound, ws.dy_bound.p, bound_bytes, hipMemcpyDeviceToHost));
+		}
+	});
+}
+int tcnn_debug_grid_backward_items(tcnn_trainer* t, void* stream, uint32_t n, const float* input, const void* dldy_pairs,
+                                   const float* dy_bound, float* host_slabs, size_t slab_floats, uint32_t* n_chunks,
+                                   uint32_t* slab_stride) {
+	return guard([&] {
+		auto& tr = *t->t;
+		TCNN_CHECK(tr.model->grid != nullptr, "debug: trainer model has no grid encoding");
+		TCNN_CHECK(n % 32 == 0, "debug: batch must be a multiple of 32");
+		GridEncodingHost& g = *tr.model->grid;
+		hipStream_t st = (hipStream_t)stream;
+		GridBwdBufs w;
+		g.backward_items(st, w, n, input, g.desc.n_pos_dims, dldy_pairs, 0, 0, nullptr, 0, dy_bound);
+		TCNN_HIP_CHECK(hipStreamSynchronize(st));
+		*n_chunks = w.n_chunks;
+		*slab_stride = g.n_lds_params;
+		const size_t nfl = (size_t)w.n_chunks * g.n_lds_params;
+		TCNN_CHECK(nfl <= slab_floats, "debug: slab buffer too small");
+		TCNN_HIP_CHECK(hipMemcpy(host_slabs, w.partial.p, nfl * 4, hipMemcpyDeviceToHost));
+	});
+}
+
 int tcnn_debug_hfma(void* stream, const void* a, const void* b, const void* c, void* out, uint32_t n_pairs) {
 	return guard([&] { launch_probe_hfma((hipStream_t)stream, a, b, c, out, n_pairs); });
 }
diff --git a/neuralbtf-tiny-cuda-nn_amd/csrc/debug_grid_bwd.h b/neuralbtf-tiny-cuda-nn_amd/csrc/debug_grid_bwd.h
--- /dev/null
+++ b/neuralbtf-tiny-cuda-nn_amd/csrc/debug_grid_bwd.h
@@ -0,0 +1,19 @@
+#ifndef TCNN_DEBUG_GRID_BWD_H
+#define TCNN_DEBUG_GRID_BWD_H
+#include "../../include/tcnn_mi355x.h"
+#ifdef __cplusplus
+extern "C" {
+#endif
+
+int tcnn_debug_grid_bwd_count_fallbacks(int on);
+int tcnn_debug_grid_bwd_fallbacks(uint32_t* count);
+int tcnn_debug_step_dldenc(tcnn_trainer* t, void* host_dldenc, size_t dldenc_bytes, float* host_bound, size_t bound_bytes,
+                           int* bound_live);
+int tcnn_debug_grid_backward_items(tcnn_trainer* t, void* stream, uint32_t n, const float* input, const void* dldy_pairs,
+                                   const float* dy_bound, float* host_slabs, size_t slab_floats, uint32_t* n_chunks,
+                                   uint32_t* slab_stride);
+
+#ifdef __cplusplus
+}
+#endif
+#endif
diff --git a/neuralbtf-tiny-cuda-nn_amd/csrc/dp.cpp b/neuralbtf-tiny-cuda-nn_amd/csrc/dp.cpp
--- a/neuralbtf-tiny-cuda-nn_amd/csrc/dp.cpp
+++ b/neuralbtf-tiny-cuda-nn_amd/csrc/dp.cpp
@@ -132,7 +132,7 @@
 	float* g = g32.as<float>();
 	mark(st, 0);
 	if (overlapped_ok()) {
-		m.fused_kernel(st, ws, B, input, target, n_output_dims, loss_scale, w16.p, false);
+		m.fused_kernel(st, ws, B, input, target, n_output_dims, loss_scale, w16.p, false, nullptr, nullptr, nullptr, true);
 		launch_column_sums(st, ws.wgrad_partial.as<float>(), ws.n_fused_blocks, (uint32_t)n_mlp, g);
 		launch_sum(st, ws.loss_partial.as<float>(), ws.n_loss_partials, d_loss.as<float>());
 		if (!dp_sharded) {
diff --git a/neuralbtf-tiny-cuda-nn_amd/csrc/fused.hip b/neuralbtf-tiny-cuda-nn_amd/csrc/fused.hip
--- a/neuralbtf-tiny-cuda-nn_amd/csrc/fused.hip
+++ b/neuralbtf-tiny-cuda-nn_amd/csrc/fused.hip
@@ -116,7 +116,7 @@
                         const float* pos, const float* target, void* out16, void* dLdenc_pairs,
                         float* wgrad_partial, float* loss_partial, const LevelInfo* levels, bool hash_grid,
                         Interp interp, uint32_t n_blocks, const void* dout16, const void* wimage, uint32_t loss_l2,
-                        bool inrange_index, const void* enc16, float dout_scale) {
+                        bool inrange_index, const void* enc16, float dout_scale, float* dy_bound) {
 	TCNN_CHECK(B % 32 == 0, "fused train: batch must be a multiple of 32");
 	TCNN_CHECK(wimage || ((uintptr_t)params16 & 15) == 0, "fused train: parameters must be 16-byte aligned");
 	FusedTrainArgs a;
@@ -142,6 +142,8 @@
 	a.hash_grid = hash_grid ? 1u : 0u;
 	a.interp = (uint32_t)interp;
 	a.prof = nullptr;
+	TCNN_CHECK(!dy_bound || (!dout16 && !enc16), "fused train: slice sums only with the loss inside and the encoding gathered");
+	a.dy_bound = dy_bound;
 #define X(w, in, nh) if (W == w && IN == in && NH == nh) { launch_fused_shape<w, in, nh>(st, D, h, act, a, n_blocks); return; }
 	TCNN_FUSED_SHAPES(X)
 #undef X
diff --git a/neuralbtf-tiny-cuda-nn_amd/csrc/grid.hip b/neuralbtf-tiny-cuda-nn_amd/csrc/grid.hip
--- a/neuralbtf-tiny-cuda-nn_amd/csrc/grid.hip
+++ b/neuralbtf-tiny-cuda-nn_amd/csrc/grid.hip
@@ -591,6 +591,17 @@
 
 uint32_t grid_bwd_slot_budget() { return GRID_BWD_SLOTS; }
 
+static DevBufLite g_fallbacks;
+static bool g_count_fallbacks = false;
+void grid_bwd_debug_count_fallbacks(bool on) { g_count_fallbacks = on; }
+uint32_t grid_bwd_debug_fallbacks() {
+	uint32_t n = 0;
+	if (!g_fallbacks.p) return 0;
+	TCNN_HIP_CHECK(hipDeviceSynchronize());
+	TCNN_HIP_CHECK(hipMemcpy(&n, g_fallbacks.p, 4, hipMemcpyDeviceToHost));
+	return n;
+}
+
 extern template void grid_bwd_f<2>(hipStream_t, uint32_t, HashType, int, uint32_t, dim3, size_t, uint32_t, const float*, uint32_t,
                                    const _Float16*, const GridSlice*, float*, uint32_t, const LevelInfo*, uint32_t, uint32_t, uint32_t,
                                    const GridBwdLaunch&);
@@ -605,7 +616,7 @@
                      uint32_t pos_stride, const void* dLdy16, int dy_layout, uint32_t dy_stride, const GridSlice* slices,
                      uint32_t n_slices, uint32_t n_chunks, float* partial, uint32_t partial_stride,
                      const LevelInfo* levels, bool hash_grid, Interp interp, const GridBwdEpilogue* ep, const GridOpts& go,
-                     const GridSlice* host_slices, const LevelInfo* host_levels, uint32_t n_levels) {
+                     const GridSlice* host_slices, const LevelInfo* host_levels, uint32_t n_levels, const float* dy_bound) {
 	const uint32_t n_tail = (ep && ep->enabled) ? ep->n_mlp_groups : 0u;
 	if (n_tail == 0 && (n_slices == 0 || B == 0)) return;
 	if (B == 0) n_slices = 0;
@@ -617,6 +628,12 @@
 	else gl.ep.enabled = 0;
 	gl.dbg_times = nullptr;
 	gl.opts = go;
+	gl.dy_bound = dy_layout == 0 ? dy_bound : nullptr;
+	gl.fallback_count = nullptr;
+	if (g_count_fallbacks) {
+		gl.fallback_count = (uint32_t*)g_fallbacks.get(4);
+		TCNN_HIP_CHECK(hipMemsetAsync(gl.fallback_count, 0, 4, st));
+	}
 	gl.tb.n_items = gl.tb.n_levels = 0;
 	if (host_slices && host_levels && n_slices <= GRID_BWD_ARG_ITEMS && n_levels <= GRID_BWD_ARG_LEVELS) {
 		gl.tb.n_items = n_slices;
diff --git a/neuralbtf-tiny-cuda-nn_amd/csrc/grid_bwd_lds.h b/neuralbtf-tiny-cuda-nn_amd/csrc/grid_bwd_lds.h
--- a/neuralbtf-tiny-cuda-nn_amd/csrc/grid_bwd_lds.h
+++ b/neuralbtf-tiny-cuda-nn_amd/csrc/grid_bwd_lds.h
@@ -8,6 +8,7 @@
 #include <vector>
 
 #include "adam_device.h"
+#include "grid_bwd_scale.h"
 #include "grid_device.h"
 
 namespace tcnn_amd {
@@ -163,8 +164,18 @@
 	}
 }
 
-template <uint32_t D, uint32_t F, HashType H, int KIND, int MODE>
-__device__ __forceinline__ void grid_bwd_points_regs(const uint32_t (&dyb)[GRID_BWD_PR], const float (&xs0)[GRID_BWD_PU][D],
+__device__ __forceinline__ void load_dy_batch(const uint32_t* __restrict__ dy_lv, uint32_t i0, uint32_t i1, uint32_t k,
+                                              uint32_t (&dst)[GRID_BWD_PU]) {
+#pragma unroll
+	for (uint32_t u = 0; u < GRID_BWD_PU; ++u) {
+		const uint32_t i = i0 + threadIdx.x + (k * GRID_BWD_PU + u) * blockDim.x;
+		dst[u] = i < i1 ? dy_lv[i] : 0u;
+	}
+}
+
+template <uint32_t D, uint32_t F, HashType H, int KIND, int MODE, bool STREAM = false>
+__device__ __forceinline__ void grid_bwd_points_regs(const uint32_t (&dyb)[STREAM ? GRID_BWD_PU : GRID_BWD_PR],
+                                                     const float (&xs0)[GRID_BWD_PU][D], const uint32_t* __restrict__ dy_lv,
                                                      uint32_t B, const float* __restrict__ pos,
                                                      uint32_t pstride, uint32_t level, const LevelInfo& li, bool hash_grid,
                                                      Interp interp, uint32_t begin, uint32_t len, uint32_t f0, uint32_t nf,
@@ -173,14 +184,24 @@
 	constexpr bool FAST_KIND = D == 2 && (KIND == IDX_HASH_POW2 || KIND == IDX_DENSE || KIND == IDX_HASH_RANGE);
 	const bool fast = FAST_KIND && interp == Interp::Linear && (begin == 0 || KIND == IDX_HASH_RANGE);
 	float xs[2][U][D];
-#pragma unroll
-	for (uint32_t u = 0; u < U; ++u)
+	uint32_t ds[2][STREAM ? U : 1];
+#pragma unroll
+	for (uint32_t u = 0; u < U; ++u) {
 #pragma unroll
 		for (uint32_t d = 0; d < D; ++d) xs[0][u][d] = xs0[u][d];
+		if constexpr (STREAM) ds[0][u] = dyb[u];
+	}
+	auto dy_bits = [&](uint32_t k, uint32_t u) -> uint32_t {
+		if constexpr (STREAM) return ds[k & 1][u];
+		else return dyb[k * U + u];
+	};
 #pragma unroll
 	for (uint32_t k = 0; k < NB; ++k) {
 		if (i0 + threadIdx.x + k * U * blockDim.x >= i1) break;
-		if (k + 1 < NB) load_pos_batch<D>(pos, pstride, i0, i1, k + 1, xs[(k + 1) & 1]);
+		if (k + 1 < NB) {
+			load_pos_batch<D>(pos, pstride, i0, i1, k + 1, xs[(k + 1) & 1]);
+			if constexpr (STREAM) load_dy_batch(dy_lv, i0, i1, k + 1, ds[(k + 1) & 1]);
+		}
 		bool fast_b = fast;
 		if constexpr (FAST_KIND && KIND == IDX_DENSE) {
 			bool inr = true;
@@ -195,10 +216,9 @@
 				if (i0 + threadIdx.x + (k * U + U - 1) * blockDim.x < i1) {
 #pragma unroll
 					for (uint32_t u = 0; u < U; ++u) {
-						const uint32_t p = k * U + u;
 						float dy[F];
 #pragma unroll
-						for (uint32_t f = 0; f < F; ++f) dy[f] = dy_bits_feature(dyb[p], f) * scale;
+						for (uint32_t f = 0; f < F; ++f) dy[f] = dy_bits_feature(dy_bits(k, u), f) * scale;
 						accum_point_2d_fast<F, H, KIND, MODE>(*(const float(*)[2]) & xs[k & 1][u][0], dy, li, f0, nf, acc, begin, len);
 					}
 				} else {
@@ -208,7 +228,7 @@
 						if (i0 + threadIdx.x + p * blockDim.x >= i1) break;
 						float dy[F];
 #pragma unroll
-						for (uint32_t f = 0; f < F; ++f) dy[f] = dy_bits_feature(dyb[p], f) * scale;
+						for (uint32_t f = 0; f < F; ++f) dy[f] = dy_bits_feature(dy_bits(k, u), f) * scale;
 						accum_point_2d_fast<F, H, KIND, MODE>(*(const float(*)[2]) & xs[k & 1][u][0], dy, li, f0, nf, acc, begin, len);
 					}
 				}
@@ -222,7 +242,7 @@
 			if (i >= i1) break;
 			float dy[F];
 #pragma unroll
-			for (uint32_t f = 0; f < F; ++f) dy[f] = dy_bits_feature(dyb[p], f) * scale;
+			for (uint32_t f = 0; f < F; ++f) dy[f] = dy_bits_feature(dy_bits(k, u), f) * scale;
 			accum_point<D, F, H, KIND, MODE, false>(xs[k & 1][u], dy, i, level, B, li, hash_grid, interp, begin, len, f0, nf, acc, o);
 		}
 	}
@@ -307,9 +327,9 @@
                                                    uint32_t begin, uint32_t len, uint32_t f0, uint32_t nf, uint32_t i0, uint32_t i1,
                                                    float scale, int* acc, const GridOpts& o) {
 	if constexpr (F == 2) {
-		if (mode == 0) { grid_bwd_points_regs<D, F, H, KIND, 0>(dyb, xs0, B, pos, pstride, level, li, hash_grid, interp, begin, len, f0, nf, i0, i1, scale, acc, o); return; }
-	}
-	grid_bwd_points_regs<D, F, H, KIND, 1>(dyb, xs0, B, pos, pstride, level, li, hash_grid, interp, begin, len, f0, nf, i0, i1, scale, acc, o);
+		if (mode == 0) { grid_bwd_points_regs<D, F, H, KIND, 0>(dyb, xs0, nullptr, B, pos, pstride, level, li, hash_grid, interp, begin, len, f0, nf, i0, i1, scale, acc, o); return; }
+	}
+	grid_bwd_points_regs<D, F, H, KIND, 1>(dyb, xs0, nullptr, B, pos, pstride, level, li, hash_grid, interp, begin, len, f0, nf, i0, i1, scale, acc, o);
 }
 
 __device__ __forceinline__ void grid_bwd_mlp_tail(const GridBwdEpilogue& ep, uint32_t g, float* lds) {
@@ -364,7 +384,8 @@
 	int layout, uint32_t B, const float* __restrict__ pos, uint32_t pstride, const _Float16* __restrict__ dLdy, uint32_t dy_stride,
 	const GridSlice* __restrict__ items, float* __restrict__ partial, uint32_t partial_stride,
 	const LevelInfo* __restrict__ levels, uint32_t hash_grid, uint32_t interp_u, uint32_t pts_per_chunk, uint32_t n_items,
-	uint32_t n_chunks, const GridBwdEpilogue ep, unsigned long long* dbg_times, const GridOpts o, const GridBwdTables tb) {
+	uint32_t n_chunks, const GridBwdEpilogue ep, unsigned long long* dbg_times, const GridOpts o, const GridBwdTables tb,
+	const float* __restrict__ dy_bound, uint32_t* fallback_count) {
 	extern __shared__ __attribute__((aligned(16))) int acc[];
 	const unsigned long long t_start = dbg_times ? wall_clock64() : 0ull;
 	__shared__ float red[GRID_BWD_THREADS / 64];
@@ -393,22 +414,9 @@
 	const uint32_t i0 = chunk * pts_per_chunk;
 	const uint32_t i1 = min(B, i0 + pts_per_chunk);
 
-	float m = 0.0f;
 	constexpr bool REGS_OK = D == 2 && F <= 2 && !OPTS;
 	const uint32_t n_pts = i1 > i0 ? i1 - i0 : 0u;
 	const bool use_regs = REGS_OK && n_pts <= GRID_BWD_THREADS * GRID_BWD_PR;
-	uint32_t dyb[GRID_BWD_PR];
-	float xs0[GRID_BWD_PU][D];
-	if constexpr (REGS_OK) {
-		if (use_regs) {
-#pragma unroll
-			for (uint32_t p = 0; p < GRID_BWD_PR; ++p) {
-				const uint32_t i = i0 + threadIdx.x + p * blockDim.x;
-				dyb[p] = i < i1 ? load_dy_bits<F>(layout, dLdy, dy_stride, it.level, B, i) : 0u;
-			}
-			load_pos_batch<D>(pos, pstride, i0, i1, 0, xs0);
-		}
-	}
 	LevelInfo li;
 	if (it.level < tb.n_levels) {
 		li.scale = tb.levels[it.level].scale;
@@ -421,10 +429,81 @@
 	const uint32_t slots = len * nf;
 	const uint32_t R = max(1u, min(16u, GRID_BWD_SLOTS / max(slots, 1u)));
 	const uint32_t nz = R * slots;
-	for (uint32_t j = 4 * threadIdx.x; j + 4 <= nz; j += 4 * blockDim.x) *(int4*)(acc + j) = int4{0, 0, 0, 0};
-	for (uint32_t j = nz / 4 * 4 + threadIdx.x; j < nz; j += blockDim.x) acc[j] = 0;
-	if (dbg_times && threadIdx.x == 0) dbg_times[8 * blockIdx.x + 6] = wall_clock64();
 	int* acc_w = acc + ((threadIdx.x >> 6) % R) * slots;
+	auto zero_acc = [&] {
+		for (uint32_t j = 4 * threadIdx.x; j + 4 <= nz; j += 4 * blockDim.x) *(int4*)(acc + j) = int4{0, 0, 0, 0};
+		for (uint32_t j = nz / 4 * 4 + threadIdx.x; j < nz; j += blockDim.x) acc[j] = 0;
+		if (dbg_times && threadIdx.x == 0) dbg_times[8 * blockIdx.x + 6] = wall_clock64();
+	};
+	auto item_kind = [&] {
+		uint64_t full = 1;
+		for (uint32_t d = 0; d < D; ++d) full = full * li.res > 0xffffffffull ? 0x100000000ull : full * li.res;
+		const bool whole = it.begin == 0 && len == li.size;
+		int kind = IDX_GENERIC;
+		if (whole && full <= li.size) kind = IDX_DENSE;
+		else if (whole && hash_grid && (li.size & (li.size - 1)) == 0) kind = IDX_HASH_POW2;
+		else if (!whole && hash_grid && (li.size & (li.size - 1)) == 0 && full > li.size) kind = IDX_HASH_RANGE;
+		return kind;
+	};
+	const int mode = nf < F ? 1 : (F == 2 ? 0 : 2);
+	const float P = (float)(i1 > i0 ? i1 - i0 : 1u);
+	int e = 0;
+	bool finite = true;
+
+	constexpr bool STREAM_OK = D == 2 && F == 2 && !OPTS;
+	bool stream = false;
+	if constexpr (STREAM_OK) {
+		const uint32_t n_sl = n_pts / 32u;
+		if (dy_bound && layout == 0 && nf == F && use_regs && n_pts > 0 && ((i0 | i1) & 31u) == 0 && n_sl <= GRID_BWD_THREADS) {
+			float mh = threadIdx.x < n_sl ? dy_bound[(size_t)it.level * (B / 32u) + i0 / 32u + threadIdx.x] : 0.0f;
+			const uint32_t* dy_lv = (const uint32_t*)dLdy + (size_t)it.level * B;
+			uint32_t ds0[GRID_BWD_PU];
+			float xs0[GRID_BWD_PU][D];
+			load_dy_batch(dy_lv, i0, i1, 0, ds0);
+			load_pos_batch<D>(pos, pstride, i0, i1, 0, xs0);
+			zero_acc();
+#pragma unroll
+			for (int o2 = 32; o2 > 0; o2 >>= 1) mh += __shfl_xor(mh, o2);
+			if ((threadIdx.x & 63) == 0) red[threadIdx.x >> 6] = mh;
+			__syncthreads();
+			mh = red[0];
+#pragma unroll
+			for (uint32_t w = 1; w < GRID_BWD_THREADS / 64; ++w) mh += red[w];
+			stream = grid_bwd_scale_guard(mh, P, D);
+			if (stream) {
+				e = grid_bwd_scale_exp(mh, P, D);
+				const float scale = ldexpf(1.0f, e);
+				if (dbg_times && threadIdx.x == 0) dbg_times[8 * blockIdx.x + 5] = dbg_times[8 * blockIdx.x + 1] = wall_clock64();
+				const int kind = item_kind();
+				if (kind == IDX_HASH_POW2)
+					grid_bwd_points_regs<D, F, H, IDX_HASH_POW2, 0, true>(ds0, xs0, dy_lv, B, pos, pstride, it.level, li, hash_grid != 0, interp, it.begin, len, f0, nf, i0, i1, scale, acc_w, o);
+				else if (kind == IDX_HASH_RANGE)
+					grid_bwd_points_regs<D, F, H, IDX_HASH_RANGE, 0, true>(ds0, xs0, dy_lv, B, pos, pstride, it.level, li, hash_grid != 0, interp, it.begin, len, f0, nf, i0, i1, scale, acc_w, o);
+				else if (kind == IDX_DENSE)
+					grid_bwd_points_regs<D, F, H, IDX_DENSE, 0, true>(ds0, xs0, dy_lv, B, pos, pstride, it.level, li, hash_grid != 0, interp, it.begin, len, f0, nf, i0, i1, scale, acc_w, o);
+				else
+					grid_bwd_points_regs<D, F, H, IDX_GENERIC, 0, true>(ds0, xs0, dy_lv, B, pos, pstride, it.level, li, hash_grid != 0, interp, it.begin, len, f0, nf, i0, i1, scale, acc_w, o);
+			} else {
+				if (fallback_count && threadIdx.x == 0) atomicAdd(fallback_count, 1u);
+				__syncthreads();
+			}
+		}
+	}
+	if (!stream) {
+	float m = 0.0f;
+	uint32_t dyb[GRID_BWD_PR];
+	float xs0[GRID_BWD_PU][D];
+	if constexpr (REGS_OK) {
+		if (use_regs) {
+#pragma unroll
+			for (uint32_t p = 0; p < GRID_BWD_PR; ++p) {
+				const uint32_t i = i0 + threadIdx.x + p * blockDim.x;
+				dyb[p] = i < i1 ? load_dy_bits<F>(layout, dLdy, dy_stride, it.level, B, i) : 0u;
+			}
+			load_pos_batch<D>(pos, pstride, i0, i1, 0, xs0);
+		}
+	}
+	zero_acc();
 	if constexpr (REGS_OK) {
 		if (use_regs) {
 #pragma unroll
@@ -469,25 +548,11 @@
 	m = red[0];
 #pragma unroll
 	for (uint32_t w = 1; w < GRID_BWD_THREADS / 64; ++w) m += red[w];
-	const float P = (float)(i1 > i0 ? i1 - i0 : 1u);
-	const bool finite = __builtin_isfinite(m);
-	int e = 0;
-	if (m > 0.0f && finite) {
-		const float lim = (2147483647.0f - (float)(1u << D) * P) / (m * 1.01f);
-		e = ilogbf(lim);
-		e = max(-126, min(e, 100));
-	}
+	finite = __builtin_isfinite(m);
+	e = grid_bwd_scale_exp(m, P, D);
 	const float scale = ldexpf(1.0f, e);
 	if (dbg_times && threadIdx.x == 0) dbg_times[8 * blockIdx.x + 1] = wall_clock64();
-
-	uint64_t full = 1;
-	for (uint32_t d = 0; d < D; ++d) full = full * li.res > 0xffffffffull ? 0x100000000ull : full * li.res;
-	const bool whole = it.begin == 0 && len == li.size;
-	int kind = IDX_GENERIC;
-	if (whole && full <= li.size) kind = IDX_DENSE;
-	else if (whole && hash_grid && (li.size & (li.size - 1)) == 0) kind = IDX_HASH_POW2;
-	else if (!whole && hash_grid && (li.size & (li.size - 1)) == 0 && full > li.size) kind = IDX_HASH_RANGE;
-	const int mode = nf < F ? 1 : (F == 2 ? 0 : 2);
+	const int kind = item_kind();
 	if constexpr (REGS_OK) {
 		if (use_regs) {
 			if (kind == IDX_HASH_POW2)
@@ -509,6 +574,7 @@
 		grid_bwd_mode<D, F, H, IDX_DENSE, OPTS>(mode, layout, B, pos, pstride, dLdy, dy_stride, it.level, li, hash_grid != 0, interp, it.begin, len, f0, nf, i0, i1, scale, acc_w, o);
 	else
 		grid_bwd_mode<D, F, H, IDX_GENERIC, OPTS>(mode, layout, B, pos, pstride, dLdy, dy_stride, it.level, li, hash_grid != 0, interp, it.begin, len, f0, nf, i0, i1, scale, acc_w, o);
+	}
 	}
 	__syncthreads();
 	if (dbg_times && threadIdx.x == 0) dbg_times[8 * blockIdx.x + 2] = wall_clock64();
@@ -574,6 +640,8 @@
 	unsigned long long* dbg_times;
 	GridOpts opts;
 	GridBwdTables tb;
+	const float* dy_bound;
+	uint32_t* fallback_count;
 };
 
 template <uint32_t D, uint32_t F, HashType H>
@@ -585,10 +653,10 @@
 	set_dyn_lds((const void*)k_grid_bwd_lds<D, F, H, true>, (int)GRID_BWD_LDS_BYTES, done1);
 	if (gl.opts.active)
 		hipLaunchKernelGGL((k_grid_bwd_lds<D, F, H, true>), g, dim3(GRID_BWD_THREADS), lds, st, layout, B, pos, ps, dy, dys, sl, part, pstr, lv, hg, in,
-		                   ppc, gl.n_items, gl.n_chunks, gl.ep, gl.dbg_times, gl.opts, gl.tb);
+		                   ppc, gl.n_items, gl.n_chunks, gl.ep, gl.dbg_times, gl.opts, gl.tb, gl.dy_bound, gl.fallback_count);
 	else
 		hipLaunchKernelGGL((k_grid_bwd_lds<D, F, H, false>), g, dim3(GRID_BWD_THREADS), lds, st, layout, B, pos, ps, dy, dys, sl, part, pstr, lv, hg, in,
-		                   ppc, gl.n_items, gl.n_chunks, gl.ep, gl.dbg_times, gl.opts, gl.tb);
+		                   ppc, gl.n_items, gl.n_chunks, gl.ep, gl.dbg_times, gl.opts, gl.tb, gl.dy_bound, gl.fallback_count);
 }
 
 template <uint32_t D, uint32_t F>
diff --git a/neuralbtf-tiny-cuda-nn_amd/csrc/grid_bwd_scale.h b/neuralbtf-tiny-cuda-nn_amd/csrc/grid_bwd_scale.h
--- /dev/null
+++ b/neuralbtf-tiny-cuda-nn_amd/csrc/grid_bwd_scale.h
@@ -0,0 +1,41 @@
+#pragma once
+
+#include <cmath>
+#include <cstdint>
+#include <cstring>
+
+#if defined(__HIPCC__) || defined(__CUDACC__)
+#define TCNN_SCALE_HD __host__ __device__ __forceinline__
+#else
+#define TCNN_SCALE_HD inline
+#endif
+
+namespace tcnn_amd {
+
+TCNN_SCALE_HD float grid_bwd_scale_lim(float m, float P, uint32_t D) {
+	return (2147483647.0f - (float)(1u << D) * P) / (m * 1.01f);
+}
+
+TCNN_SCALE_HD int grid_bwd_scale_exp(float m, float P, uint32_t D) {
+	int e = 0;
+	if (m > 0.0f && std::isfinite(m)) {
+		e = ilogbf(grid_bwd_scale_lim(m, P, D));
+		e = e < 100 ? e : 100;
+		e = e > -126 ? e : -126;
+	}
+	return e;
+}
+
+constexpr uint32_t GRID_BWD_GUARD_BITS = 1u << 9;
+TCNN_SCALE_HD bool grid_bwd_scale_guard(float mh, float P, uint32_t D) {
+	if (!std::isfinite(mh)) return false;
+	if (!(mh > 0.0f)) return true;
+	const float lim = grid_bwd_scale_lim(mh, P, D);
+	uint32_t b;
+	memcpy(&b, &lim, 4);
+	const uint32_t ex = (b >> 23) & 0xffu, mant = b & 0x7fffffu;
+	if (ex == 0u || ex == 0xffu) return false;
+	return mant >= GRID_BWD_GUARD_BITS && mant <= 0x800000u - 2u * GRID_BWD_GUARD_BITS;
+}
+
+}
diff --git a/neuralbtf-tiny-cuda-nn_amd/csrc/kernels.h b/neuralbtf-tiny-cuda-nn_amd/csrc/kernels.h
--- a/neuralbtf-tiny-cuda-nn_amd/csrc/kernels.h
+++ b/neuralbtf-tiny-cuda-nn_amd/csrc/kernels.h
@@ -113,7 +113,8 @@
                         float* wgrad_partial, float* loss_partial, const LevelInfo* levels, bool hash_grid,
                         Interp interp, uint32_t n_blocks, const void* dout16, const void* wimage, uint32_t loss_l2 = 0, bool inrange_index = false,
                         const void* enc16 = nullptr,
-                        float dout_scale = 1.0f);
+                        float dout_scale = 1.0f,
+                        float* dy_bound = nullptr);
 size_t fused_weight_image_bytes(uint32_t W, uint32_t IN, uint32_t NH);
 void launch_pack_weights(hipStream_t st, uint32_t W, uint32_t IN, uint32_t NH, const void* params16, void* image);
 
@@ -136,7 +137,10 @@
                      uint32_t n_slices, uint32_t n_chunks, float* partial, uint32_t partial_stride,
                      const LevelInfo* levels, bool hash_grid, Interp interp, const GridBwdEpilogue* ep = nullptr,
                      const GridOpts& opts = GridOpts{}, const GridSlice* host_slices = nullptr, const LevelInfo* host_levels = nullptr,
-                     uint32_t n_levels = 0);
+                     uint32_t n_levels = 0,
+                     const float* dy_bound = nullptr);
+void grid_bwd_debug_count_fallbacks(bool on);
+uint32_t grid_bwd_debug_fallbacks();
 void launch_grid_bin(hipStream_t st, uint32_t D, uint32_t F, HashType h, uint32_t B, const float* pos, uint32_t pos_stride,
                      const void* dLdy16, int dy_layout, uint32_t dy_stride, const LevelInfo* levels, bool hash_grid, Interp interp,
                      const GridBinArgs& a, const GridOpts& opts = GridOpts{});
diff --git a/neuralbtf-tiny-cuda-nn_amd/csrc/mlp_fused.h b/neuralbtf-tiny-cuda-nn_amd/csrc/mlp_fused.h
--- a/neuralbtf-tiny-cuda-nn_amd/csrc/mlp_fused.h
+++ b/neuralbtf-tiny-cuda-nn_amd/csrc/mlp_fused.h
@@ -259,7 +259,26 @@
 	float dout_scale;
 	const _Float16* enc;
 	unsigned long long* prof;
+	float* dy_bound;
 };
+
+__device__ __forceinline__ float dy_pair_bound(uint32_t w) {
+	const uint32_t m = w & 0x7fff7fffu;
+	const uint32_t b = min(max(m >> 16, m & 0xffffu), 0x7c00u);
+	return (float)__builtin_bit_cast(_Float16, (uint16_t)b);
+}
+
+template <int CTRL>
+__device__ __forceinline__ float dpp_row_perm(float v) {
+	return __builtin_bit_cast(float, __builtin_amdgcn_update_dpp(0, __builtin_bit_cast(int, v), CTRL, 0xf, 0xf, true));
+}
+__device__ __forceinline__ float row_sum16(float v) {
+	v += dpp_row_perm<0xB1>(v);
+	v += dpp_row_perm<0x4E>(v);
+	v += dpp_row_perm<0x141>(v);
+	v += dpp_row_perm<0x140>(v);
+	return v;
+}
 
 __device__ __forceinline__ unsigned long long stamp() {
 	unsigned long long t;
@@ -376,7 +395,7 @@
 	}
 }
 
-template <int W, int IN, int NH, Act ACT, bool EXT_DOUT, bool PROF, class TargetFn, class AfterLossFn>
+template <int W, int IN, int NH, Act ACT, bool EXT_DOUT, bool PROF, bool EMIT_BOUND, class TargetFn, class AfterLossFn>
 __device__ __forceinline__ void fused_slice(const FusedTrainArgs& a, uint32_t base, int c, int q, const h4 (&xt)[2][IN / 16],
                                             TargetFn target, AfterLossFn after_loss, const h4 (&Gext)[2], const _Float16* sW0,
                                             const _Float16* sWh, const _Float16* sWo, _Float16* bufA, _Float16* bufD,
@@ -481,10 +500,21 @@
 		const h4 d1 = __builtin_convertvector(acc1, h4);
 		const uint32_t lv = 8 * u + 2 * q;
 		const uint32_t i0 = base + c, i1 = base + 16 + c;
-		a.dLdenc[(size_t)lv * a.B + i0] = __builtin_bit_cast(uint32_t, h2{d0[0], d0[1]});
-		a.dLdenc[(size_t)(lv + 1) * a.B + i0] = __builtin_bit_cast(uint32_t, h2{d0[2], d0[3]});
-		a.dLdenc[(size_t)lv * a.B + i1] = __builtin_bit_cast(uint32_t, h2{d1[0], d1[1]});
-		a.dLdenc[(size_t)(lv + 1) * a.B + i1] = __builtin_bit_cast(uint32_t, h2{d1[2], d1[3]});
+		const uint32_t w00 = __builtin_bit_cast(uint32_t, h2{d0[0], d0[1]}), w01 = __builtin_bit_cast(uint32_t, h2{d0[2], d0[3]});
+		const uint32_t w10 = __builtin_bit_cast(uint32_t, h2{d1[0], d1[1]}), w11 = __builtin_bit_cast(uint32_t, h2{d1[2], d1[3]});
+		a.dLdenc[(size_t)lv * a.B + i0] = w00;
+		a.dLdenc[(size_t)(lv + 1) * a.B + i0] = w01;
+		a.dLdenc[(size_t)lv * a.B + i1] = w10;
+		a.dLdenc[(size_t)(lv + 1) * a.B + i1] = w11;
+		if constexpr (EMIT_BOUND) if (a.dy_bound) {
+			const float b0 = row_sum16(dy_pair_bound(w00) + dy_pair_bound(w10));
+			const float b1 = row_sum16(dy_pair_bound(w01) + dy_pair_bound(w11));
+			if (c == 0) {
+				const uint32_t ns = a.B / 32u, sl = base / 32u;
+				a.dy_bound[(size_t)lv * ns + sl] = b0;
+				a.dy_bound[(size_t)(lv + 1) * ns + sl] = b1;
+			}
+		}
 	}
 	if constexpr (PROF) { t1 = stamp(); ph[5] += t1 - t0; t0 = t1; }
 }
@@ -757,7 +787,7 @@
 		if constexpr (PROF) { t1 = stamp(); ph[0] += t1 - t0; t0 = t1; }
 		auto target = [&](int tau, int r, uint32_t o) { return r == 0 ? tg[tau] : a.target[(size_t)(base + 16 * tau + c) * a.dims + o]; };
 		auto after_loss = [] {};
-		fused_slice<W, IN, NH, ACT, EXT_DOUT, PROF>(a, base, c, q, xt, target, after_loss, Gext, smem + L::oW0,
+		fused_slice<W, IN, NH, ACT, EXT_DOUT, PROF, !EXT_DOUT && !ENC_MEM && !PROF>(a, base, c, q, xt, target, after_loss, Gext, smem + L::oW0,
 		                                            smem + L::oWh, smem + L::oWo, bufA, bufD, acc, ph, t0);
 	}
 	if (image_pending) {
diff --git a/neuralbtf-tiny-cuda-nn_amd/csrc/runtime.cpp b/neuralbtf-tiny-cuda-nn_amd/csrc/runtime.cpp
--- a/neuralbtf-tiny-cuda-nn_amd/csrc/runtime.cpp
+++ b/neuralbtf-tiny-cuda-nn_amd/csrc/runtime.cpp
@@ -99,6 +99,7 @@
 		if (std::atoi(e) > 0) s.grid_bwd_chunks = (uint32_t)std::atoi(e);
 	if (const char* e = std::getenv("TCNN_GRID_BWD_RANGES"))
 		if (std::atoi(e) > 0) s.grid_bwd_ranges = (uint32_t)std::atoi(e);
+	if (const char* e = std::getenv("TCNN_GRID_BWD_STREAM")) s.no_grid_bwd_stream = std::string(e) == "0";
 	if (const char* e = std::getenv("TCNN_GRID_BWD_PLAN")) s.grid_bwd_plan = std::string(e) == "feature" ? 1 : (std::string(e) == "range" ? 0 : -1);
 	return s;
 }
@@ -300,7 +301,7 @@
 }
 
 void GridEncodingHost::backward_items(hipStream_t st, GridBwdBufs& w, uint32_t B, const float* pos, uint32_t pstride, const void* dy,
-                                      int layout, uint32_t dy_stride, const GridBwdEpilogue* ep, uint32_t reserved) const {
+                                      int layout, uint32_t dy_stride, const GridBwdEpilogue* ep, uint32_t reserved, const float* dy_bound) const {
 	const uint32_t n_chunks = bwd_chunks(B, reserved);
 	w.n_chunks = n_chunks;
 	w.plan = plan_for(B, reserved);
@@ -308,7 +309,7 @@
 	if (!pl.slices.empty()) w.partial.reserve((size_t)n_chunks * n_lds_params * 4);
 	launch_grid_bwd(st, desc.n_pos_dims, desc.n_features_per_level, desc.hash_type, B, pos, pstride, dy, layout, dy_stride,
 	                pl.d_slices.as<GridSlice>(), (uint32_t)pl.slices.size(), n_chunks, w.partial.as<float>(), n_lds_params, dev_levels(),
-	                hash_grid(), desc.interp, ep, opts(), pl.slices.data(), levels.data(), (uint32_t)levels.size());
+	                hash_grid(), desc.interp, ep, opts(), pl.slices.data(), levels.data(), (uint32_t)levels.size(), dy_bound);
 }
 
 void GridEncodingHost::backward_bin(hipStream_t st, GridBwdBufs& w, uint32_t B, const float* pos, uint32_t pstride, const void* dy,
@@ -944,7 +945,8 @@
 }
 
 void NetworkHost::fused_kernel(hipStream_t st, StepWorkspace& ws, uint32_t B, const float* pos, const float* target, uint32_t dims,
-                               float loss_scale, const void* params16, bool pack, const void* dout16, void* out16, const void* enc_soa) {
+                               float loss_scale, const void* params16, bool pack, const void* dout16, void* out16, const void* enc_soa,
+                               bool emit_dy_bound) {
 	TCNN_CHECK(B % 32 == 0, "training: batch must be a multiple of 32");
 	const uint32_t n_mlp = mlp.n_params();
 	const uint32_t L = grid->desc.n_levels, F = grid->desc.n_features_per_level;
@@ -953,6 +955,8 @@
 	ws.n_fused_blocks = nb;
 	ws.n_loss_partials = nb;
 	ws.dLdenc.reserve((size_t)L * F * B * 2);
+	ws.dy_bound_live = emit_dy_bound && !sw.no_grid_bwd_stream && !dout16 && !enc_soa && grid->desc.n_pos_dims == 2 && F == 2;
+	if (ws.dy_bound_live) ws.dy_bound.reserve((size_t)L * (B / 32) * 4);
 	ws.wgrad_partial.reserve((size_t)nb * n_mlp * 4);
 	ws.loss_partial.reserve((size_t)nb * 4);
 	ws.wimage.reserve(fused_weight_image_bytes(mlp.width, mlp.n_input, mlp.n_hidden_layers));
@@ -967,7 +971,7 @@
 	                   ws.wgrad_partial.as<float>(), ws.loss_partial.as<float>(), grid->dev_levels(), grid->hash_grid(),
 	                   grid->desc.interp, nb, dout16, use_image ? ws.wimage.p : nullptr, loss_l2,
 	                   grid->inrange_index_ok && grid->desc.interp == Interp::Linear && !sw.no_inrange_index, enc_soa,
-	                   dout16 ? ext_dout_scale : 1.0f);
+	                   dout16 ? ext_dout_scale : 1.0f, ws.dy_bound_live ? ws.dy_bound.as<float>() : nullptr);
 }
 
 void NetworkHost::grid_backward(hipStream_t st, StepWorkspace& ws, uint32_t B, const float* pos, GridBwdEpilogue* ep) {
@@ -981,7 +985,8 @@
 		ep->n_wparts = ws.n_fused_blocks;
 		ep->lpart = ws.loss_partial.as<float>();
 	}
-	grid->backward_items(st, ws.gbw, B, pos, grid->desc.n_pos_dims, ws.dLdenc.p, 0, 0, ep, ep ? ep->n_mlp_groups : 0u);
+	grid->backward_items(st, ws.gbw, B, pos, grid->desc.n_pos_dims, ws.dLdenc.p, 0, 0, ep, ep ? ep->n_mlp_groups : 0u,
+	                     ws.dy_bound_live ? ws.dy_bound.as<float>() : nullptr);
 	grid->backward_bin(st, ws.gbw, B, pos, grid->desc.n_pos_dims, ws.dLdenc.p, 0, 0);
 	if (ep && ep->apply_adam) ws.wimage_valid = true;
 }
@@ -1242,7 +1247,7 @@
 		m.grid->forward(st, B, input, m.grid->desc.n_pos_dims, m.enc_params(w16.p), ws.enc16.p, true, 0);
 		enc_soa = ws.enc16.p;
 	}
-	m.fused_kernel(st, ws, B, input, target, n_output_dims, loss_scale, w16.p, false, nullptr, nullptr, enc_soa);
+	m.fused_kernel(st, ws, B, input, target, n_output_dims, loss_scale, w16.p, false, nullptr, nullptr, enc_soa, true);
 	mark(st, 1);
 	if (run_optimizer) ++adam_step;
 	GridBwdEpilogue ep{};
@@ -1329,7 +1334,7 @@
 	                           (uint64_t)(uintptr_t)w32.p, (uint64_t)(uintptr_t)w16.p, (uint64_t)(uintptr_t)g16.p,
 	                           (uint64_t)(uintptr_t)g32.p, (uint64_t)(uintptr_t)m1.p, (uint64_t)(uintptr_t)m2.p,
 	                           (uint64_t)(uintptr_t)steps.p, (uint64_t)(uintptr_t)d_loss.p, (uint64_t)(uintptr_t)d_ftable.p,
-	                           (uint64_t)(uintptr_t)ws.dLdenc.p, (uint64_t)(uintptr_t)ws.wgrad_partial.p,
+	                           (uint64_t)(uintptr_t)ws.dLdenc.p, (uint64_t)(uintptr_t)ws.dy_bound.p, (uint64_t)(uintptr_t)ws.wgrad_partial.p,
 	                           (uint64_t)(uintptr_t)ws.loss_partial.p, (uint64_t)(uintptr_t)ws.wimage.p,
 	                           (uint64_t)(uintptr_t)ws.gbw.partial.p, (uint64_t)(uintptr_t)ws.gbw.recs.p,
 	                           (uint64_t)(uintptr_t)ws.gbw.dir.p, (uint64_t)(uintptr_t)ws.gbw.dysum.p, ws.n_fused_blocks,
@@ -1481,7 +1486,7 @@
 		return;
 	}
 	if (part == 0) {
-		m.fused_kernel(st, ws, B, input, target, n_output_dims, loss_scale, w16.p, false);
+		m.fused_kernel(st, ws, B, input, target, n_output_dims, loss_scale, w16.p, false, nullptr, nullptr, nullptr, true);
 		launch_column_sums(st, ws.wgrad_partial.as<float>(), ws.n_fused_blocks, (uint32_t)n_mlp, g32.as<float>());
 		launch_sum(st, ws.loss_partial.as<float>(), ws.n_loss_partials, d_loss.as<float>());
 		last_B = B;
diff --git a/neuralbtf-tiny-cuda-nn_amd/csrc/runtime.h b/neuralbtf-tiny-cuda-nn_amd/csrc/runtime.h
--- a/neuralbtf-tiny-cuda-nn_amd/csrc/runtime.h
+++ b/neuralbtf-tiny-cuda-nn_amd/csrc/runtime.h
@@ -70,6 +70,7 @@
 	uint32_t grid_bwd_chunks = 0;
 	uint32_t grid_bwd_ranges = 0;
 	int grid_bwd_plan = -1;
+	bool no_grid_bwd_stream = false;
 	static EngineSwitches from_env();
 };
 
@@ -127,7 +128,7 @@
 	}
 	GridBinArgs bin_args(GridBwdBufs& w, uint32_t B) const;
 	void backward_items(hipStream_t st, GridBwdBufs& w, uint32_t B, const float* pos, uint32_t pstride, const void* dy, int layout,
-	                    uint32_t dy_stride, const GridBwdEpilogue* ep = nullptr, uint32_t reserved = 0) const;
+	                    uint32_t dy_stride, const GridBwdEpilogue* ep = nullptr, uint32_t reserved = 0, const float* dy_bound = nullptr) const;
 	void backward_bin(hipStream_t st, GridBwdBufs& w, uint32_t B, const float* pos, uint32_t pstride, const void* dy, int layout,
 	                  uint32_t dy_stride) const;
 	void backward_acc(hipStream_t st, GridBwdBufs& w, uint32_t B, const void* dy, int layout, uint32_t dy_stride, float* grad32,
@@ -237,6 +238,8 @@
 
 struct StepWorkspace {
 	DevBuf dLdenc, wgrad_partial, loss_partial, grad32_tmp, out16, enc16, wimage;
+	DevBuf dy_bound;
+	bool dy_bound_live = false;
 	GridBwdBufs gbw;
 	DevBuf acts, delta0, delta1, dout16, red_tmp;
 	DevBuf tile_wT;
@@ -283,7 +286,7 @@
 
 	void fused_kernel(hipStream_t st, StepWorkspace& ws, uint32_t B, const float* pos, const float* target, uint32_t dims,
 	                  float loss_scale, const void* params16, bool pack, const void* dout16 = nullptr, void* out16 = nullptr,
-	                  const void* enc_soa = nullptr);
+	                  const void* enc_soa = nullptr, bool emit_dy_bound = false);
 	void grid_backward(hipStream_t st, StepWorkspace& ws, uint32_t B, const float* pos, GridBwdEpilogue* ep = nullptr);
 	void pack_weights(hipStream_t st, StepWorkspace& ws, const void* params16);
 
```

Measured after the change: 12140 training steps/s (2^18-sample batches, whole job), median of 6. 3.7% higher.
